# IRVLUTD/Proto-CLIP

Measured on AMD Instinct MI355X. Metric: query images/sec, ImageNet 16-shot ViT-B/16 (few-shot top-1 parity: tests/), higher is better.
Workload: dtype f16; 1 GPU; C3 ImageNet 16-shot ViT-B/16 conv-3x: prototype reduce + encode_image + adapter + dual-bank classify; batch_per_gpu=1024, global_batch=1024, classes=1000, shots=16, embed_dim=512, parallelism=dp1 (support rows and queries sharded; all-gather of class sums)

## Files before the change

### include/pclip.h

```cpp
#ifndef PCLIP_H
#define PCLIP_H
#include <stddef.h>
#include <stdint.h>

#ifdef __cplusplus
extern "C" {
#endif

#define PCLIP_ABI_VERSION 1
#define PCLIP_OK 0
#define PCLIP_E_INVALID (-1)
#define PCLIP_E_LAUNCH (-2)
#define PCLIP_E_WORKSPACE (-3)

typedef void* pclip_stream_t;

int pclip_abi_version(void);
const char* pclip_last_error(void);
int pclip_device_cus(void);
int pclip_gemm_timing(void* buf, int nslots);
int pclip_gemm_timing_count(void);
long pclip_gemm_kernel_launches(void);


int pclip_l2norm_rows_f16(const void* x, void* y, int R, int D, float* sq_out, pclip_stream_t stream);

int pclip_row_sqnorm_f16(const void* x, int R, int D, float* sq_out, pclip_stream_t stream);

int pclip_proto_build_f16(const void* mem, int N, int K, int D, int per_shot_norm, void* proto_f16,
                          float* proto_f32, float* proto_sq, pclip_stream_t stream);

int pclip_bank_reduce_f16(const void* feats, int A, int R, int D, const int32_t* perm, void* keys,
                          pclip_stream_t stream);

int pclip_transpose_f16(const void* x, int R, int C, void* y, pclip_stream_t stream);

int pclip_partial_sums_f16(const void* mem, const int32_t* labels, int R, int N, int D, int per_shot_norm,
                           float* sums, int32_t* counts, pclip_stream_t stream);

int pclip_proto_finalize(const float* sums, const int32_t* counts, int W, int N, int D, void* proto_f16,
                         float* proto_f32, float* proto_sq, pclip_stream_t stream);


int pclip_sqdist_f16(const void* q, const void* zi, const void* zt, int Q, int N, int D,
                     const float* q_sq, const float* zi_sq, const float* zt_sq,
                     float* d2i, float* d2t, int ldd, void* ws, size_t ws_bytes, pclip_stream_t stream);

int pclip_sqdist_f32(const float* q, const float* zi, const float* zt, int Q, int N, int D, float* d2i,
                     float* d2t, int ldd, pclip_stream_t stream);

int pclip_fuse_probs(const float* d2i, const float* d2t, int Q, int N, int ldd, float alpha,
                     float one_minus_alpha, float beta, float* p, int32_t* argmax, float* topk_p,
                     int32_t* topk_i, int k, pclip_stream_t stream);

int pclip_classify_f16(const void* q, const void* zi, const void* zt, int Q, int N, int D,
                       const float* q_sq, const float* zi_sq, const float* zt_sq, float alpha,
                       float one_minus_alpha, float beta, float* p, int32_t* argmax, float* topk_p,
                       int32_t* topk_i, int k, void* ws, size_t ws_bytes, pclip_stream_t stream);
int pclip_classify_ex_f16(const void* q, const void* zi, const void* zt, int Q, int N, int D,
                          const float* q_sq, const float* zi_sq, const float* zt_sq, float alpha,
                          float one_minus_alpha, float beta, float* p, int32_t* argmax, float* topk_p,
                          int32_t* topk_i, int k, int flags, void* ws, size_t ws_bytes, pclip_stream_t stream);

#define PCLIP_CLASSIFY_NO_SMALL 0x1
#define PCLIP_CLASSIFY_NO_MID 0x2
#define PCLIP_CLASSIFY_FORCE_MID 0x4
#define PCLIP_CLASSIFY_NO_PANELS 0x8
#define PCLIP_CLASSIFY_FORCE_PANELS 0x10
#define PCLIP_CLASSIFY_PANEL_TWO_PASS 0x20
#define PCLIP_CLASSIFY_PANEL_FORCE_SECOND 0x40
#define PCLIP_CLASSIFY_PANEL_EXACT 0x80

int pclip_classify_route(int Q, int N, int D, float alpha, float one_minus_alpha, float beta, int has_zt, int want_p, int want_argmax, int topk, size_t ws_bytes);
int pclip_classify_route_ex(int Q, int N, int D, float alpha, float one_minus_alpha, float beta, int has_zt, int want_p, int want_argmax, int topk, int flags,
                            size_t ws_bytes);

int pclip_classify_panel_stats(int* out3, int reset);

int pclip_classify_panel_dump_f16(const void* q, const void* zi, const void* zt, int Q, int N, int D, float* dump, int exact,
                                  void* ws, size_t ws_bytes, pclip_stream_t stream);


int pclip_cosine_logits_f16(const void* a, int lda, int M, const void* b, int ldb, int T, int D, float scale, int flags,
                            void* logits, int ldl, int32_t* argmax, void* topk_v, int32_t* topk_i, int k,
                            void* ws, size_t ws_bytes, pclip_stream_t stream);
#define PCLIP_LOGITS_NORMALIZE_A 0x1
#define PCLIP_LOGITS_NORMALIZE_B 0x2


int pclip_cosine_ce_f16(const void* a, int lda, int M, const void* b, int ldb, int T, int D, float scale, int flags, const void* labels,
                        float* lse_row, float* lse_col, float* row_loss, float* loss, void* ws, size_t ws_bytes, pclip_stream_t stream);
int pclip_cosine_ce_backward_f16(const void* a, int lda, int M, const void* b, int ldb, int T, int D, float scale, int flags, const void* labels,
                                 const float* lse_row, const float* lse_col, float weight, int direction, float* grad, float* dscale,
                                 void* ws, size_t ws_bytes, pclip_stream_t stream);
#define PCLIP_CE_NORMALIZE_A 0x1
#define PCLIP_CE_NORMALIZE_B 0x2
#define PCLIP_CE_SYMMETRIC 0x4
#define PCLIP_CE_LABELS_I64 0x8

int pclip_cosine_ce_grouped_f16(const void* a, int lda, size_t gsa, int M, const void* b, int ldb, size_t gsb, int T, int D, int G, float scale, int flags,
                                const void* labels, float* lse_row, float* row_loss, float* loss, void* ws, size_t ws_bytes, pclip_stream_t stream);
int pclip_cosine_ce_grouped_backward_f16(const void* a, int lda, size_t gsa, int M, const void* b, int ldb, size_t gsb, int T, int D, int G, float scale,
                                         int flags, const void* labels, const float* lse_row, float weight, int direction, float* grad, float* dscale,
                                         void* ws, size_t ws_bytes, pclip_stream_t stream);
size_t pclip_cosine_ce_grouped_workspace(int backward, int G, int M, int T, int D);


int pclip_cosine_sigmoid_f16(const void* a, int lda, int M, const void* b, int ldb, int T, int D, float scale, float bias, int flags,
                             const void* ids_a, const void* ids_b, float* row_loss, float* loss, void* ws, size_t ws_bytes, pclip_stream_t stream);
int pclip_cosine_sigmoid_backward_f16(const void* a, int lda, int M, const void* b, int ldb, int T, int D, float scale, float bias, int flags,
                                      const void* ids_a, const void* ids_b, float weight, int direction, float* grad, float* dscale, float* dbias,
                                      void* ws, size_t ws_bytes, pclip_stream_t stream);
#define PCLIP_SIG_NORMALIZE_A 0x1
#define PCLIP_SIG_NORMALIZE_B 0x2
#define PCLIP_SIG_IDS_I64 0x8


int pclip_tip_logits_f16(const void* f, int ldf, int Q, const void* keys, int ldk, int NK, const int32_t* seg, const void* w, int ldw, int N, int D,
                         float scale, float alpha, float beta, void* logits, int ldl, float* logits32, int32_t* argmax, pclip_stream_t stream);
int pclip_tip_grid_f16(const void* f, int ldf, int Q, const void* keys, int ldk, int NK, const int32_t* seg, const void* w, int ldw, int N, int D,
                       float scale, const float* betas, int nb, const float* alphas, int na, const int32_t* labels, int32_t* correct, pclip_stream_t stream);

int pclip_tip_keys_backward_f16(const void* f, int ldf, int Q, const void* keys, int ldk, int NK, const int32_t* seg, int N, int D, float alpha, float beta,
                                const float* dL, float* dkeys, void* ws, size_t ws_bytes, pclip_stream_t stream);

int pclip_hp_sweep(const float* d2i, const float* d2t, const int32_t* labels, int Q, int N, int ldd,
                   const float* alphas, const float* one_minus_alphas, int na, const float* betas,
                   int nb, int32_t* correct, pclip_stream_t stream);


int pclip_adapter_fc_f16(const void* x, int B, int D, int H, const void* w1, const void* g1, const void* b1,
                         const void* w2, const void* g2, const void* b2, float ratio, float one_minus_ratio,
                         int l2norm_out, void* y, float* y_sq, void* ws, size_t ws_bytes,
                         pclip_stream_t stream);

int pclip_layernorm_blend_f16(const void* h, const void* gamma, const void* beta, float eps, const void* x, float ratio,
                              float one_minus_ratio, int l2norm_out, void* y, float* y_sq, int R, int D,
                              pclip_stream_t stream);

int pclip_adapter_conv_f16(const void* x, int B, int D, int three_x, const void* conv1, const void* ln1w,
                           const void* ln1b, const void* conv2, const void* ln2w, const void* ln2b,
                           const void* conv3, const void* ln3w, const void* ln3b, int l2norm_out, void* y,
                           float* y_sq, pclip_stream_t stream);

int pclip_adapter_conv_w_f16(const void* x, int B, int D, int three_x, int width, const void* conv1, const void* ln1w,
                             const void* ln1b, const void* conv2, const void* ln2w, const void* ln2b,
                             const void* conv3, const void* ln3w, const void* ln3b, int l2norm_out, void* y,
                             float* y_sq, pclip_stream_t stream);


int pclip_gemm_f16(const void* A, int lda, const void* B, int ldb, void* C, int ldc, int M, int N, int K,
                   const void* bias, int act, const void* residual, pclip_stream_t stream);

int pclip_gemm4w_f16(const void* A, int lda, const void* B, int ldb, void* C, int ldc, int M, int N, int K,
                     const void* bias, int act, const void* residual, pclip_stream_t stream);
int pclip_gemm4w_var_f16(const void* A, int lda, const void* B, int ldb, void* C, int ldc, int M, int N, int K,
                         const void* bias, int act, const void* residual, int var, pclip_stream_t stream);
#define PCLIP_ROUTE_AUTO (-1)
#define PCLIP_ROUTE_GENERIC 5
#define PCLIP_ROUTE_RING 6
#define PCLIP_ROUTE_FIELDS 5
#define PCLIP_ROUTE_RAN_FOUR_WAVE 10
#define PCLIP_ROUTE_RAN_RING 11
#define PCLIP_ROUTE_RAN_GENERIC 12
int pclip_gemm_route_f16(const void* A, int lda, const void* B, int ldb, void* C, int ldc, int M, int N, int K,
                         const void* bias, int act, const void* residual, const float* scale, const float* shift,
                         int cfg, int may_split, int band, int band_n, int rev, int use4w, int cus,
                         int* report, int report_len, pclip_stream_t stream);
int pclip_gemm4w_stamp_buffer(void* stamps);
int pclip_gemm4w_config(int mode);

size_t pclip_gemm_splitk_workspace(int M, int N, int K);
int pclip_gemm_splitk_f16(const void* A, int lda, const void* B, int ldb, void* C, int ldc, int M, int N, int K,
                          const void* bias, int act, void* ws, size_t ws_bytes, pclip_stream_t stream);

int pclip_gemm_bn_f16(const void* A, int lda, const void* B, int ldb, void* C, int ldc, int M, int N, int K,
                      const float* scale, const float* shift, int relu, pclip_stream_t stream);

int pclip_gemm_bn_res_f16(const void* A, int lda, const void* B, int ldb, void* C, int ldc, int M, int N, int K,
                          const float* scale, const float* shift, const void* residual, pclip_stream_t stream);

int pclip_conv3x3_bn_f16(const void* x, const void* w, const void* zero_line, int B, int H, int W, int Cin, int Cout,
                         const float* scale, const float* shift, int relu, void* y, pclip_stream_t stream);

int pclip_conv3x3_strip_applies(int B, int H, int W, int Cin, int Cout);
int pclip_conv3x3_strip_config(int mode);

int pclip_conv3x3_pool_applies(int H, int W, int Cin, int Cout);
int pclip_conv3x3_bn_pool_f16(const void* x, const void* w, int B, int H, int W, int Cin, int Cout, const float* scale, const float* shift, void* y,
                              pclip_stream_t stream);

int pclip_stem_conv_applies(int R, int Cout);
int pclip_stem_conv_bn_f16(const void* img, int img_is_f32, int B, int R, const void* w, int Cout, const float* scale, const float* shift, int relu, void* y,
                           pclip_stream_t stream);

int pclip_layernorm_f16(const void* x, int ld_x, const float* gamma, const float* beta, float eps, void* y,
                        int R, int D, pclip_stream_t stream);

int pclip_add_layernorm_f16(const void* x, const void* delta, int ld, void* x_out, const float* gamma,
                            const float* beta, float eps, void* y, int R, int D, pclip_stream_t stream);

int pclip_attention_f16(const void* qkv, void* out, int B, int L, int H, int dh, int causal,
                        pclip_stream_t stream);

int pclip_attention_q_f16(const void* q, int ldq, long q_batch_stride, const void* kv, int ldkv, int k_off, int v_off, void* out,
                          int B, int L, int Lq, int H, int dh, int causal, pclip_stream_t stream);

int pclip_attention_long_q_f16(const void* q, int ldq, long q_batch_stride, const void* kv, int ldkv, int k_off, int v_off, void* out,
                               int B, int L, int Lq, int H, int dh, int causal, pclip_stream_t stream);

int pclip_attention_config(int mode, int max_grid);

int pclip_im2col_patches_f16(const void* img, int B, int R, int P, void* cols, int ld, pclip_stream_t stream);
int pclip_im2col_patches_f32(const float* img, int B, int R, int P, void* cols, int ld, pclip_stream_t stream);
int pclip_vit_assemble_tokens_f16(const void* patch_emb, const void* class_emb, const void* pos_emb, int B,
                                  int G2, int W, void* tokens, pclip_stream_t stream);
int pclip_vit_embed_ln_f16(const void* patch_emb, const void* class_emb, const void* pos_emb, int B, int G2, int W,
                           const float* gamma_pre, const float* beta_pre, const float* gamma_1, const float* beta_1, float eps,
                           void* x0, void* h, pclip_stream_t stream);

int pclip_text_embed_f16(const int64_t* tokens, const void* tok_emb, const void* pos_emb, int B, int L, int W,
                         int vocab, void* x, pclip_stream_t stream);
int pclip_gather_eot_f16(const void* x, const int64_t* tokens, int B, int L, int W, void* out,
                         pclip_stream_t stream);


int pclip_im2col3x3_f16(const void* x, long sb, long sh, long sw, long sc, int B, int H, int W, int C, int stride,
                        void* cols, int ld, pclip_stream_t stream);

int pclip_bn_act_f16(const void* x, const float* scale, const float* shift, const void* residual, int relu, void* y,
                     size_t rows, int C, pclip_stream_t stream);

int pclip_avgpool_nhwc_f16(const void* x, int B, int H, int W, int C, int k, void* y, pclip_stream_t stream);

int pclip_attnpool_tokens_f16(const void* x, const void* pos, int B, int HW, int C, void* tokens, pclip_stream_t stream);

int pclip_cast_f32_f16(const float* x, void* y, size_t n, pclip_stream_t stream);


int pclip_cast_f16_f32(const void* x, float* y, size_t n, pclip_stream_t stream);

int pclip_gemm_f32(const void* A, int a_f16, long rsa, long csa, const void* B, int b_f16, long rsb, long csb, float* C, int ldc,
                   int M, int N, int K, float alpha, float beta, void* ws, size_t ws_bytes, pclip_stream_t stream);

int pclip_colsum_f32(const float* x, int ldx, int R, int C, float scale, float* out, int accumulate, void* ws, size_t ws_bytes,
                     pclip_stream_t stream);

int pclip_addscaled_rows_f32(float* C, int ldc, const float* X, int ldx, const float* rowscale, float s, int R, int D,
                             pclip_stream_t stream);

int pclip_nll_grad(const float* d2i, const float* d2t, const int32_t* labels, int Q, int q_total, int N, int ldd, float alpha,
                   float one_minus_alpha, float beta, float* gi, float* gt, float* rowsum, float* nll, float* pmax,
                   int32_t* argmax, pclip_stream_t stream);

int pclip_fuse_probs_backward(const float* d2i, const float* d2t, const float* dp, int ldp, int Q, int N, int ldd, float alpha,
                              float one_minus_alpha, float beta, float* gi, float* gt, float* rowsum, pclip_stream_t stream);

int pclip_nll_mean_backward(const float* p, int ldp, const int32_t* labels, int Q, int N, const float* g, float* dp, int lddp,
                            pclip_stream_t stream);

int pclip_nll_rows(const float* p, int ldp, const int32_t* labels, int Q, int N, float* nll, float* pmax, int32_t* argmax,
                   pclip_stream_t stream);

int pclip_softmax_ce_rows(const float* S, int lds, int R, int C, float scale, float* dS, int ldds, float* loss,
                          pclip_stream_t stream);

int pclip_l2norm_rows_f32(const float* x, float* y, int R, int D, float eps, pclip_stream_t stream);
int pclip_l2norm_rows_backward_f32(const float* x, const float* gy, float* gx, int R, int D, float eps, int accumulate,
                                   pclip_stream_t stream);

int pclip_proto_backward_f16(const void* mem, const float* g, int N, int K, int D, int per_shot_norm, int final_norm, void* dmem,
                             pclip_stream_t stream);

int pclip_layernorm_backward_f16(const void* x, int ldx, const void* gamma, const void* dy, int lddy, int R, int D, float eps,
                                 float dy_scale, void* dx, int lddx, float* part, int nblk, pclip_stream_t stream);

int pclip_adapter_conv_backward_partials(int B, int D, int three_x);
int pclip_adapter_conv_backward_f16(const void* x, const void* g, int B, int D, int three_x, const void* conv1, const void* ln1w,
                                    const void* ln1b, const void* conv2, const void* ln2w, const void* ln2b, const void* conv3,
                                    const void* ln3w, float* pw1, float* pw2, float* pw3, float* pg1, float* pb1, float* pg2,
                                    float* pb2, float* pg3, float* pb3, pclip_stream_t stream);

int pclip_adapter_conv_w_backward_partials(int B, int D, int three_x, int width);
int pclip_adapter_conv_w_backward_f16(const void* x, const void* g, int B, int D, int three_x, int width, const void* conv1,
                                      const void* ln1w, const void* ln1b, const void* conv2, const void* ln2w, const void* ln2b,
                                      const void* conv3, const void* ln3w, float* pw1, float* pw2, float* pw3, float* pg1, float* pb1,
                                      float* pg2, float* pb2, float* pg3, float* pb3, pclip_stream_t stream);


int pclip_attention_backward_f16(const void* qkv, const void* dout, void* dqkv, int B, int L, int H, int dh, int causal,
                                 pclip_stream_t stream);

int pclip_quick_gelu_backward_f16(const void* u, const void* dy, void* du, size_t n, pclip_stream_t stream);

int pclip_colsum_f16(const void* x, int ldx, int R, int C, float* part, int nslice, pclip_stream_t stream);

int pclip_layernorm_backward_g32_f16(const void* x, int ldx, const float* gamma, const void* dy, int lddy, const void* residual, int ldr,
                                     int R, int D, float eps, void* dx, int lddx, float* part, int nblk, pclip_stream_t stream);



int pclip_prompt_embed_f16(const int64_t* tokens, int L_tok, const void* tok_emb, const void* pos_emb, const float* ctx, int class_specific,
                           int n_ctx, int N, int L_out, int W, int vocab, void* x, pclip_stream_t stream);

#define PCLIP_PROMPT_CTX_SLICE 16
int pclip_prompt_ctx_grad_f32(const void* dx, int N, int L_out, int n_ctx, int W, int class_specific, float* dctx, float* part, int nslice,
                              pclip_stream_t stream);


#define PCLIP_VPT_MAX_L 288
#define PCLIP_VPT_SLICE 16

int pclip_vpt_append_f16(const void* t, const float* ctx, int B, int L0, int P, int W, void* out, pclip_stream_t stream);

int pclip_vpt_replace_f16(void* x, const float* ctx, int B, int L0, int P, int W, pclip_stream_t stream);

int pclip_vpt_grad_f32(void* g, int B, int L0, int P, int W, int clear, float* dctx, float* part, int nslice, pclip_stream_t stream);



int pclip_rows_replace_f16(void* x, const float* ctx, int B, int L, int off, int P, int W, pclip_stream_t stream);

int pclip_rows_grad_f32(void* g, int B, int L, int off, int P, int W, int clear, float* dctx, float* part, int nslice, pclip_stream_t stream);

#define PCLIP_COUPLE_MAX_P 16
#define PCLIP_COUPLE_SLICE 32
int pclip_couple_fwd_f32(const float* X, const float* Wc, const float* bc, int depth, int P, int Wt, int Wv, float* Y, pclip_stream_t stream);

int pclip_couple_bwd_f32(const float* dY, const float* X, const float* Wc, int depth, int P, int Wt, int Wv, float* dWc, float* dbc, float* dX,
                         float* part, int nslice, pclip_stream_t stream);


#define PCLIP_COCOOP_MAX_B 16
int pclip_metanet_fwd_f32(const void* f, const float* W1, const float* b1, const float* W2, const float* b2, int B, int E, int Hd, int Wt, float* h,
                          float* pi, pclip_stream_t stream);

int pclip_metanet_bwd_f32(const float* dpi, const void* f, const float* h, const float* W2, int B, int E, int Hd, int Wt, float* dW1, float* db1,
                          float* dW2, float* db2, float* dpre, pclip_stream_t stream);

int pclip_prompt_embed_cond_f16(const int64_t* tokens, int L_tok, const void* tok_emb, const void* pos_emb, const float* ctx, const float* pi, int n_ctx,
                                int B, int N, int L_out, int W, int vocab, void* x, pclip_stream_t stream);

int pclip_prompt_cond_grad_f32(const void* dx, int B, int N, int L_out, int n_ctx, int W, float* dshift, float* dctx, float* dpi, float* part, int nslice,
                               pclip_stream_t stream);


#define PCLIP_EMBED_BWD_CHUNK 128

int pclip_text_embed_backward(const void* dx, const int64_t* sorted_ids, const int64_t* order, int B, int L, int W, int V, float* dE, float* dpos,
                              float* part, pclip_stream_t stream);

int pclip_vit_embed_backward_f16(const void* dt, int B, int L, int W, float* dpos, void* dpatch, pclip_stream_t stream);

int pclip_adamw_f16(void* p, const void* g, void* m, void* v, size_t n, double lr, double beta1, double beta2, double eps,
                    double weight_decay, int step, pclip_stream_t stream);

#define PCLIP_TOWER_CHUNK 4096
#define PCLIP_TOWER_ROW_BYTES 64
#define PCLIP_TOWER_STATE_BYTES 64
#define PCLIP_TOWER_PARAM_F16 0x1
#define PCLIP_TOWER_GRAD_F16 0x2
#define PCLIP_TOWER_ALIGNED 0x4
#define PCLIP_TOWER_DECAY 0x8

int pclip_tower_grad_sumsq(const void* table, int ntensors, int nchunks, float* partials, pclip_stream_t stream);

int pclip_tower_optim_finish(const float* partials, int nchunks, void* state, float max_norm, double beta1, double beta2, float growth,
                             float backoff, int growth_interval, int dynamic, pclip_stream_t stream);

int pclip_tower_adamw(const void* table, const float* hyper, int ntensors, int nchunks, const void* state, double beta1, double beta2,
                      double eps, pclip_stream_t stream);


int pclip_preprocess_u8(const void* const* srcs, const int32_t* desc, int B, int n_px, int max_box_h, float mean0, float mean1,
                        float mean2, float std0, float std1, float std2, void* out, int out_f16, void* ws, pclip_stream_t stream);

#define PCLIP_OP_SQDIST 1
#define PCLIP_OP_CLASSIFY 2
#define PCLIP_OP_ADAPTER_FC 3
#define PCLIP_OP_LOGITS 4
#define PCLIP_OP_COSINE_CE 5
#define PCLIP_OP_COSINE_CE_BACKWARD 6
#define PCLIP_OP_TIP_BACKWARD 7
#define PCLIP_OP_COSINE_SIGMOID 8
#define PCLIP_OP_COSINE_SIGMOID_BACKWARD 9
size_t pclip_workspace_bytes(int op, int Q, int N, int D);

#ifdef __cplusplus
}
#endif
#endif
```

### proto-clip_amd/_lib.py

```python
import ctypes
import os
from ctypes import c_char_p, c_double, c_float, c_int, c_long, c_size_t, c_void_p

import torch

_HERE = os.path.dirname(os.path.abspath(__file__))
LIB_PATH = os.path.join(_HERE, "libpclip.so")

OP_SQDIST, OP_CLASSIFY, OP_ADAPTER_FC, OP_LOGITS, OP_COSINE_CE, OP_COSINE_CE_BACKWARD, OP_TIP_BACKWARD = 1, 2, 3, 4, 5, 6, 7
OP_COSINE_SIGMOID, OP_COSINE_SIGMOID_BACKWARD = 8, 9
LOGITS_NORMALIZE_A, LOGITS_NORMALIZE_B = 0x1, 0x2
SIG_NORMALIZE_A, SIG_NORMALIZE_B, SIG_IDS_I64 = 0x1, 0x2, 0x8
CE_NORMALIZE_A, CE_NORMALIZE_B, CE_SYMMETRIC, CE_LABELS_I64 = 0x1, 0x2, 0x4, 0x8
CLASSIFY_NO_SMALL, CLASSIFY_NO_MID, CLASSIFY_FORCE_MID, CLASSIFY_NO_PANELS, CLASSIFY_FORCE_PANELS = 0x1, 0x2, 0x4, 0x8, 0x10
CLASSIFY_PANEL_TWO_PASS, CLASSIFY_PANEL_FORCE_SECOND, CLASSIFY_PANEL_EXACT = 0x20, 0x40, 0x80
TIP_MAX_ALPHAS, TIP_MAX_CLASSES, TIP_MAX_D = 32, 4096, 2048
TOWER_CHUNK, TOWER_ROW_BYTES, TOWER_STATE_BYTES = 4096, 64, 64
TOWER_PARAM_F16, TOWER_GRAD_F16, TOWER_ALIGNED, TOWER_DECAY = 0x1, 0x2, 0x4, 0x8
ROUTE_AUTO, ROUTE_GENERIC, ROUTE_RING, ROUTE_FIELDS = -1, 5, 6, 5
ROUTE_RAN = {0: "cfg0", 1: "cfg1", 2: "cfg2", 3: "cfg3", 4: "cfg4", 10: "four_wave", 11: "ring", 12: "generic"}
EMBED_BWD_CHUNK = 128
PROMPT_CTX_SLICE = 16
VPT_SLICE, VPT_MAX_L = 16, 288
COUPLE_MAX_P, COUPLE_SLICE = 16, 32
COCOOP_MAX_B = 16


class PclipError(RuntimeError):
    pass


_lib = None

_P = c_void_p
_SIGS = {
    "pclip_abi_version": [],
    "pclip_last_error": [],
    "pclip_device_cus": [],
    "pclip_gemm_kernel_launches": [],
    "pclip_l2norm_rows_f16": [_P, _P, c_int, c_int, _P, _P],
    "pclip_row_sqnorm_f16": [_P, c_int, c_int, _P, _P],
    "pclip_proto_build_f16": [_P, c_int, c_int, c_int, c_int, _P, _P, _P, _P],
    "pclip_bank_reduce_f16": [_P, c_int, c_int, c_int, _P, _P, _P],
    "pclip_transpose_f16": [_P, c_int, c_int, _P, _P],
    "pclip_partial_sums_f16": [_P, _P, c_int, c_int, c_int, c_int, _P, _P, _P],
    "pclip_proto_finalize": [_P, _P, c_int, c_int, c_int, _P, _P, _P, _P],
    "pclip_sqdist_f16": [_P, _P, _P, c_int, c_int, c_int, _P, _P, _P, _P, _P, c_int, _P, c_size_t, _P],
    "pclip_sqdist_f32": [_P, _P, _P, c_int, c_int, c_int, _P, _P, c_int, _P],
    "pclip_fuse_probs": [_P, _P, c_int, c_int, c_int, c_float, c_float, c_float, _P, _P, _P, _P, c_int, _P],
    "pclip_classify_f16": [_P, _P, _P, c_int, c_int, c_int, _P, _P, _P, c_float, c_float, c_float, _P, _P, _P,
                           _P, c_int, _P, c_size_t, _P],
    "pclip_classify_ex_f16": [_P, _P, _P, c_int, c_int, c_int, _P, _P, _P, c_float, c_float, c_float, _P, _P, _P,
                              _P, c_int, c_int, _P, c_size_t, _P],
    "pclip_classify_panel_stats": [_P, c_int],
    "pclip_classify_panel_dump_f16": [_P, _P, _P, c_int, c_int, c_int, _P, c_int, _P, c_size_t, _P],
    "pclip_gemm_timing": [_P, c_int],
    "pclip_gemm_timing_count": [],
    "pclip_classify_route": [c_int, c_int, c_int, c_float, c_float, c_float, c_int, c_int, c_int, c_int, c_size_t],
    "pclip_classify_route_ex": [c_int, c_int, c_int, c_float, c_float, c_float, c_int, c_int, c_int, c_int, c_int, c_size_t],
    "pclip_cosine_logits_f16": [_P, c_int, c_int, _P, c_int, c_int, c_int, c_float, c_int, _P, c_int, _P, _P, _P, c_int, _P, c_size_t, _P],
    "pclip_cosine_ce_f16": [_P, c_int, c_int, _P, c_int, c_int, c_int, c_float, c_int, _P, _P, _P, _P, _P, _P, c_size_t, _P],
    "pclip_cosine_ce_backward_f16": [_P, c_int, c_int, _P, c_int, c_int, c_int, c_float, c_int, _P, _P, _P, c_float, c_int, _P, _P, _P, c_size_t, _P],
    "pclip_cosine_ce_grouped_f16": [_P, c_int, c_size_t, c_int, _P, c_int, c_size_t, c_int, c_int, c_int, c_float, c_int, _P, _P, _P, _P, _P, c_size_t, _P],
    "pclip_cosine_ce_grouped_backward_f16": [_P, c_int, c_size_t, c_int, _P, c_int, c_size_t, c_int, c_int, c_int, c_float, c_int, _P, _P, c_float, c_int, _P, _P,
                                             _P, c_size_t, _P],
    "pclip_cosine_ce_grouped_workspace": [c_int, c_int, c_int, c_int, c_int],
    "pclip_cosine_sigmoid_f16": [_P, c_int, c_int, _P, c_int, c_int, c_int, c_float, c_float, c_int, _P, _P, _P, _P, _P, c_size_t, _P],
    "pclip_cosine_sigmoid_backward_f16": [_P, c_int, c_int, _P, c_int, c_int, c_int, c_float, c_float, c_int, _P, _P, c_float, c_int, _P, _P, _P, _P, c_size_t, _P],
    "pclip_tip_logits_f16": [_P, c_int, c_int, _P, c_int, c_int, _P, _P, c_int, c_int, c_int, c_float, c_float, c_float, _P, c_int, _P, _P, _P],
    "pclip_tip_grid_f16": [_P, c_int, c_int, _P, c_int, c_int, _P, _P, c_int, c_int, c_int, c_float, _P, c_int, _P, c_int, _P, _P, _P],
    "pclip_tip_keys_backward_f16": [_P, c_int, c_int, _P, c_int, c_int, _P, c_int, c_int, c_float, c_float, _P, _P, _P, c_size_t, _P],
    "pclip_hp_sweep": [_P, _P, _P, c_int, c_int, c_int, _P, _P, c_int, _P, c_int, _P, _P],
    "pclip_adapter_fc_f16": [_P, c_int, c_int, c_int, _P, _P, _P, _P, _P, _P, c_float, c_float, c_int, _P, _P, _P,
                             c_size_t, _P],
    "pclip_layernorm_blend_f16": [_P, _P, _P, c_float, _P, c_float, c_float, c_int, _P, _P, c_int, c_int, _P],
    "pclip_adapter_conv_f16": [_P, c_int, c_int, c_int, _P, _P, _P, _P, _P, _P, _P, _P, _P, c_int, _P, _P, _P],
    "pclip_adapter_conv_w_f16": [_P, c_int, c_int, c_int, c_int, _P, _P, _P, _P, _P, _P, _P, _P, _P, c_int, _P, _P, _P],
    "pclip_gemm_f16": [_P, c_int, _P, c_int, _P, c_int, c_int, c_int, c_int, _P, c_int, _P, _P],
    "pclip_gemm4w_f16": [_P, c_int, _P, c_int, _P, c_int, c_int, c_int, c_int, _P, c_int, _P, _P],
    "pclip_gemm4w_var_f16": [_P, c_int, _P, c_int, _P, c_int, c_int, c_int, c_int, _P, c_int, _P, c_int, _P],
    "pclip_gemm_route_f16": [_P, c_int, _P, c_int, _P, c_int, c_int, c_int, c_int, _P, c_int, _P, _P, _P, c_int, c_int, c_int, c_int, c_int, c_int, c_int,
                             _P, c_int, _P],
    "pclip_gemm4w_stamp_buffer": [_P],
    "pclip_gemm4w_config": [c_int],
    "pclip_gemm_splitk_workspace": [c_int, c_int, c_int],
    "pclip_gemm_splitk_f16": [_P, c_int, _P, c_int, _P, c_int, c_int, c_int, c_int, _P, c_int, _P, c_size_t, _P],
    "pclip_gemm_bn_f16": [_P, c_int, _P, c_int, _P, c_int, c_int, c_int, c_int, _P, _P, c_int, _P],
    "pclip_gemm_bn_res_f16": [_P, c_int, _P, c_int, _P, c_int, c_int, c_int, c_int, _P, _P, _P, _P],
    "pclip_conv3x3_bn_f16": [_P, _P, _P, c_int, c_int, c_int, c_int, c_int, _P, _P, c_int, _P, _P],
    "pclip_conv3x3_strip_applies": [c_int, c_int, c_int, c_int, c_int],
    "pclip_conv3x3_strip_config": [c_int],
    "pclip_conv3x3_pool_applies": [c_int, c_int, c_int, c_int],
    "pclip_conv3x3_bn_pool_f16": [_P, _P, c_int, c_int, c_int, c_int, c_int, _P, _P, _P, _P],
    "pclip_stem_conv_applies": [c_int, c_int],
    "pclip_stem_conv_bn_f16": [_P, c_int, c_int, c_int, _P, c_int, _P, _P, c_int, _P, _P],
    "pclip_layernorm_f16": [_P, c_int, _P, _P, c_float, _P, c_int, c_int, _P],
    "pclip_add_layernorm_f16": [_P, _P, c_int, _P, _P, _P, c_float, _P, c_int, c_int, _P],
    "pclip_attention_f16": [_P, _P, c_int, c_int, c_int, c_int, c_int, _P],
    "pclip_attention_q_f16": [_P, c_int, c_long, _P, c_int, c_int, c_int, _P, c_int, c_int, c_int, c_int, c_int, c_int, _P],
    "pclip_attention_long_q_f16": [_P, c_int, c_long, _P, c_int, c_int, c_int, _P, c_int, c_int, c_int, c_int, c_int, c_int, _P],
    "pclip_attention_config": [c_int, c_int],
    "pclip_im2col_patches_f16": [_P, c_int, c_int, c_int, _P, c_int, _P],
    "pclip_im2col_patches_f32": [_P, c_int, c_int, c_int, _P, c_int, _P],
    "pclip_vit_assemble_tokens_f16": [_P, _P, _P, c_int, c_int, c_int, _P, _P],
    "pclip_vit_embed_ln_f16": [_P, _P, _P, c_int, c_int, c_int, _P, _P, _P, _P, c_float, _P, _P, _P],
    "pclip_text_embed_f16": [_P, _P, _P, c_int, c_int, c_int, c_int, _P, _P],
    "pclip_gather_eot_f16": [_P, _P, c_int, c_int, c_int, _P, _P],
    "pclip_im2col3x3_f16": [_P, c_long, c_long, c_long, c_long, c_int, c_int, c_int, c_int, c_int, _P, c_int, _P],
    "pclip_bn_act_f16": [_P, _P, _P, _P, c_int, _P, c_size_t, c_int, _P],
    "pclip_avgpool_nhwc_f16": [_P, c_int, c_int, c_int, c_int, c_int, _P, _P],
    "pclip_attnpool_tokens_f16": [_P, _P, c_int, c_int, c_int, _P, _P],
    "pclip_cast_f32_f16": [_P, _P, c_size_t, _P],
    "pclip_cast_f16_f32": [_P, _P, c_size_t, _P],
    "pclip_gemm_f32": [_P, c_int, c_long, c_long, _P, c_int, c_long, c_long, _P, c_int, c_int, c_int, c_int, c_float, c_float, _P, c_size_t, _P],
    "pclip_colsum_f32": [_P, c_int, c_int, c_int, c_float, _P, c_int, _P, c_size_t, _P],
    "pclip_adapter_conv_backward_f16": [_P, _P, c_int, c_int, c_int] + [_P] * 8 + [_P] * 9 + [_P],
    "pclip_adapter_conv_backward_partials": [c_int, c_int, c_int],
    "pclip_adapter_conv_w_backward_f16": [_P, _P, c_int, c_int, c_int, c_int] + [_P] * 8 + [_P] * 9 + [_P],
    "pclip_adapter_conv_w_backward_partials": [c_int, c_int, c_int, c_int],
    "pclip_addscaled_rows_f32": [_P, c_int, _P, c_int, _P, c_float, c_int, c_int, _P],
    "pclip_nll_grad": [_P, _P, _P, c_int, c_int, c_int, c_int, c_float, c_float, c_float, _P, _P, _P, _P, _P, _P, _P],
    "pclip_nll_rows": [_P, c_int, _P, c_int, c_int, _P, _P, _P, _P],
    "pclip_fuse_probs_backward": [_P, _P, _P, c_int, c_int, c_int, c_int, c_float, c_float, c_float, _P, _P, _P, _P],
    "pclip_nll_mean_backward": [_P, c_int, _P, c_int, c_int, _P, _P, c_int, _P],
    "pclip_softmax_ce_rows": [_P, c_int, c_int, c_int, c_float, _P, c_int, _P, _P],
    "pclip_l2norm_rows_f32": [_P, _P, c_int, c_int, c_float, _P],
    "pclip_l2norm_rows_backward_f32": [_P, _P, _P, c_int, c_int, c_float, c_int, _P],
    "pclip_proto_backward_f16": [_P, _P, c_int, c_int, c_int, c_int, c_int, _P, _P],
    "pclip_layernorm_backward_f16": [_P, c_int, _P, _P, c_int, c_int, c_int, c_float, c_float, _P, c_int, _P, c_int, _P],
    "pclip_attention_backward_f16": [_P, _P, _P, c_int, c_int, c_int, c_int, c_int, _P],
    "pclip_quick_gelu_backward_f16": [_P, _P, _P, c_size_t, _P],
    "pclip_colsum_f16": [_P, c_int, c_int, c_int, _P, c_int, _P],
    "pclip_layernorm_backward_g32_f16": [_P, c_int, _P, _P, c_int, _P, c_int, c_int, c_int, c_float, _P, c_int, _P, c_int, _P],
    "pclip_prompt_embed_f16": [_P, c_int, _P, _P, _P, c_int, c_int, c_int, c_int, c_int, c_int, _P, _P],
    "pclip_prompt_ctx_grad_f32": [_P, c_int, c_int, c_int, c_int, c_int, _P, _P, c_int, _P],
    "pclip_vpt_append_f16": [_P, _P, c_int, c_int, c_int, c_int, _P, _P],
    "pclip_vpt_replace_f16": [_P, _P, c_int, c_int, c_int, c_int, _P],
    "pclip_vpt_grad_f32": [_P, c_int, c_int, c_int, c_int, c_int, _P, _P, c_int, _P],
    "pclip_rows_replace_f16": [_P, _P, c_int, c_int, c_int, c_int, c_int, _P],
    "pclip_rows_grad_f32": [_P, c_int, c_int, c_int, c_int, c_int, c_int, _P, _P, c_int, _P],
    "pclip_couple_fwd_f32": [_P, _P, _P, c_int, c_int, c_int, c_int, _P, _P],
    "pclip_couple_bwd_f32": [_P, _P, _P, c_int, c_int, c_int, c_int, _P, _P, _P, _P, c_int, _P],
    "pclip_metanet_fwd_f32": [_P, _P, _P, _P, _P, c_int, c_int, c_int, c_int, _P, _P, _P],
    "pclip_metanet_bwd_f32": [_P, _P, _P, _P, c_int, c_int, c_int, c_int, _P, _P, _P, _P, _P, _P],
    "pclip_prompt_embed_cond_f16": [_P, c_int, _P, _P, _P, _P, c_int, c_int, c_int, c_int, c_int, c_int, _P, _P],
    "pclip_prompt_cond_grad_f32": [_P, c_int, c_int, c_int, c_int, c_int, _P, _P, _P, _P, c_int, _P],
    "pclip_text_embed_backward": [_P, _P, _P, c_int, c_int, c_int, c_int, _P, _P, _P, _P],
    "pclip_vit_embed_backward_f16": [_P, c_int, c_int, c_int, _P, _P, _P],
    "pclip_adamw_f16": [_P, _P, _P, _P, c_size_t, c_double, c_double, c_double, c_double, c_double, c_int, _P],
    "pclip_tower_grad_sumsq": [_P, c_int, c_int, _P, _P],
    "pclip_tower_optim_finish": [_P, c_int, _P, c_float, c_double, c_double, c_float, c_float, c_int, c_int, _P],
    "pclip_tower_adamw": [_P, _P, c_int, c_int, _P, c_double, c_double, c_double, _P],
    "pclip_preprocess_u8": [_P, _P, c_int, c_int, c_int, c_float, c_float, c_float, c_float, c_float, c_float, _P, c_int, _P, _P],
    "pclip_workspace_bytes": [c_int, c_int, c_int, c_int],
}
_RESTYPES = {"pclip_last_error": c_char_p, "pclip_workspace_bytes": c_size_t, "pclip_gemm_splitk_workspace": c_size_t, "pclip_cosine_ce_grouped_workspace": c_size_t, "pclip_gemm_kernel_launches": c_long}
EXPORTED_SYMBOLS = tuple(_SIGS)


def load():
    global _lib
    if _lib is not None:
        return _lib
    if not os.path.exists(LIB_PATH):
        raise PclipError(
            f"{LIB_PATH} is missing: the HIP extension is not built. Run `python -c 'import __graft_entry__ as g; "
            "g.build()'` (or `make -C proto-clip_amd/csrc`). There is no CPU/eager fallback for this path.")
    lib = ctypes.CDLL(LIB_PATH)
    for name, argtypes in _SIGS.items():
        fn = getattr(lib, name)
        fn.argtypes = argtypes
        fn.restype = _RESTYPES.get(name, c_int)
    if lib.pclip_abi_version() != 1:
        raise PclipError(f"libpclip ABI version {lib.pclip_abi_version()} != 1")
    _lib = lib
    return lib


def check(rc: int, what: str):
    if rc != 0:
        msg = load().pclip_last_error()
        raise PclipError(f"{what} failed (rc={rc}): {msg.decode() if msg else '?'}")


def ptr(t):
    return None if t is None else c_void_p(t.data_ptr())


def stream():
    return c_void_p(torch.cuda.current_stream().cuda_stream)


def require_cuda(*tensors):
    dev = None
    for t in tensors:
        if t is None:
            continue
        if not t.is_cuda:
            raise PclipError("libpclip operates on device tensors only (got a CPU tensor); there is no CPU fallback")
        if dev is None:
            dev = t.device
        elif t.device != dev:
            raise PclipError(f"operands on different GPUs ({dev} and {t.device}): move them to one device")
    if dev is not None and dev.index != torch.cuda.current_device():
        raise PclipError(f"operands live on {dev} but the current device is cuda:{torch.cuda.current_device()}: call "
                         f"torch.cuda.set_device({dev.index}) or wrap the call in `with torch.cuda.device({dev.index}):`")


def workspace_bytes(op: int, Q: int, N: int, D: int) -> int:
    return int(load().pclip_workspace_bytes(op, Q, N, D))
```

### proto-clip_amd/csrc/pclip_attention.hip

```cpp
#include "pclip_attention_tile.h"
#include <stdlib.h>
#include <type_traits>

namespace {
constexpr int ATT_MAX_L = 288;

template <int NW, int VAR, bool QF = false>
__global__ __launch_bounds__(NW * 64, NW / 2) void attention_kernel(const half_t* __restrict__ qp, int ldq, long q_batch,
                                                           const half_t* __restrict__ kvp, int ldkv, int k_off, int v_off,
                                                           half_t* __restrict__ out, int L, int Lq, int H, int causal, int NT,
                                                           int ) {
    extern __shared__ __attribute__((aligned(16))) char smem[];
    const int LP = NT * 32;
    half_t* Ks = reinterpret_cast<half_t*>(smem);
    half_t* Vs = Ks + LP * ATT_DH;
    const int b = blockIdx.x / H, h = blockIdx.x % H;
    const int W = H * ATT_DH;
    const half_t* kbase = kvp + (size_t)b * L * ldkv + h * ATT_DH + k_off;
    const half_t* vbase = kvp + (size_t)b * L * ldkv + h * ATT_DH + v_off;
    const half_t* qbase = qp + (size_t)b * q_batch + h * ATT_DH;
    const int tid = threadIdx.x, lane = tid & 63, wave = tid >> 6;
    half8_t qf0[4];
    if (QF) {
        const int q0 = wave * 32 + (lane & 31), qc0 = q0 < Lq ? q0 : Lq - 1;
#pragma unroll
        for (int s_ = 0; s_ < 4; ++s_) qf0[s_] = ld_half8(qbase + (size_t)qc0 * ldq + s_ * 16 + (lane >> 5) * 8);
    }

    for (int r0 = wave * 8; r0 < LP; r0 += NW * 8) {
        const int r = r0 + (lane >> 3);
        const int c = (lane & 7) ^ pgemm::swz_key(r);
        const int rc = r < L ? r : L - 1;
        __builtin_amdgcn_global_load_lds((pgemm::gbl_ptr_t)(kbase + (size_t)rc * ldkv + c * 8),
                                         (pgemm::lds_ptr_t)(Ks + r0 * ATT_DH), 16, 0, 0);
    }
    for (int r0 = wave * 8; r0 < LP; r0 += NW * 8) {
        const int r = r0 + (lane >> 3);
        const int c = (lane & 7) ^ (((r >> 1) & 1) << 2);
        const int rc = r < L ? r : L - 1;
        __builtin_amdgcn_global_load_lds((pgemm::gbl_ptr_t)(vbase + (size_t)rc * ldkv + c * 8),
                                         (pgemm::lds_ptr_t)(Vs + r0 * ATT_DH), 16, 0, 0);
    }
#ifndef PCLIP_ATT_VBAR
#define PCLIP_ATT_VBAR 1
#endif
    constexpr bool VB = PCLIP_ATT_VBAR && QF;
    if (VB) {
        const int nv = (LP - wave * 8 + NW * 8 - 1) / (NW * 8);
        if (nv <= 1) pgemm::wait_vm<1>(); else if (nv == 2) pgemm::wait_vm<2>(); else if (nv == 3) pgemm::wait_vm<3>(); else pgemm::wait_vm<4>();
        pgemm::lds_barrier();
    } else
        __syncthreads();

    const int hi = lane >> 5, ql = lane & 31;
    int voff[2];
    attn_voff(lane, voff);
    const int NTq = (Lq + 31) >> 5;
    auto process = [&](int qb, const half8_t (&qf)[4]) {
        const int q = qb * 32 + ql;
        float16_t o[2];
        float lrun;
        attn_query_tile<false, VAR, VB>(Ks, Vs, qf, q, qb, L, causal, NT, hi, ql, voff, o, lrun);
        attn_store_tile(out + ((size_t)b * Lq + q) * W + h * ATT_DH, o, lrun, hi, q < Lq);
    };
    if (QF) {
        if (wave < NTq) process(wave, qf0);
        else if (VB) { pgemm::wait_vm<0>(); pgemm::lds_barrier(); }
        return;
    }
    for (int qb = wave; qb < NTq; qb += NW) {
        const int q = qb * 32 + ql;
        const int qc = q < Lq ? q : Lq - 1;
        half8_t qf[4];
#pragma unroll
        for (int s = 0; s < 4; ++s) qf[s] = ld_half8(qbase + (size_t)qc * ldq + s * 16 + hi * 8);
        process(qb, qf);
    }
}

template <int NW, int WPS, int VAR>
__global__ __launch_bounds__(NW * 64, WPS) void attention_pipe_kernel(const half_t* __restrict__ qp, int ldq, long q_batch,
                                                                      const half_t* __restrict__ kvp, int ldkv, int k_off, int v_off,
                                                                      half_t* __restrict__ out, int L, int H, int causal, int NT, int KR,
                                                                      int nitems) {
    extern __shared__ __attribute__((aligned(16))) char smem[];
    constexpr int NST = 4;
    constexpr int MAXP = 4;
    constexpr int RB = ATT_DH * 2;
    const int LP = NT * 32;
    const int BUF = (KR + LP) * RB;
    const int tid = threadIdx.x, lane = tid & 63, wave = __builtin_amdgcn_readfirstlane(tid >> 6);
    const int hi = lane >> 5, ql = lane & 31;
    const int W = H * ATT_DH, G = gridDim.x;
    const bool has_tile = wave < NT;
    const unsigned lds0 = (unsigned)(size_t)(pgemm::lds_ptr_t)smem;
    char* Qs = smem + 2 * BUF;
    int voff[2];
    attn_voff(lane, voff);
    int kvo[MAXP], vvo[MAXP], qvo[MAXP];
#pragma unroll
    for (int i = 0; i < MAXP; ++i) {
        const int r = wave * 8 + i * NW * 8 + (lane >> 3);
        const int rc = r < L ? r : L - 1;
        const int ck = ((lane & 7) ^ pgemm::swz_key(r)) << 3, cv = ((lane & 7) ^ (((r >> 1) & 1) << 2)) << 3;
        kvo[i] = (rc * ldkv + ck) * 2;
        vvo[i] = (rc * ldkv + cv) * 2;
        qvo[i] = (rc * ldq + ck) * 2;
    }
    const int q = wave * 32 + ql;
    auto stage = [&](int item, int buf) {
        const int b = item / H, h = item - b * H;
        const uint4_t rkv = attn_rsrc(kvp + (size_t)b * L * ldkv + h * ATT_DH);
        const uint4_t rq = attn_rsrc(qp + (size_t)b * q_batch + h * ATT_DH);
        const unsigned kb = lds0 + buf * BUF, vb = kb + KR * RB, qb = lds0 + 2 * BUF;
#pragma unroll
        for (int i = 0; i < MAXP; ++i) {
            const int r0 = wave * 8 + i * NW * 8;
            if (r0 < KR) attn_dma16(rkv, kvo[i], k_off * 2, kb + r0 * RB);
        }
#pragma unroll
        for (int i = 0; i < MAXP; ++i) {
            const int r0 = wave * 8 + i * NW * 8;
            if (r0 < LP) attn_dma16(rkv, vvo[i], v_off * 2, vb + r0 * RB);
        }
#pragma unroll
        for (int i = 0; i < MAXP; ++i) {
            const int r0 = wave * 8 + i * NW * 8;
            if (r0 < KR) attn_dma16(rq, qvo[i], 0, qb + r0 * RB);
        }
    };
    int item = blockIdx.x;
    if (item >= nitems) return;
    stage(item, 0);
    for (int it = 0; item < nitems; item += G, ++it) {
        const int cur = it & 1;
        if (has_tile && it > 0) pgemm::wait_vm<NST>(); else pgemm::wait_vm<0>();
        pgemm::lds_barrier();
        half8_t qf[4];
        if (has_tile) {
            const int qr = q < KR ? q : KR - 1;
#pragma unroll
            for (int s = 0; s < 4; ++s)
                qf[s] = *reinterpret_cast<const half8_t*>(Qs + qr * RB + (((s * 2 + hi) ^ pgemm::swz_key(qr)) << 4));
        }
        pgemm::lds_barrier();
#ifndef PCLIP_ATT_ABL
#define PCLIP_ATT_ABL 0
#endif
        const int next = item + G;
        if (next < nitems && !(PCLIP_ATT_ABL & 1)) stage(next, cur ^ 1);
        if (has_tile) {
            const half_t* Ks = reinterpret_cast<const half_t*>(smem + cur * BUF);
            const half_t* Vs = Ks + KR * ATT_DH;
            float16_t o[2];
            float lrun;
#ifndef PCLIP_ATT_STAGGER
#define PCLIP_ATT_STAGGER 0
#endif
#if PCLIP_ATT_STAGGER && defined(__HIP_DEVICE_COMPILE__)
            if (wave >= NW / 2) __builtin_amdgcn_s_sleep(PCLIP_ATT_STAGGER);
#endif
            if (PCLIP_ATT_ABL & 2) {
#pragma unroll
                for (int j = 0; j < 2; ++j)
#pragma unroll
                    for (int e = 0; e < 16; ++e) o[j][e] = (float)qf[e & 3][e & 7];
                lrun = 1.f;
            } else
                attn_query_tile<true, VAR>(Ks, Vs, qf, q, wave, L, causal, NT, hi, ql, voff, o, lrun);
            const int b = item / H, h = item - b * H;
            attn_store_tile(out + ((size_t)b * L + q) * W + h * ATT_DH, o, lrun, hi, q < L && !(PCLIP_ATT_ABL & 4));
        }
    }
}

}

static int att_mode_from_env() {
    const char* e = getenv("PCLIP_ATT_PIPE");
    return e && (e[0] == '0' || e[0] == '1') ? e[0] - '0' : -1;
}
static int g_att_mode = att_mode_from_env(), g_att_grid = 0;
extern "C" int pclip_attention_config(int mode, int max_grid) {
    PCLIP_REQUIRE(mode >= -1 && mode <= 1 && max_grid >= 0, "pclip_attention_config: bad mode=%d max_grid=%d", mode, max_grid);
    g_att_mode = mode;
    g_att_grid = max_grid;
    return PCLIP_OK;
}

extern "C" int pclip_attention_q_f16(const void* q, int ldq, long q_batch_stride, const void* kv, int ldkv, int k_off, int v_off,
                                     void* out, int B, int L, int Lq, int H, int dh, int causal, pclip_stream_t stream) {
    PCLIP_REQUIRE(q && kv && out, "pclip_attention_q_f16: null pointer");
    PCLIP_REQUIRE(dh == ATT_DH, "pclip_attention_q_f16: head dim %d unsupported (must be 64)", dh);
    PCLIP_REQUIRE(B >= 0 && H > 0 && L > 0 && L <= ATT_MAX_L && Lq > 0 && Lq <= L, "pclip_attention_q_f16: bad B=%d H=%d L=%d Lq=%d (L <= %d)",
                  B, H, L, Lq, ATT_MAX_L);
    PCLIP_REQUIRE(!causal || Lq == L, "pclip_attention_q_f16: the causal mask needs all queries (Lq == L)");
    PCLIP_REQUIRE(ldq % 8 == 0 && ldkv % 8 == 0 && k_off % 8 == 0 && v_off % 8 == 0 && q_batch_stride % 8 == 0,
                  "pclip_attention_q_f16: strides / offsets must be multiples of 8 halves");
    if (B == 0) return PCLIP_OK;
    const int NT = ceil_div(L, 32), LP = NT * 32;
    const long nitems = (long)B * H;
    const int cus = pclip_device_cus();
    const int KR = (L + 7) / 8 * 8;
    const size_t plds = (2 * (size_t)(KR + LP) + KR) * ATT_DH * 2;
    if (Lq == L && g_att_mode != 0 && NT <= 8 && plds <= 160 * 1024 && cus > 0 && g_att_mode == 1) {
        static DevOnce pipe_attr;
        if (int e = pclip_raise_lds(pipe_attr, {(const void*)attention_pipe_kernel<4, 2, PCLIP_ATT_VAR_SHORT>, (const void*)attention_pipe_kernel<8, 2, PCLIP_ATT_VAR_LONG>},
                                    160 * 1024, "pclip_attention_f16"))
            return e;
        int per_cu = NT <= 4 ? (int)((160 * 1024) / plds) : 1;
        per_cu = per_cu < 1 ? 1 : (per_cu > 2 ? 2 : per_cu);
        long grid = (long)cus * per_cu;
        if (g_att_grid > 0 && g_att_grid < grid) grid = g_att_grid;
        if (grid > nitems) grid = nitems;
        if (NT <= 4)
            attention_pipe_kernel<4, 2, PCLIP_ATT_VAR_SHORT><<<(int)grid, 256, plds, (hipStream_t)stream>>>((const half_t*)q, ldq, q_batch_stride, (const half_t*)kv, ldkv,
                                                                                      k_off, v_off, (half_t*)out, L, H, causal, NT, KR, (int)nitems);
        else
            attention_pipe_kernel<8, 2, PCLIP_ATT_VAR_LONG><<<(int)grid, 512, plds, (hipStream_t)stream>>>((const half_t*)q, ldq, q_batch_stride, (const half_t*)kv, ldkv,
                                                                                      k_off, v_off, (half_t*)out, L, H, causal, NT, KR, (int)nitems);
        return pclip_check_launch("attention (pipelined)");
    }
    const size_t lds = 2 * (size_t)LP * ATT_DH * 2;
    static DevOnce attr_set;
    if (int e = pclip_raise_lds(attr_set, {(const void*)attention_kernel<8, PCLIP_ATT_VAR_LONG>, (const void*)attention_kernel<4, PCLIP_ATT_VAR_LONG>,
                                           (const void*)attention_kernel<4, PCLIP_ATT_VAR_SHORT>, (const void*)attention_kernel<8, PCLIP_ATT_VAR_LONG, true>,
                                           (const void*)attention_kernel<4, PCLIP_ATT_VAR_SHORT, true>},
                                80 * 1024, "pclip_attention_f16"))
        return e;
#define PCLIP_ATT_LAUNCH(NW, VAR)                                                                                                         \
    attention_kernel<NW, VAR><<<B * H, NW * 64, lds, (hipStream_t)stream>>>((const half_t*)q, ldq, q_batch_stride, (const half_t*)kv, ldkv, k_off, \
                                                                             v_off, (half_t*)out, L, Lq, H, causal, NT, 0)
    static const bool qfirst = pclip_env_on("PCLIP_ATT_QFIRST");
    if (PCLIP_ATT_QF4 && qfirst && NT <= 4 && Lq == L && !causal)
        attention_kernel<4, PCLIP_ATT_VAR_SHORT, true><<<B * H, 4 * 64, lds, (hipStream_t)stream>>>((const half_t*)q, ldq, q_batch_stride, (const half_t*)kv, ldkv, k_off,
                                                                                                     v_off, (half_t*)out, L, Lq, H, causal, NT, 0);
    else if ((Lq + 31) / 32 > 4 && (Lq + 31) / 32 <= 8 && NT <= 8 && qfirst)
        attention_kernel<8, PCLIP_ATT_VAR_LONG, true><<<B * H, 8 * 64, lds, (hipStream_t)stream>>>((const half_t*)q, ldq, q_batch_stride, (const half_t*)kv, ldkv, k_off,
                                                                                                    v_off, (half_t*)out, L, Lq, H, causal, NT, 0);
    else if ((Lq + 31) / 32 > 4) PCLIP_ATT_LAUNCH(8, PCLIP_ATT_VAR_LONG);
    else if (NT > 4) PCLIP_ATT_LAUNCH(4, PCLIP_ATT_VAR_LONG);
    else PCLIP_ATT_LAUNCH(4, PCLIP_ATT_VAR_SHORT);
#undef PCLIP_ATT_LAUNCH
    return pclip_check_launch("attention");
}

extern "C" int pclip_attention_f16(const void* qkv, void* out, int B, int L, int H, int dh, int causal,
                                   pclip_stream_t stream) {
    PCLIP_REQUIRE(qkv && out, "pclip_attention_f16: null pointer");
    PCLIP_REQUIRE(H > 0 && L > 0, "pclip_attention_f16: bad H=%d L=%d", H, L);
    const int W = H * dh;
    return pclip_attention_q_f16(qkv, 3 * W, (long)L * 3 * W, qkv, 3 * W, W, 2 * W, out, B, L, L, H, dh, causal, stream);
}
```

### proto-clip_amd/csrc/pclip_gemm4w.hip

```cpp
#include "pclip_gemm.h"
#include "pclip_epilogue.h"
#include "pclip_gemm4w_loop.inc"
#include <stdlib.h>

unsigned long long* pclip_gemm_time_slot();
static unsigned* g_gemm4w_stamps = nullptr;

namespace {
using Cfg4 = pgemm::Cfg<256, 256, 2, 2>;
constexpr int RING_BYTES = 5 * 32768;
typedef unsigned uint4_t __attribute__((ext_vector_type(4)));

enum Build : int {
    PRODUCT = 0,
    STRESS = 1,
    NO_EPILOGUE = 6,
    STAMPED = 8,
};
constexpr bool is_build(int var) { return var == PRODUCT || var == STRESS || var == NO_EPILOGUE || var == STAMPED; }

__device__ __forceinline__ int fresh_tid(int wave) {
#if defined(__HIP_DEVICE_COMPILE__)
    int lane;
    asm volatile("v_mbcnt_lo_u32_b32 %0, -1, 0\n\tv_mbcnt_hi_u32_b32 %0, -1, %0" : "=v"(lane));
    return wave * 64 + lane;
#else
    return 0;
#endif
}

template <bool BATCH, class Ahead, class Pre, class Post, class Stamp>
__device__ __forceinline__ void epilogue4w(const pgemm::Acc16& acc, int wave, char* buf0, char* buf1, const Ahead& ahead, const Pre& pre, const Post& post,
                                           const Stamp& stamp) {
    constexpr int NSLAB = 4;
    const int tid = fresh_tid(wave);
    const int lane = tid & 63, wm = wave >> 1, wn = wave & 1;
    constexpr int RB = 512;
    auto stage = [&](int k) {
        char* buf = (k & 1) ? buf1 : buf0;
#pragma unroll
        for (int j = 0; j < 4; ++j)
#pragma unroll
            for (int g = 0; g < 4; ++g) {
                const int rl = (g >> 1) * 16 + (lane & 15), coff = (g & 1) * 16 + 4 * (lane >> 4);
                const int ml = wm * 32 + rl, nl = wn * 128 + j * 32 + coff;
                const half4_t hv = pre(acc.q[2 * k + (g >> 1)][2 * j + (g & 1)]);
                const int unit = (nl >> 2) ^ (ml & 15);
                *reinterpret_cast<half4_t*>(buf + ml * RB + unit * 8) = hv;
            }
    };
#pragma unroll
    for (int ps = 0; ps < 8; ++ps) ahead(0, ps);
    pgemm::lds_barrier();
    stamp(3);
    stage(0);
#pragma unroll
    for (int k = 0; k < NSLAB; ++k) {
        pgemm::lds_barrier();
        stamp(4 + k);
        const bool stage_first = (wave & 1) == 0;
        if (k + 1 < NSLAB && stage_first) stage(k + 1);
        const char* buf = (k & 1) ? buf1 : buf0;
        const int c = tid & 31;
        if (BATCH) {
            half8_t hv[8];
#pragma unroll
            for (int ps = 0; ps < 8; ++ps) {
                const int r = (tid >> 5) + ps * 8;
                hv[ps] = *reinterpret_cast<const half8_t*>(buf + r * RB + ((c ^ ((r & 15) >> 1)) << 4));
            }
#pragma unroll
            for (int ps = 0; ps < 8; ++ps) {
                if ((tid >> 5) & 1) hv[ps] = half8_t{hv[ps][4], hv[ps][5], hv[ps][6], hv[ps][7], hv[ps][0], hv[ps][1], hv[ps][2], hv[ps][3]};
                post(k, ps, hv[ps]);
                if (k + 1 < NSLAB) ahead(k + 1, ps);
            }
        } else {
#pragma unroll
            for (int ps = 0; ps < 8; ++ps) {
                const int r = (tid >> 5) + ps * 8;
                const int pair = c ^ ((r & 15) >> 1);
                half8_t hv = *reinterpret_cast<const half8_t*>(buf + r * RB + pair * 16);
                if (r & 1) hv = half8_t{hv[4], hv[5], hv[6], hv[7], hv[0], hv[1], hv[2], hv[3]};
                post(k, ps, hv);
                if (k + 1 < NSLAB) ahead(k + 1, ps);
            }
        }
        if (k + 1 < NSLAB && !stage_first) stage(k + 1);
    }
}

__device__ __forceinline__ uint4_t make_rsrc(const half_t* base, long bytes) {
    const uint64_t a = (uint64_t)base;
    return uint4_t{(uint32_t)__builtin_amdgcn_readfirstlane((uint32_t)a), (uint32_t)__builtin_amdgcn_readfirstlane((uint32_t)(a >> 32)) & 0xffffu,
                   (uint32_t)__builtin_amdgcn_readfirstlane((uint32_t)(bytes < 0x7fffffffL ? bytes : 0x7fffffffL)), 0x00020000u};
}

struct LaneK {
    int voffa0, voffa1, voffb0, voffb1, lanea, laneb;
    __device__ __forceinline__ LaneK(int lda, int ldb, int ring0, int wave) {
        const int lane = fresh_tid(wave) & 63, wm = wave >> 1, wn = wave & 1;
        const int r0 = wave * 64 + (lane >> 3), r1 = r0 + 8;
        const int c0 = (lane & 7) ^ pgemm::swz_key(r0), c1 = (lane & 7) ^ pgemm::swz_key(r1);
        voffa0 = (r0 * lda + c0 * 8) * 2;
        voffa1 = (r1 * lda + c1 * 8) * 2;
        voffb0 = (r0 * ldb + c0 * 8) * 2;
        voffb1 = (r1 * ldb + c1 * 8) * 2;
        const int lpart = (lane & 15) * pgemm::ROW_BYTES + (((lane >> 4) ^ ((lane & 15) >> 1)) << 4);
        lanea = ring0 + wm * 16384 + lpart;
        laneb = ring0 + wn * 16384 + lpart;
    }
};

template <int ACT, bool HAS_BIAS, int VAR>
__global__ __launch_bounds__(256, 1) void linear4w_kernel(const half_t* __restrict__ A, int lda, const half_t* __restrict__ B, int ldb, int M,
                                                          int N, int K, const half_t* __restrict__ bias, half_t* Cout, int ldc, int tiles_n,
                                                          int ntiles, const half_t* residual, int rev, int band, unsigned* stamps) {
    extern __shared__ __attribute__((aligned(16))) char smem[];
    constexpr bool STAMP = VAR == STAMPED;
    unsigned stampv = 0;
    int stamp_tile = 0;
    auto stamp = [&](int phase) {
        if constexpr (STAMP) {
#if defined(__HIP_DEVICE_COMPILE__)
            if (stamp_tile < 8) { const unsigned t = (unsigned)wall_clock64(); if ((fresh_tid(0) & 63) == stamp_tile * 8 + phase) stampv = t; }
#endif
        }
    };
    const int G = gridDim.x;
    int tile = pgemm::xcd_remap(blockIdx.x, G);
    if (tile >= ntiles) return;
    if constexpr (!STAMP) pgemm::time_begin(reinterpret_cast<unsigned long long*>(stamps));
    const int wave = __builtin_amdgcn_readfirstlane(threadIdx.x >> 6);
    const int nt = K / pgemm::BK;
    const int row16a = 16 * lda * 2, row16b = 16 * ldb * 2;
    const int ring0 = (int)(uintptr_t)smem;
    const int wbase = __builtin_amdgcn_readfirstlane(ring0 + wave * 8192);
    const int tiles_m = ntiles / tiles_n;
    auto origin = [&](int tl, int& m0, int& n0) {
        const int t = rev ? ntiles - 1 - tl : tl;
        int tm, tn;
        if (band <= 0 || band >= tiles_n) { tm = t / tiles_n; tn = t - tm * tiles_n; }
        else {
            const int per_band = tiles_m * band, bnd = t / per_band, r = t - bnd * per_band;
            const int w = band < tiles_n - bnd * band ? band : tiles_n - bnd * band;
            tm = r / w;
            tn = bnd * band + r - tm * w;
        }
        m0 = tm * 256;
        n0 = tn * 256;
    };
    auto rsrc_a = [&](int m0) { return make_rsrc(A + (size_t)m0 * lda, (long)(M - m0) * lda * 2); };
    auto rsrc_b = [&](int n0) { return make_rsrc(B + (size_t)n0 * ldb, (long)(N - n0) * ldb * 2); };
    auto bias_ptr = [&](int n0) { return (HAS_BIAS ? bias : A) + n0 + (wave & 1) * 128 + 4 * ((fresh_tid(wave) & 63) >> 4); };

    int ring_wr = 0, ring_rda = 0, ring_rdb = 0x8000;
    int m0, n0;
    origin(tile, m0, n0);
    uint4_t rsa2 = rsrc_a(m0), rsb2 = rsrc_b(n0);
    half4_t nb[8];
    {
        const half_t* biasp = bias_ptr(n0);
        const LaneK lk(lda, ldb, ring0, wave);
        const int voffa0 = lk.voffa0, voffa1 = lk.voffa1, voffb0 = lk.voffb0, voffb1 = lk.voffb1;
        int so[8], st_cnt, st_tmp, st_scr;
#if defined(__HIP_DEVICE_COMPILE__)
        if (VAR == STRESS) PCLIP_GEMM4W_COLD_STRESS(); else PCLIP_GEMM4W_COLD();
#endif
    }
    for (; tile < ntiles; tile += G) {
        stamp(0);
        const bool full = m0 + 256 <= M;
        const uint4_t rsa = rsa2, rsb = rsb2;
        int m0n = m0, n0n = n0;
        if (tile + G < ntiles) origin(tile + G, m0n, n0n);
        rsa2 = rsrc_a(m0n);
        rsb2 = rsrc_b(n0n);
        const half_t* biasp = bias_ptr(n0n);
        pgemm::Acc16 acc;
#pragma unroll
        for (int j = 0; j < 8; ++j) {
            const float4_t b = HAS_BIAS ? float4_t{(float)nb[j][0], (float)nb[j][1], (float)nb[j][2], (float)nb[j][3]} : float4_t{0.f, 0.f, 0.f, 0.f};
#pragma unroll
            for (int i = 0; i < 8; ++i) acc.q[i][j] = b;
        }
        pgemm::lds_barrier();
        stamp(1);
        {
            const LaneK lk(lda, ldb, ring0, wave);
            const int voffa0 = lk.voffa0, voffa1 = lk.voffa1, voffb0 = lk.voffb0, voffb1 = lk.voffb1, lanea = lk.lanea, laneb = lk.laneb;
            half8_t fr[32];
            int vr[4], so[8], st_cnt, st_tmp, st_scr;
#if defined(__HIP_DEVICE_COMPILE__)
            if constexpr (VAR == STRESS) PCLIP_GEMM4W_LOOP_STRESS(); else PCLIP_GEMM4W_LOOP();
#endif
        }
        stamp(2);
        if constexpr (VAR == NO_EPILOGUE) {
#if defined(__HIP_DEVICE_COMPILE__)
#pragma unroll
            for (int i = 0; i < 8; ++i)
#pragma unroll
                for (int j = 0; j < 8; ++j) asm volatile("" ::"a"(acc.q[i][j]));
#endif
            m0 = m0n;
            n0 = n0n;
            continue;
        }
        char* buf0 = smem + ring_wr;
        char* buf1 = smem + (ring_wr + 0x8000 == RING_BYTES ? 0 : ring_wr + 0x8000);
        const int etid = fresh_tid(wave);
        const int evoff = ((etid >> 5) * ldc + 8 * (etid & 31)) * 2;
        const long cbytes = ((long)(M - m0) * ldc - n0) * 2;
        pgemm::rsrc_t rc;
#if defined(__HIP_DEVICE_COMPILE__)
        {
            auto mk = [&](const half_t* base) {
                const uint64_t a = (uint64_t)(base + (size_t)m0 * ldc + n0);
                const uint32_t lo = __builtin_amdgcn_readfirstlane((uint32_t)a), hi = __builtin_amdgcn_readfirstlane((uint32_t)(a >> 32));
                return __builtin_amdgcn_make_buffer_rsrc((void*)(((uint64_t)hi << 32) | lo), 0, __builtin_amdgcn_readfirstlane((int)(cbytes < 0x7fffffffL ? cbytes : 0x7fffffffL)), 0x00020000);
            };
            rc = mk(Cout);
        }
#endif
        constexpr bool RES = ACT == 6;
        auto soff = [&](int k, int ps) { return ((ps >> 2) * 128 + k * 32 + 8 * (ps & 3)) * ldc * 2; };
        auto pre = [&](float4_t v) { return ACT == 1 ? quick_gelu16x4(v) : cvt16x4(v); };
        constexpr bool FLAT = RES;
        constexpr bool BATCH = !RES;
        const int col = n0 + 8 * (etid & 31);
        half8_t rr[RES ? 8 : 1];
        auto ahead = [&](int k, int ps) {
            if (!RES) return;
            const int r = (ps >> 2) * 128 + k * 32 + 8 * (ps & 3) + (etid >> 5);
            if (full || m0 + r < M) rr[RES ? ps : 0] = ld_half8(residual + (size_t)(m0 + r) * ldc + col);
        };
        auto add_res = [&](int pass, half8_t h) { return add_residual16x8<false>(rr[RES ? pass : 0], h); };
        if (!FLAT)
            epilogue4w<true>(acc, wave, buf0, buf1, ahead, pre, [&](int k, int ps, half8_t h) {
#if defined(__HIP_DEVICE_COMPILE__)
                __builtin_amdgcn_raw_buffer_store_b128(__builtin_bit_cast(uint4_t, h), rc, evoff, soff(k, ps), PCLIP_NT_STORE ? 2 : 0);
#endif
            }, stamp);
        else if (full)
            epilogue4w<BATCH>(acc, wave, buf0, buf1, ahead, pre, [&](int k, int ps, half8_t h) {
                const int r = (ps >> 2) * 128 + k * 32 + 8 * (ps & 3) + (etid >> 5);
                st_out(Cout + (size_t)(m0 + r) * ldc + col, add_res(ps, h));
            }, stamp);
        else
            epilogue4w<BATCH>(acc, wave, buf0, buf1, ahead, pre, [&](int k, int ps, half8_t h) {
                const int r = (ps >> 2) * 128 + k * 32 + 8 * (ps & 3) + (etid >> 5);
                if (m0 + r < M) st_out(Cout + (size_t)(m0 + r) * ldc + col, add_res(ps, h));
            }, stamp);
        m0 = m0n;
        n0 = n0n;
        ++stamp_tile;
    }
    if constexpr (!STAMP) pgemm::time_end(reinterpret_cast<unsigned long long*>(stamps));
    if constexpr (STAMP) {
        const int l = fresh_tid(wave) & 63;
        const int slot = (blockIdx.x == 0 ? 0 : (blockIdx.x == gridDim.x / 2 ? 2 : -1));
        if (stamps && slot >= 0 && (wave == 0 || wave == 3)) {
            const int w = slot + (wave == 3 ? 1 : 0);
            stamps[w * 64 + l] = stampv;
#if defined(__HIP_DEVICE_COMPILE__)
            if (l == 0) stamps[256 + w] = (unsigned)wall_clock64();
#endif
        }
    }
}

template <int ACT, bool HAS_BIAS, int VAR>
int launch4w_v(const half_t* A, int lda, const half_t* B, int ldb, int M, int N, int K, const half_t* bias, half_t* C, int ldc, const half_t* residual,
               int slots, int rev, int band, hipStream_t s) {
    static DevOnce attr;
    auto kern = linear4w_kernel<ACT, HAS_BIAS, VAR>;
    if (int e = pclip_raise_lds(attr, {(const void*)kern}, RING_BYTES, "pclip_gemm4w_f16")) return e;
    const int tiles_m = ceil_div(M, Cfg4::BM), tiles_n = N / Cfg4::BN, ntiles = tiles_m * tiles_n;
    const int grid = ntiles < slots ? ntiles : slots;
    kern<<<grid, 256, RING_BYTES, s>>>(A, lda, B, ldb, M, N, K, bias, C, ldc, tiles_n, ntiles, residual, rev, band, VAR == STAMPED ? g_gemm4w_stamps : reinterpret_cast<unsigned*>(pclip_gemm_time_slot()));
    return pclip_check_launch("gemm4w_f16");
}

template <int ACT, bool HAS_BIAS>
int launch4w(const half_t* A, int lda, const half_t* B, int ldb, int M, int N, int K, const half_t* bias, half_t* C, int ldc, const half_t* residual,
             int slots, int rev, int band, int var, hipStream_t s) {
#define PCLIP_4W_CASE(V) case V: return launch4w_v<ACT, HAS_BIAS, V>(A, lda, B, ldb, M, N, K, bias, C, ldc, residual, slots, rev, band, s)
    if constexpr (HAS_BIAS) {
        switch (var) {
            PCLIP_4W_CASE(STRESS); PCLIP_4W_CASE(NO_EPILOGUE); PCLIP_4W_CASE(STAMPED);
            default: break;
        }
    } else if (var == STRESS) return launch4w_v<ACT, HAS_BIAS, STRESS>(A, lda, B, ldb, M, N, K, bias, C, ldc, residual, slots, rev, band, s);
#undef PCLIP_4W_CASE
    return launch4w_v<ACT, HAS_BIAS, PRODUCT>(A, lda, B, ldb, M, N, K, bias, C, ldc, residual, slots, rev, band, s);
}
}

extern "C" int pclip_gemm4w_stamp_buffer(void* p) { g_gemm4w_stamps = (unsigned*)p; return PCLIP_OK; }

bool pclip_gemm4w_supports(int M, int N, int K, int lda, int ldb, int ldc, const void* C, const void* bias, const void* residual, int act) {
    if (N % 256 || K % 64 || K < 192 || M < 1) return false;
    if (lda % 8 || ldb % 8 || ldc % 8 || ((uintptr_t)C & 15) || ((uintptr_t)bias & 7) || ((uintptr_t)residual & 15)) return false;
    if ((long)256 * lda * 2 >= 0x7fffffffL || (long)256 * ldb * 2 >= 0x7fffffffL) return false;
    if (!(act == 0 || act == 1 || act == 6)) return false;
    if (act == 6 && !(bias && residual)) return false;
    if (act != 6 && residual) return false;
    return true;
}

int pclip_gemm4w_launch_var(const half_t* A, int lda, const half_t* B, int ldb, int M, int N, int K, const half_t* bias, half_t* C, int ldc, int act,
                            const half_t* residual, int slots, int rev, int band, int var, hipStream_t s) {
    if (act == 6) return launch4w<6, true>(A, lda, B, ldb, M, N, K, bias, C, ldc, residual, slots, rev, band, var, s);
    if (act == 1) return bias ? launch4w<1, true>(A, lda, B, ldb, M, N, K, bias, C, ldc, residual, slots, rev, band, var, s)
                              : launch4w<1, false>(A, lda, B, ldb, M, N, K, bias, C, ldc, residual, slots, rev, band, var, s);
    return bias ? launch4w<0, true>(A, lda, B, ldb, M, N, K, bias, C, ldc, residual, slots, rev, band, var, s)
                : launch4w<0, false>(A, lda, B, ldb, M, N, K, bias, C, ldc, residual, slots, rev, band, var, s);
}

int pclip_gemm4w_launch(const half_t* A, int lda, const half_t* B, int ldb, int M, int N, int K, const half_t* bias, half_t* C, int ldc, int act,
                        const half_t* residual, int slots, int rev, int band, hipStream_t s) {
    static const bool stress = getenv("PCLIP_RACE_STRESS") && getenv("PCLIP_RACE_STRESS")[0] == '1';
    return pclip_gemm4w_launch_var(A, lda, B, ldb, M, N, K, bias, C, ldc, act, residual, slots, rev, band, stress ? STRESS : PRODUCT, s);
}

extern "C" int pclip_gemm4w_var_f16(const void* A, int lda, const void* B, int ldb, void* C, int ldc, int M, int N, int K, const void* bias, int act,
                                    const void* residual, int var, pclip_stream_t stream) {
    PCLIP_REQUIRE(A && B && C, "pclip_gemm4w_f16: null pointer");
    PCLIP_REQUIRE(act == 0 || act == 1, "pclip_gemm4w_f16: unknown activation %d", act);
    PCLIP_REQUIRE(lda >= K && ldb >= K && ldc >= N, "pclip_gemm4w_f16: bad leading dims");
    PCLIP_REQUIRE(is_build(var), "pclip_gemm4w_f16: unknown loop variant %d", var);
    if (M == 0) return PCLIP_OK;
    const int a = (residual && bias && act == 0) ? 6 : act;
    PCLIP_REQUIRE(pclip_gemm4w_supports(M, N, K, lda, ldb, ldc, C, bias, residual, a),
                  "pclip_gemm4w_f16: shape M=%d N=%d K=%d / alignment outside the four-wave kernel (N %% 256 == 0, K %% 64 == 0, K >= 192; residual needs bias, no activation)", M, N, K);
    const char* be = getenv("PCLIP_GEMM4W_BAND");
    return pclip_gemm4w_launch_var((const half_t*)A, lda, (const half_t*)B, ldb, M, N, K, (const half_t*)bias, (half_t*)C, ldc, a, (const half_t*)residual, pclip_cus(), 0,
                                   be ? atoi(be) : 0, var, (hipStream_t)stream);
}

extern "C" int pclip_gemm4w_f16(const void* A, int lda, const void* B, int ldb, void* C, int ldc, int M, int N, int K, const void* bias, int act,
                                const void* residual, pclip_stream_t stream) {
    return pclip_gemm4w_var_f16(A, lda, B, ldb, C, ldc, M, N, K, bias, act, residual, PRODUCT, stream);
}
```

### proto-clip_amd/csrc/pclip_linear.hip

```cpp
#include "pclip_encoder_common.h"
#include <stdlib.h>
#include <type_traits>

unsigned long long* pclip_gemm_time_slot();

namespace {
template <class C, bool HAS_BIAS, int ACT>
__global__ __launch_bounds__(C::NTHREADS, 2) void linear_fast_kernel(const half_t* __restrict__ A, int lda,
                                                                     const half_t* __restrict__ B, int ldb, int M, int N,
                                                                     int K, const half_t* __restrict__ bias,
                                                                     const float* __restrict__ scale,
                                                                     const float* __restrict__ shift,
                                                                     half_t* Cout, int ldc, int tiles_n,
                                                                     int ntiles, const half_t* residual = nullptr, int band = 0,
                                                                     unsigned long long* tslot = nullptr) {
    extern __shared__ __attribute__((aligned(16))) char smem[];
    constexpr bool KT = C::TAIL;
    constexpr bool M16 = true;
    half_t* bias_lds = reinterpret_cast<half_t*>(smem + C::LDS_BYTES);
    float* affine_lds = reinterpret_cast<float*>(smem + C::LDS_BYTES);
    constexpr bool AFFINE = ACT == 2 || ACT == 3 || ACT == 5;
    const int G = gridDim.x;
    int tile = pgemm::xcd_remap(blockIdx.x, G);
    if (tile >= ntiles) return;
    pgemm::time_begin(tslot);
    const int tiles_m_all = ntiles / tiles_n;
    auto decomp = [&](int t, int& tm, int& tn) {
        if (band < 0) t = ntiles - 1 - t;
        if (band <= 0 || band >= tiles_n) { tm = t / tiles_n; tn = t - tm * tiles_n; return; }
        const int per_band = tiles_m_all * band, bnd = t / per_band, r = t - bnd * per_band;
        const int w = band < tiles_n - bnd * band ? band : tiles_n - bnd * band;
        tm = r / w;
        tn = bnd * band + r - tm * w;
    };
    int p = 0;
    const int tid = threadIdx.x, lane = tid & 63, wave = __builtin_amdgcn_readfirstlane(tid >> 6), wn = wave % C::WN;
    using TP = std::conditional_t<(PCLIP_DMA_ROLES && C::NWAVES == 8), pgemm::TilePairR<C, KT>, pgemm::TilePair<C, KT>>;
    TP tp;
    const pgemm::rsrc_t rs_bias = pgemm::make_rsrc(bias, KT ? (unsigned)N * 2u : 0x7fffffffu), rs_scale = pgemm::make_rsrc(scale, KT ? (unsigned)N * 4u : 0x7fffffffu),
                        rs_shift = pgemm::make_rsrc(shift, KT ? (unsigned)N * 4u : 0x7fffffffu);
    (void)rs_bias; (void)rs_scale; (void)rs_shift;
    auto copy_bias = [&](int t, int par) {
        int tm_, tn;
        decomp(t, tm_, tn);
        (void)tn;
#if defined(__HIP_DEVICE_COMPILE__)
        if (lane < C::BN / 8)
            __builtin_amdgcn_raw_ptr_buffer_load_lds(rs_bias, (pgemm::lds_ptr_t)(bias_lds + par * C::BN), 16, (tn * C::BN + lane * 8) * 2, 0, 0, 0);
#endif
    };
    auto copy_affine = [&](int t, int par) {
        int tm_, tn;
        decomp(t, tm_, tn);
        (void)tn;
#if defined(__HIP_DEVICE_COMPILE__)
        if (lane < C::BN / 4) {
            __builtin_amdgcn_raw_ptr_buffer_load_lds(rs_scale, (pgemm::lds_ptr_t)(affine_lds + par * 2 * C::BN), 16, (tn * C::BN + lane * 4) * 4, 0, 0, 0);
            __builtin_amdgcn_raw_ptr_buffer_load_lds(rs_shift, (pgemm::lds_ptr_t)(affine_lds + par * 2 * C::BN + C::BN), 16, (tn * C::BN + lane * 4) * 4, 0, 0, 0);
        }
#endif
    };
    if (HAS_BIAS || AFFINE) {
        if (AFFINE) copy_affine(tile, 0); else copy_bias(tile, 0);
        pgemm::wait_vm<0>();
        pgemm::lds_barrier();
    }
    {
        int tm, tn;
        decomp(tile, tm, tn);
        tp.prepare(A, lda, B, ldb, M, N, tm * C::BM, tn * C::BN, wave, lane, K);
        tp.stage(0, smem + p * C::STAGE_BYTES, wave);
    }
    constexpr int YOUNGER = C::NH * C::NPASS + (AFFINE ? 2 : (HAS_BIAS ? 1 : 0));
    bool prev_full = false;
    int parity = 0;
    for (; tile < ntiles; tile += G, parity ^= 1) {
        int tile_m, tile_n;
        decomp(tile, tile_m, tile_n);
        const int m0 = tile_m * C::BM, n0 = tile_n * C::BN;
        const bool full = m0 + C::BM <= M;
        pgemm::Acc<C> acc;
        if (HAS_BIAS) {
            if (KT ? K <= pgemm::BK : K == pgemm::BK) { pgemm::wait_vm<0>(); pgemm::lds_barrier(); }
            const half_t* bl = bias_lds + parity * C::BN + wn * (C::BN / C::WN);
#pragma unroll
            for (int j = 0; j < C::TN; ++j)
#pragma unroll
                for (int g = 0; g < 4; ++g) {
                    const int coff = (g & 1) * 16 + 4 * (lane >> 4);
                    const half4_t b = *reinterpret_cast<const half4_t*>(bl + j * 32 + coff);
#pragma unroll
                    for (int e = 0; e < 4; ++e)
#pragma unroll
                        for (int i = 0; i < C::TM; ++i) acc.v[i][j][4 * g + e] = (float)b[e];
                }
            copy_bias(tile + G < ntiles ? tile + G : tile, parity ^ 1);
        }
        if (AFFINE) copy_affine(tile + G < ntiles ? tile + G : tile, parity ^ 1);
        const int next = tile + G;
        pgemm::mainloop_sr<C, YOUNGER, !HAS_BIAS, TP>(tp, KT ? (K + pgemm::BK - 1) / pgemm::BK : K / pgemm::BK, smem, acc, p, prev_full, wave, lane);
        if (next < ntiles) {
            int tm, tn;
            decomp(next, tm, tn);
            tp.prepare(A, lda, B, ldb, M, N, tm * C::BM, tn * C::BN, wave, lane, K);
            tp.stage(0, smem + p * C::STAGE_BYTES, wave);
        }
        char* stg = smem + (p ^ 1) * C::STAGE_BYTES;
        int etid = tid;
#if defined(__HIP_DEVICE_COMPILE__)
        asm volatile("" : "+v"(etid));
#endif
        const int col = n0 + 8 * (etid % C::CPR);
        const bool colok = !KT || col < N;
        auto pre = [&](int i, int j, int coff, float4_t v, int rl, int g) {
            if (ACT == 1) return quick_gelu16x4(v);
            if (AFFINE) {
                const float* st = affine_lds + parity * 2 * C::BN + wn * (C::BN / C::WN) + j * 32 + coff;
                return bn16x4<ACT == 3>(v, *reinterpret_cast<const float4_t*>(st), *reinterpret_cast<const float4_t*>(st + C::BN));
            }
            return cvt16x4(v);
        };
        constexpr bool RES = ACT == 5 || ACT == 6;
        constexpr bool PIPE = PCLIP_EPI_PIPE && (ACT == 1 || PCLIP_EPI_PIPE == 2) && C::BM == 256 && C::BN == 256 && C::WM == 2 && C::WN == 4;
        half8_t rr[RES ? C::NPASS : 1];
        auto ahead = [&](int k) {
            if (!RES) return;
#pragma unroll
            for (int ps = 0; ps < 4; ++ps) {
                const int rs = etid / C::CPR + ps * 16, r = (rs >> 5) * 128 + k * 32 + (rs & 31);
                if ((full || m0 + r < M) && colok) rr[RES ? (k & 1) * 4 + ps : 0] = ld_half8(residual + (size_t)(m0 + r) * ldc + col);
            }
        };
        auto slab = [&](int h) {
            if (!RES) return;
#pragma unroll
            for (int ps = 0; ps < C::NPASS; ++ps) {
                const int r = h * C::HR + etid / C::CPR + ps * C::ROWS_PER_PASS;
                if ((full || m0 + r < M) && colok) rr[ps] = ld_half8(residual + (size_t)(m0 + r) * ldc + col);
            }
        };
        auto add_res = [&](int pass, half8_t h) { return add_residual16x8<ACT == 5>(rr[RES ? pass % C::NPASS : 0], h); };
        if constexpr (PIPE) {
            static_assert(C::NPASS == 8, "rr[pass % NPASS] pairs slab parity and pass");
            if (full)
                pgemm::epilogue_pipe<C>(acc, stg, ahead, pre, [&](int r, int c, int pass, half8_t h) {
                    const size_t o = (size_t)(m0 + r) * ldc + col;
                    if (RES) h = add_res(pass, h);
                    if (colok) st_out(Cout + o, h);
                });
            else
                pgemm::epilogue_pipe<C>(acc, stg, ahead, pre, [&](int r, int c, int pass, half8_t h) {
                    const size_t o = (size_t)(m0 + r) * ldc + col;
                    if (RES) h = add_res(pass, h);
                    if (m0 + r < M && colok) st_out(Cout + o, h);
                });
            prev_full = full;
            continue;
        }
        if (full)
            pgemm::epilogue_f16<C, M16>(acc, stg, slab, pre, [&](int r, int c, int pass, half8_t h) {
                const size_t o = (size_t)(m0 + r) * ldc + col;
                if (RES) h = add_res(pass, h);
                if (colok) st_out(Cout + o, h);
            });
        else
            pgemm::epilogue_f16<C, M16>(acc, stg, slab, pre, [&](int r, int c, int pass, half8_t h) {
                const size_t o = (size_t)(m0 + r) * ldc + col;
                if (RES) h = add_res(pass, h);
                if (m0 + r < M && colok) st_out(Cout + o, h);
            });
        prev_full = full;
    }
    pgemm::time_end(tslot);
}


template <class C, int ACT>
__global__ __launch_bounds__(C::NTHREADS, 2) void conv3x3_fast_kernel(const half_t* __restrict__ x,
                                                                      const half_t* __restrict__ w, int H, int W, int Cin, int M,
                                                                      int N, const float* __restrict__ scale,
                                                                      const float* __restrict__ shift, half_t* __restrict__ Cout,
                                                                      int tiles_n, int ntiles) {
    extern __shared__ __attribute__((aligned(16))) char smem[];
    float* affine_lds = reinterpret_cast<float*>(smem + C::LDS_BYTES);
    constexpr bool TAIL = C::TAIL;
    const int G = gridDim.x;
    int tile = pgemm::xcd_remap(blockIdx.x, G);
    if (tile >= ntiles) return;
    const int nt = (9 * Cin + pgemm::BK - 1) / pgemm::BK, ldb = nt * pgemm::BK;
    const int tid = threadIdx.x, lane = tid & 63, wave = __builtin_amdgcn_readfirstlane(tid >> 6), wn = wave % C::WN;
    pgemm::ConvPair<C, TAIL> cp(x, H, W, Cin, M);
    pgemm::ConvGather<C, TAIL>& ga = cp.a.g;
    const pgemm::rsrc_t rs_scale = pgemm::make_rsrc(scale, TAIL ? (unsigned)N * 4u : 0x7fffffffu), rs_shift = pgemm::make_rsrc(shift, TAIL ? (unsigned)N * 4u : 0x7fffffffu);
    (void)rs_scale; (void)rs_shift;
    auto copy_affine = [&](int t, int par) {
        const int tn = t - (t / tiles_n) * tiles_n;
        (void)tn;
#if defined(__HIP_DEVICE_COMPILE__)
        if (lane < C::BN / 4) {
            __builtin_amdgcn_raw_ptr_buffer_load_lds(rs_scale, (pgemm::lds_ptr_t)(affine_lds + par * 2 * C::BN), 16, (tn * C::BN + lane * 4) * 4, 0, 0, 0);
            __builtin_amdgcn_raw_ptr_buffer_load_lds(rs_shift, (pgemm::lds_ptr_t)(affine_lds + par * 2 * C::BN + C::BN), 16, (tn * C::BN + lane * 4) * 4, 0, 0, 0);
        }
#endif
    };
    auto stage0 = [&](int t, int pbuf) {
        const int tm = t / tiles_n, tn = t - tm * tiles_n;
        char* a = smem + pbuf * C::STAGE_BYTES;
        cp.b.prepare(w, ldb, tn * C::BN, N, wave, lane);
        cp.stage(0, a, wave);
    };
    copy_affine(tile, 0);
    pgemm::wait_vm<0>();
    pgemm::lds_barrier();
    int p = 0;
    ga.prepare((tile / tiles_n) * C::BM);
    stage0(tile, p);
    constexpr int YOUNGER = C::NH * C::NPASS + 2;
    bool prev_full = false;
    int parity = 0;
    for (; tile < ntiles; tile += G, parity ^= 1) {
        const int tile_m = tile / tiles_n, tile_n = tile - tile_m * tiles_n;
        const int m0 = tile_m * C::BM, n0 = tile_n * C::BN;
        const bool full = m0 + C::BM <= M;
        pgemm::Acc<C> acc;
        copy_affine(tile + G < ntiles ? tile + G : tile, parity ^ 1);
        pgemm::mainloop_sr<C, YOUNGER, true, pgemm::ConvPair<C, TAIL>>(cp, nt, smem, acc, p, prev_full, wave, lane);
        const int next = tile + G;
        if (next < ntiles) {
            ga.prepare((next / tiles_n) * C::BM);
            stage0(next, p);
        }
        char* stg = smem + (p ^ 1) * C::STAGE_BYTES;
        const int col = n0 + 8 * (tid % C::CPR);
        auto pre = [&](int, int j, int coff, float4_t v, int rl, int g) {
            const float* st = affine_lds + parity * 2 * C::BN + wn * (C::BN / C::WN) + j * 32 + coff;
            return bn16x4<ACT == 3>(v, *reinterpret_cast<const float4_t*>(st), *reinterpret_cast<const float4_t*>(st + C::BN));
        };
        const bool colok = !TAIL || col < N;
        if (full)
            pgemm::epilogue_f16<C, true>(acc, stg, [](int) {}, pre,
                                   [&](int r, int, int, half8_t h) { if (colok) st_half8(Cout + (size_t)(m0 + r) * N + col, h); });
        else
            pgemm::epilogue_f16<C, true>(acc, stg, [](int) {}, pre, [&](int r, int, int, half8_t h) {
                if (m0 + r < M && colok) st_half8(Cout + (size_t)(m0 + r) * N + col, h);
            });
        prev_full = full;
    }
}


template <bool KT = false>
__global__ __launch_bounds__(256, 2) void linear_generic_kernel(const half_t* __restrict__ A, int lda,
                                                                const half_t* __restrict__ B, int ldb, int M, int N,
                                                                int K, LinearEpi epi, int tiles_n) {
    using C = pgemm::CfgSmall;
    extern __shared__ __attribute__((aligned(16))) char smem[];
    const int swz = pgemm::xcd_remap(blockIdx.x, gridDim.x);
    const int tile_m = swz / tiles_n, tile_n = swz - tile_m * tiles_n;
    const int m0 = tile_m * C::BM, n0 = tile_n * C::BN;
    const int tid = threadIdx.x, wave = tid >> 6, wn = wave % C::WN;
    int p = 0;
    pgemm::stage_first<C, KT>(A, lda, B, ldb, M, N, m0, n0, smem, p, K);
    pgemm::Acc<C> acc;
    pgemm::mainloop<C, 0, true, KT, KT>(A, lda, B, ldb, M, N, K, m0, n0, smem, acc, p, false);
    const half_t* __restrict__ bias = epi.bias;
    const half_t* __restrict__ residual = epi.residual;
    const int act = epi.act, ldc = epi.ldc;
    const int col = n0 + 8 * (tid % C::CPR);
    pgemm::epilogue_f16<C, KT>(
        acc, smem + (p ^ 1) * C::STAGE_BYTES, [](int) {},
        [&](int, int j, int coff, float4_t v, int rl, int g) {
            const int n = n0 + wn * (C::BN / C::WN) + j * 32 + coff;
            half4_t h;
#pragma unroll
            for (int e = 0; e < 4; ++e) {
                float x = v[e];
                if (bias) x += (float)bias[n + e < N ? n + e : N - 1];
                x = r16(x);
                if (act == 1) x = quick_gelu16(x);
                if (act >= 2) {
                    const int nn = n + e < N ? n + e : N - 1;
                    x = r16(x * epi.scale[nn] + epi.shift[nn]);
                    if (act == 3) x = fmaxf(x, 0.f);
                }
                h[e] = (half_t)x;
            }
            return h;
        },
        [&](int r, int, int, half8_t h) {
            const int row = m0 + r;
            if (row >= M || col >= N) return;
            const size_t o = (size_t)row * ldc + col;
            for (int e = 0; e < 8 && col + e < N; ++e) {
                float x = (float)h[e];
                if (residual) x = (float)residual[o + e] + x;
                epi.C[o + e] = (half_t)x;
            }
        });
}

using CfgBig = pgemm::Cfg<256, 256, 2, 4>;
using CfgWide = pgemm::Cfg<256, 128, 4, 2>;
using CfgNarrow = pgemm::Cfg<256, 64, 4, 2>;
using CfgThin = pgemm::Cfg<256, 32, 4, 1>;
using CfgSmall = pgemm::CfgSmall;

struct TileOrder {
    int band, rev, band_n;
    bool descending(int K) const { return rev == 1 || (rev == 2 && K <= 1024); }
};
static TileOrder read_tile_order() {
    const char* b = getenv("PCLIP_GEMM_BAND");
    const char* r = getenv("PCLIP_GEMM_REV");
    const char* bn = getenv("PCLIP_GEMM_BAND_N");
    return TileOrder{b ? atoi(b) : 0, r ? atoi(r) : 2, bn ? atoi(bn) : 0};
}
static const TileOrder& tile_order() {
    static const bool live = getenv("PCLIP_GEMM_CFG_LIVE") != nullptr;
    static TileOrder order = read_tile_order();
    if (live) order = read_tile_order();
    return order;
}

struct Route {
    TileOrder order;
    int use4w;
    int* report;
    int cap;
    void note(int family, bool kt, int rows, int rev, int band) {
        const int i = report[0]++;
        if (i >= cap) return;
        int* r = report + 1 + PCLIP_ROUTE_FIELDS * i;
        r[0] = family; r[1] = kt; r[2] = rows; r[3] = rev; r[4] = band;
    }
};

template <class C, bool HAS_BIAS, int ACT, bool KT>
static int launch_fast2(const void* A, int lda, const void* B, int ldb, int M, int N, int K, const LinearEpi& epi,
                        int slots, hipStream_t s, Route* rt, int family) {
    static DevOnce attr;
    constexpr int LDS = C::LDS_BYTES + ((ACT == 2 || ACT == 3 || ACT == 5) ? 2 * 2 * C::BN * 4 : 2 * C::BN * 2) + 256;
    using CK = std::conditional_t<KT, pgemm::Tail<C>, C>;
    if (int e = pclip_raise_lds(attr, {(const void*)linear_fast_kernel<CK, HAS_BIAS, ACT>}, LDS, "pclip_gemm_f16")) return e;
    const int tiles_m = ceil_div(M, C::BM), tiles_n = KT ? ceil_div(N, C::BN) : N / C::BN, ntiles = tiles_m * tiles_n;
    const int grid = ntiles < slots ? ntiles : slots;
    const TileOrder& order = rt ? rt->order : tile_order();
    const int band = order.descending(K) ? -1 : (tiles_n >= 8 ? order.band : 0);
    if (rt) rt->note(family, KT, M, band < 0, band < 0 ? 0 : band);
    linear_fast_kernel<CK, HAS_BIAS, ACT><<<grid, C::NTHREADS, LDS, s>>>(
        (const half_t*)A, lda, (const half_t*)B, ldb, M, N, K, epi.bias, epi.scale, epi.shift, epi.C, epi.ldc, tiles_n, ntiles, epi.residual,
        band, pclip_gemm_time_slot());
    return pclip_check_launch("gemm_f16");
}

template <class C, bool KT = false>
static int launch_fast(const void* A, int lda, const void* B, int ldb, int M, int N, int K, const LinearEpi& epi,
                       int slots, hipStream_t s, Route* rt, int family) {
    if (epi.act == 2) return launch_fast2<C, false, 2, KT>(A, lda, B, ldb, M, N, K, epi, slots, s, rt, family);
    if (epi.act == 3) return launch_fast2<C, false, 3, KT>(A, lda, B, ldb, M, N, K, epi, slots, s, rt, family);
    if (epi.act == 5) return launch_fast2<C, false, 5, KT>(A, lda, B, ldb, M, N, K, epi, slots, s, rt, family);
    if (epi.act == 6) return launch_fast2<C, true, 6, KT>(A, lda, B, ldb, M, N, K, epi, slots, s, rt, family);
    if (epi.bias) {
        if (epi.act == 1) return launch_fast2<C, true, 1, KT>(A, lda, B, ldb, M, N, K, epi, slots, s, rt, family);
        return launch_fast2<C, true, 0, KT>(A, lda, B, ldb, M, N, K, epi, slots, s, rt, family);
    }
    if (epi.act == 1) return launch_fast2<C, false, 1, KT>(A, lda, B, ldb, M, N, K, epi, slots, s, rt, family);
    return launch_fast2<C, false, 0, KT>(A, lda, B, ldb, M, N, K, epi, slots, s, rt, family);
}
template <class C>
static int launch_fast_k(bool kt, const void* A, int lda, const void* B, int ldb, int M, int N, int K, const LinearEpi& epi, int slots, hipStream_t s, Route* rt, int family) {
    return kt ? launch_fast<C, true>(A, lda, B, ldb, M, N, K, epi, slots, s, rt, family) : launch_fast<C, false>(A, lda, B, ldb, M, N, K, epi, slots, s, rt, family);
}

}

#ifndef PCLIP_GEMM_4W_DEFAULT
#define PCLIP_GEMM_4W_DEFAULT 1
#endif
static long g_gemm_launches = 0;
static unsigned long long* g_time_buf = nullptr;
static int g_time_cap = 0, g_time_next = 0;
unsigned long long* pclip_gemm_time_slot() {
    if (!g_time_buf || g_time_next >= g_time_cap) return nullptr;
    return g_time_buf + 2 * (size_t)g_time_next++;
}
extern "C" int pclip_gemm_timing(void* buf, int nslots) {
    g_time_buf = (unsigned long long*)buf;
    g_time_cap = buf ? nslots : 0;
    g_time_next = 0;
    return PCLIP_OK;
}
extern "C" int pclip_gemm_timing_count(void) { return g_time_next; }
static int g_use4w = -1;
extern "C" int pclip_gemm4w_config(int mode) {
    const int before = g_use4w;
    if (mode >= 0) g_use4w = mode != 0;
    return before;
}
extern "C" long pclip_gemm_kernel_launches(void) { return g_gemm_launches; }

namespace {
struct TileCfg { int bm, bn, wg_per_cu; double eff; };
constexpr int kNumCfgs = 5;
constexpr TileCfg kTileCfgs[kNumCfgs] = {{128, 128, 2, 0.85}, {256, 128, 1, 0.85}, {256, 256, 1, 1.0}, {256, 64, 1, 0.6}, {256, 32, 2, 0.4}};
constexpr double kLaunchCost = 0.5;

inline long col_tiles(int N, int bn, bool ragged) { return ragged ? (N + bn - 1) / bn : N / bn; }
inline double tile_cost(const TileCfg& c, long M, int N, int cus, bool ragged = false) {
    if (!ragged && N % c.bn) return 1e30;
    const long slots = (long)c.wg_per_cu * cus, nt = ((M + c.bm - 1) / c.bm) * col_tiles(N, c.bn, ragged);
    const double share = nt <= cus ? 1.0 : (double)c.wg_per_cu;
    return (double)((nt + slots - 1) / slots) * (c.bm / 128.0) * (c.bn / 128.0) * share / c.eff;
}
inline int best_cfg(long M, int N, int cus, double* cost_out, bool ragged = false, unsigned allowed = ~0u) {
    int pick = -1;
    double best = 1e29;
    for (int i = 0; i < kNumCfgs; ++i) {
        if (!((allowed >> i) & 1)) continue;
        const double c = tile_cost(kTileCfgs[i], M, N, cus, ragged);
        if (c < best) { best = c; pick = i; }
    }
    if (cost_out) *cost_out = best;
    return pick;
}

bool small_applies(int M, int N, int cus, bool ragged = false);
bool small_enabled() {
    static const bool on = pclip_env_on("PCLIP_GEMM_SMALL");
    return on;
}
int launch_small_one(const half_t* A, int lda, const half_t* B, int ldb, int M, int N, int K, const LinearEpi& epi, hipStream_t s, bool kt = false, Route* rt = nullptr);

}
bool pclip_gemm4w_supports(int M, int N, int K, int lda, int ldb, int ldc, const void* C, const void* bias, const void* residual, int act);
int pclip_gemm4w_launch(const half_t* A, int lda, const half_t* B, int ldb, int M, int N, int K, const half_t* bias, half_t* C, int ldc, int act,
                        const half_t* residual, int slots, int rev, int band, hipStream_t s);
int pclip_gemm4w_launch_var(const half_t* A, int lda, const half_t* B, int ldb, int M, int N, int K, const half_t* bias, half_t* C, int ldc, int act,
                            const half_t* residual, int slots, int rev, int band, int var, hipStream_t s);
namespace {
int gemm_dispatch(const half_t* A, int lda, const half_t* B, int ldb, int M, int N, int K, LinearEpi epi, int cus, int forced,
                  bool may_split, hipStream_t s, Route* rt = nullptr) {
    const bool kt = K % pgemm::BK != 0;
    const bool aligned = (!epi.residual || ((epi.act == 5 || epi.act == 6) && ((uintptr_t)epi.residual & 15) == 0)) && epi.ldc % 8 == 0 && ((uintptr_t)epi.C & 15) == 0 &&
                         (!epi.bias || ((uintptr_t)epi.bias & 15) == 0) && (!kt || N % 8 == 0);
    const bool ring_ok = aligned && (epi.act <= 1 || epi.act == 6 || (((uintptr_t)epi.scale | (uintptr_t)epi.shift) & 15) == 0);
    if (ring_ok && forced == -1 && (rt || small_enabled()) && small_applies(M, N, cus, kt))
        return launch_small_one(A, lda, B, ldb, M, N, K, epi, s, kt, rt);
    if (forced == -3) {
        if (!ring_ok || !(kt || N % 64 == 0)) { pclip_set_error("pclip_gemm_route_f16: N=%d / alignment outside the ring kernel", N); return PCLIP_E_INVALID; }
        return launch_small_one(A, lda, B, ldb, M, N, K, epi, s, kt, rt);
    }
    double cost = 1e30;
    int pick = aligned ? best_cfg(M, N, cus, &cost, kt) : -1;
    if (forced == -2) { may_split = false; pick = -1; }
    if (epi.act == 5 && pick < 0) { pclip_set_error("pclip_gemm_bn_res_f16: N=%d / alignment not supported by the fused epilogue", N); return PCLIP_E_INVALID; }
    if (forced >= 0) {
        may_split = false;
        if (aligned && forced < kNumCfgs && (kt || N % kTileCfgs[forced].bn == 0)) pick = forced;
    }
    if (pick >= 0 && may_split) {
        long split_rows = 0;
        int split_cfg = -1;
        for (int i = 0; i < kNumCfgs; ++i) {
            const TileCfg& c = kTileCfgs[i];
            if (!kt && N % c.bn) continue;
            const long slots = (long)c.wg_per_cu * cus, tiles_n = col_tiles(N, c.bn, kt), nt = ((M + c.bm - 1) / c.bm) * tiles_n;
            const long full_rows = (nt / slots) * slots / tiles_n * c.bm;
            if (nt <= slots || nt % slots == 0 || full_rows >= M) continue;
            double rest = 1e30;
            best_cfg(M - full_rows, N, cus, &rest, kt);
            const double split = tile_cost(c, full_rows, N, cus, kt) + rest + kLaunchCost;
            if (split < cost) { cost = split; split_cfg = i; split_rows = full_rows; }
        }
        if (split_cfg >= 0) {
            int rc = gemm_dispatch(A, lda, B, ldb, (int)split_rows, N, K, epi, cus, split_cfg, false, s, rt);
            if (rc != PCLIP_OK) return rc;
            LinearEpi tail = epi;
            tail.C = epi.C + (size_t)split_rows * epi.ldc;
            if (epi.residual) tail.residual = epi.residual + (size_t)split_rows * epi.ldc;
            return gemm_dispatch(A + (size_t)split_rows * lda, lda, B, ldb, M - (int)split_rows, N, K, tail, cus, -1, true, s, rt);
        }
    }
    ++g_gemm_launches;
    if (pick < 0 && epi.act == 6) epi.act = 0;
    if (pick == 2) {
        if (!rt && g_use4w < 0) { const char* e = getenv("PCLIP_GEMM_4W"); g_use4w = e ? (atoi(e) != 0) : PCLIP_GEMM_4W_DEFAULT; }
        if ((rt ? rt->use4w : g_use4w) && pclip_gemm4w_supports(M, N, K, lda, ldb, epi.ldc, epi.C, epi.bias, epi.residual, epi.act)) {
            const TileOrder& order = rt ? rt->order : tile_order();
            const int rev = order.descending(K) ? 1 : 0, band = N / 256 >= 8 ? order.band : order.band_n;
            if (!rt) return pclip_gemm4w_launch(A, lda, B, ldb, M, N, K, epi.bias, epi.C, epi.ldc, epi.act, epi.residual, cus, rev, band, s);
            rt->note(PCLIP_ROUTE_RAN_FOUR_WAVE, false, M, rev, band);
            return pclip_gemm4w_launch_var(A, lda, B, ldb, M, N, K, epi.bias, epi.C, epi.ldc, epi.act, epi.residual, cus, rev, band, rt->use4w == 2 ? 1 : 0, s);
        }
        return launch_fast_k<CfgBig>(kt, A, lda, B, ldb, M, N, K, epi, cus, s, rt, 2);
    }
    if (pick == 1) return launch_fast_k<CfgWide>(kt, A, lda, B, ldb, M, N, K, epi, cus, s, rt, 1);
    if (pick == 0) return launch_fast_k<CfgSmall>(kt, A, lda, B, ldb, M, N, K, epi, 2 * cus, s, rt, 0);
    if (pick == 3) return launch_fast_k<CfgNarrow>(kt, A, lda, B, ldb, M, N, K, epi, cus, s, rt, 3);
    if (pick == 4) return launch_fast_k<CfgThin>(kt, A, lda, B, ldb, M, N, K, epi, 2 * cus, s, rt, 4);
    if (rt) rt->note(PCLIP_ROUTE_RAN_GENERIC, kt, M, 0, 0);
    const int tiles_m = ceil_div(M, 128), tiles_n = ceil_div(N, 128);
    if (kt)
        linear_generic_kernel<true><<<tiles_m * tiles_n, 256, CfgSmall::LDS_BYTES, s>>>(A, lda, B, ldb, M, N, K, epi, tiles_n);
    else
        linear_generic_kernel<false><<<tiles_m * tiles_n, 256, CfgSmall::LDS_BYTES, s>>>(A, lda, B, ldb, M, N, K, epi, tiles_n);
    return pclip_check_launch("gemm_f16 (generic)");
}
}

extern "C" int pclip_gemm_f16(const void* A, int lda, const void* B, int ldb, void* C, int ldc, int M, int N, int K,
                              const void* bias, int act, const void* residual, pclip_stream_t stream) {
    PCLIP_REQUIRE(A && B && C, "pclip_gemm_f16: null pointer");
    PCLIP_REQUIRE(M >= 0 && N > 0 && K > 0, "pclip_gemm_f16: bad shape M=%d N=%d K=%d", M, N, K);
    PCLIP_REQUIRE(K % 8 == 0, "pclip_gemm_f16: K=%d must be a multiple of 8", K);
    PCLIP_REQUIRE(lda >= K && ldb >= K && ldc >= N && lda % 8 == 0 && ldb % 8 == 0, "pclip_gemm_f16: bad leading dims");
    PCLIP_REQUIRE(act == 0 || act == 1, "pclip_gemm_f16: unknown activation %d", act);
    if (M == 0) return PCLIP_OK;
    LinearEpi epi{(const half_t*)bias, (const half_t*)residual, (half_t*)C, ldc, act, nullptr, nullptr};
    if (residual && bias && act == 0) epi.act = 6;
    const int cus = pclip_cus();
    static int forced = -1;
    static bool live = false, nosplit = false, init = false;
    if (!init || live) {
        init = true;
        const char* f = getenv("PCLIP_GEMM_CFG");
        forced = f ? atoi(f) : -1;
        if (forced == 3) forced = -2;
        else if (forced == 4) forced = 3;
        else if (forced >= 5) forced = -1;
        live = getenv("PCLIP_GEMM_CFG_LIVE") != nullptr;
        nosplit = getenv("PCLIP_GEMM_NOSPLIT") != nullptr;
    }
    return gemm_dispatch((const half_t*)A, lda, (const half_t*)B, ldb, M, N, K, epi, cus, forced, !nosplit, (hipStream_t)stream);
}

extern "C" int pclip_gemm_route_f16(const void* A, int lda, const void* B, int ldb, void* C, int ldc, int M, int N, int K, const void* bias, int act,
                                    const void* residual, const float* scale, const float* shift, int cfg, int may_split, int band, int band_n, int rev,
                                    int use4w, int cus, int* report, int report_len, pclip_stream_t stream) {
    PCLIP_REQUIRE(A && B && C && report, "pclip_gemm_route_f16: null pointer");
    PCLIP_REQUIRE(M >= 0 && N > 0 && K > 0, "pclip_gemm_route_f16: bad shape M=%d N=%d K=%d", M, N, K);
    PCLIP_REQUIRE(K % 8 == 0, "pclip_gemm_route_f16: K=%d must be a multiple of 8", K);
    PCLIP_REQUIRE(lda >= K && ldb >= K && ldc >= N && lda % 8 == 0 && ldb % 8 == 0, "pclip_gemm_route_f16: bad leading dims");
    PCLIP_REQUIRE(act == 0 || act == 1 || act == 2 || act == 3 || act == 5, "pclip_gemm_route_f16: unknown activation %d", act);
    PCLIP_REQUIRE(cfg >= PCLIP_ROUTE_AUTO && cfg <= PCLIP_ROUTE_RING, "pclip_gemm_route_f16: unknown configuration %d", cfg);
    PCLIP_REQUIRE(use4w >= 0 && use4w <= 2 && cus >= 1 && rev >= 0 && rev <= 2 && band >= 0 && band_n >= 0, "pclip_gemm_route_f16: bad route arguments");
    PCLIP_REQUIRE(report_len >= 1, "pclip_gemm_route_f16: the report needs room for the launch count");
    const bool affine = act >= 2;
    PCLIP_REQUIRE(!affine || (scale && shift && !bias), "pclip_gemm_route_f16: act %d takes scale and shift, no bias", act);
    PCLIP_REQUIRE(affine || (!scale && !shift), "pclip_gemm_route_f16: scale / shift without a BatchNorm epilogue");
    PCLIP_REQUIRE(act != 5 || (residual && N % 64 == 0 && (((uintptr_t)scale | (uintptr_t)shift) & 15) == 0), "pclip_gemm_route_f16: act 5 as pclip_gemm_bn_res_f16");
    PCLIP_REQUIRE(act == 5 || !affine || !residual, "pclip_gemm_route_f16: a residual with BatchNorm is act 5");
    PCLIP_REQUIRE(act != 1 || !residual, "pclip_gemm_route_f16: no residual behind QuickGELU");
    report[0] = 0;
    if (M == 0) return PCLIP_OK;
    LinearEpi epi{(const half_t*)bias, (const half_t*)residual, (half_t*)C, ldc, act, scale, shift};
    if (residual && bias && act == 0) epi.act = 6;
    int forced = cfg == PCLIP_ROUTE_GENERIC ? -2 : cfg == PCLIP_ROUTE_RING ? -3 : cfg;
    if ((act == 2 || act == 3) && !(N % 4 == 0 && (((uintptr_t)scale | (uintptr_t)shift) & 15) == 0)) forced = -2;
    Route rt{TileOrder{band, rev, band_n}, use4w, report, (report_len - 1) / PCLIP_ROUTE_FIELDS};
    return gemm_dispatch((const half_t*)A, lda, (const half_t*)B, ldb, M, N, K, epi, cus, forced, may_split != 0, (hipStream_t)stream, &rt);
}

namespace {
using CfgSplit = pgemm::Cfg<128, 64, 4, 2>;

constexpr int kSmallStages = 4;
constexpr int kSmallLds = kSmallStages * CfgSplit::STAGE_BYTES;

constexpr int ACT_KT = 0x100;
template <int ACT_FLAGS>
__global__ __launch_bounds__(CfgSplit::NTHREADS, 1) void linear_small_kernel(const half_t* __restrict__ A, int lda,
                                                                           const half_t* __restrict__ B, int ldb, int M, int N,
                                                                           int K, int tiles_n, int S, int steps_per,
                                                                           float* __restrict__ ws, const half_t* __restrict__ bias,
                                                                           half_t* Cout, int ldc,
                                                                           const float* __restrict__ scale,
                                                                           const float* __restrict__ shift,
                                                                           const half_t* residual = nullptr, unsigned long long* tslot = nullptr) {
    using C = CfgSplit;
    constexpr int ACT = ACT_FLAGS & 0xff;
    constexpr bool KT = (ACT_FLAGS & ACT_KT) != 0;
    extern __shared__ __attribute__((aligned(16))) char smem[];
    pgemm::time_begin(tslot);
    const int tile = blockIdx.x / S, ks = blockIdx.x - tile * S;
    const int tile_m = tile / tiles_n, tile_n = tile - tile_m * tiles_n;
    const int m0 = tile_m * C::BM, n0 = tile_n * C::BN;
    const int k0 = ks * steps_per * pgemm::BK;
    const int klen = (K - k0 < steps_per * pgemm::BK) ? K - k0 : steps_per * pgemm::BK;
    const int tid = threadIdx.x, lane = tid & 63, wave = tid >> 6, wm = wave / C::WN, wn = wave % C::WN;
    pgemm::Acc<C> acc;
    pgemm::mainloop_ring<C, kSmallStages, KT>(A + k0, lda, B + k0, ldb, M, N, KT ? (klen + pgemm::BK - 1) / pgemm::BK : klen / pgemm::BK, m0, n0, smem, acc, [&]() {
#pragma unroll
        for (int j = 0; j < C::TN; ++j)
#pragma unroll
            for (int g = 0; g < 4; ++g) {
                half4_t b = {(half_t)0.f, (half_t)0.f, (half_t)0.f, (half_t)0.f};
                if constexpr (KT) {
                    const int nb = n0 + wn * (C::BN / C::WN) + j * 32 + (g & 1) * 16 + 4 * (lane >> 4);
                    if (bias && nb < N) b = *reinterpret_cast<const half4_t*>(bias + nb);
                } else if (S == 1 && bias) b = *reinterpret_cast<const half4_t*>(bias + n0 + wn * (C::BN / C::WN) + j * 32 + (g & 1) * 16 + 4 * (lane >> 4));
#pragma unroll
                for (int e = 0; e < 4; ++e)
#pragma unroll
                    for (int i = 0; i < C::TM; ++i) acc.v[i][j][4 * g + e] = (float)b[e];
            }
    }, klen);
    if (S == 1) {
        const int col = n0 + 8 * (tid % C::CPR);
        auto pre = [&](int i, int j, int coff, float4_t v, int rl, int g) {
            if (ACT == 1) return quick_gelu16x4(v);
            if (ACT == 2 || ACT == 3 || ACT == 5) {
                const int n = n0 + wn * (C::BN / C::WN) + j * 32 + coff;
                const float4_t z4 = {0.f, 0.f, 0.f, 0.f};
                const float4_t sc = KT && n >= N ? z4 : *reinterpret_cast<const float4_t*>(scale + n), sh = KT && n >= N ? z4 : *reinterpret_cast<const float4_t*>(shift + n);
                return bn16x4<ACT == 3>(v, sc, sh);
            }
            return cvt16x4(v);
        };
        pgemm::epilogue_f16<C, true>(acc, smem, [](int) {}, pre, [&](int r, int c, int, half8_t h) {
            const bool valid = KT ? m0 + r < M && col < N : m0 + r < M;
            const size_t o = (size_t)(m0 + r) * ldc + col;
            if ((ACT == 5 || ACT == 6) && valid) h = add_residual16x8<ACT == 5>(ld_half8(residual + o), h);
            if (valid) st_half8(Cout + o, h);
        });
        pgemm::time_end(tslot);
        return;
    }
    float* slab = ws + (size_t)ks * M * N;
#pragma unroll
    for (int i = 0; i < C::TM; ++i)
#pragma unroll
        for (int j = 0; j < C::TN; ++j)
#pragma unroll
            for (int g = 0; g < 4; ++g) {
                const int m = m0 + wm * (C::BM / C::WM) + i * 32 + (g >> 1) * 16 + (lane & 15);
                const int n = n0 + wn * (C::BN / C::WN) + j * 32 + (g & 1) * 16 + 4 * (lane >> 4);
                if (m < M)
                    *reinterpret_cast<float4_t*>(slab + (size_t)m * N + n) =
                        float4_t{acc.v[i][j][4 * g], acc.v[i][j][4 * g + 1], acc.v[i][j][4 * g + 2], acc.v[i][j][4 * g + 3]};
            }
}

template <int ACT_FLAGS>
__global__ __launch_bounds__(CfgSplit::NTHREADS, 1) void conv3x3_small_kernel(const half_t* __restrict__ x,
                                                                            const half_t* __restrict__ w, int H, int W, int Cin, int M,
                                                                            int N, const float* __restrict__ scale,
                                                                            const float* __restrict__ shift, half_t* __restrict__ Cout,
                                                                            int tiles_n) {
    using C = CfgSplit;
    constexpr int ACT = ACT_FLAGS & 0xff;
    constexpr bool TAIL = (ACT_FLAGS & ACT_KT) != 0;
    extern __shared__ __attribute__((aligned(16))) char smem[];
    const int tile_m = blockIdx.x / tiles_n, tile_n = blockIdx.x - tile_m * tiles_n;
    const int m0 = tile_m * C::BM, n0 = tile_n * C::BN;
    const int nt = (9 * Cin + pgemm::BK - 1) / pgemm::BK, K = nt * pgemm::BK;
    const int tid = threadIdx.x, wave = tid >> 6, wn = wave % C::WN;
    pgemm::ConvGather<C, TAIL> ga(x, H, W, Cin, M);
    ga.prepare(m0);
    pgemm::Acc<C> acc;
    pgemm::mainloop_ring_g<C, kSmallStages>([&](int t, char* dst) { ga.stage(t, dst); }, w, K, N, nt, n0, smem, acc, [&]() {
#pragma unroll
        for (int i = 0; i < C::TM; ++i)
#pragma unroll
            for (int j = 0; j < C::TN; ++j)
#pragma unroll
                for (int e = 0; e < 16; ++e) acc.v[i][j][e] = 0.f;
    });
    const int col = n0 + 8 * (tid % C::CPR);
    auto pre = [&](int, int j, int coff, float4_t v, int rl, int g) {
        const int n = n0 + wn * (C::BN / C::WN) + j * 32 + coff;
        const float4_t z4 = {0.f, 0.f, 0.f, 0.f};
        const float4_t sc = TAIL && n >= N ? z4 : *reinterpret_cast<const float4_t*>(scale + n), sh = TAIL && n >= N ? z4 : *reinterpret_cast<const float4_t*>(shift + n);
        return bn16x4<ACT == 3>(v, sc, sh);
    };
    pgemm::epilogue_f16<C, true>(acc, smem, [](int) {}, pre, [&](int r, int, int, half8_t h) {
        if (TAIL ? m0 + r < M && col < N : m0 + r < M) st_half8(Cout + (size_t)(m0 + r) * N + col, h);
    });
}


template <int ACT>
__global__ __launch_bounds__(256) void splitk_reduce_kernel(const float* __restrict__ ws, int S, int M, int N,
                                                            const half_t* __restrict__ bias, half_t* __restrict__ Cout, int ldc) {
    const int cpr = N >> 3;
    const size_t idx = (size_t)blockIdx.x * 256 + threadIdx.x;
    if (idx >= (size_t)M * cpr) return;
    const int m = (int)(idx / cpr), n = (int)(idx - (size_t)m * cpr) * 8;
    const float* src = ws + (size_t)m * N + n;
    const size_t slab = (size_t)M * N;
    float4_t lo = {0.f, 0.f, 0.f, 0.f}, hi = lo;
#pragma unroll 8
    for (int s = 0; s < S; ++s) {
        lo += *reinterpret_cast<const float4_t*>(src + s * slab);
        hi += *reinterpret_cast<const float4_t*>(src + s * slab + 4);
    }
    if (bias) {
        const half8_t b = ld_half8(bias + n);
#pragma unroll
        for (int e = 0; e < 4; ++e) { lo[e] += (float)b[e]; hi[e] += (float)b[e + 4]; }
    }
    half4_t h0, h1;
    if (ACT == 1) { h0 = quick_gelu16x4(lo); h1 = quick_gelu16x4(hi); }
    else {
#pragma unroll
        for (int e = 0; e < 4; ++e) { h0[e] = (half_t)lo[e]; h1[e] = (half_t)hi[e]; }
    }
    st_half8(Cout + (size_t)m * ldc + n, half8_t{h0[0], h0[1], h0[2], h0[3], h1[0], h1[1], h1[2], h1[3]});
}

inline int small_attr() {
    static DevOnce done;
    return pclip_raise_lds(done,
                           {(const void*)linear_small_kernel<0>, (const void*)linear_small_kernel<1>, (const void*)linear_small_kernel<2>,
                            (const void*)linear_small_kernel<3>, (const void*)linear_small_kernel<5>, (const void*)linear_small_kernel<6>,
                            (const void*)linear_small_kernel<7>, (const void*)linear_small_kernel<8>, (const void*)linear_small_kernel<9>, (const void*)conv3x3_small_kernel<2>, (const void*)conv3x3_small_kernel<3>,
                            (const void*)linear_small_kernel<0 | ACT_KT>, (const void*)linear_small_kernel<1 | ACT_KT>, (const void*)linear_small_kernel<2 | ACT_KT>,
                            (const void*)linear_small_kernel<3 | ACT_KT>, (const void*)linear_small_kernel<5 | ACT_KT>, (const void*)linear_small_kernel<6 | ACT_KT>,
                            (const void*)conv3x3_small_kernel<2 | ACT_KT>, (const void*)conv3x3_small_kernel<3 | ACT_KT>},
                           kSmallLds, "gemm_f16 (small M)");
}

bool small_applies(int M, int N, int cus, bool ragged) {
    return M > 0 && (ragged || N % CfgSplit::BN == 0) && (long)ceil_div(M, CfgSplit::BM) * col_tiles(N, CfgSplit::BN, ragged) <= cus;
}

template <bool KT>
int launch_small_kt(const half_t* A, int lda, const half_t* B, int ldb, int M, int N, int K, const LinearEpi& epi, hipStream_t s, Route* rt) {
    if (int e = small_attr()) return e;
    if (rt) rt->note(PCLIP_ROUTE_RAN_RING, KT, M, 0, 0);
    constexpr int FLAGS = KT ? ACT_KT : 0;
    const int tiles_n = KT ? ceil_div(N, CfgSplit::BN) : N / CfgSplit::BN, grid = ceil_div(M, CfgSplit::BM) * tiles_n;
    const int steps = KT ? ceil_div(K, pgemm::BK) : K / pgemm::BK;
    ++g_gemm_launches;
    unsigned long long* tslot = pclip_gemm_time_slot();
#define PCLIP_SMALL_LAUNCH(ACT)                                                                                                                  \
    linear_small_kernel<ACT | FLAGS><<<grid, CfgSplit::NTHREADS, kSmallLds, s>>>(A, lda, B, ldb, M, N, K, tiles_n, 1, steps, nullptr, epi.bias, epi.C, \
                                                                                epi.ldc, epi.scale, epi.shift, epi.residual, tslot)
    if (epi.act == 5) PCLIP_SMALL_LAUNCH(5);
    else if (epi.act == 6) PCLIP_SMALL_LAUNCH(6);
    else if (epi.act == 1) PCLIP_SMALL_LAUNCH(1);
    else if (epi.act == 2) PCLIP_SMALL_LAUNCH(2);
    else if (epi.act == 3) PCLIP_SMALL_LAUNCH(3);
    else PCLIP_SMALL_LAUNCH(0);
#undef PCLIP_SMALL_LAUNCH
    return pclip_check_launch("gemm_f16 (small M)");
}
int launch_small_one(const half_t* A, int lda, const half_t* B, int ldb, int M, int N, int K, const LinearEpi& epi, hipStream_t s, bool kt, Route* rt) {
    return kt ? launch_small_kt<true>(A, lda, B, ldb, M, N, K, epi, s, rt) : launch_small_kt<false>(A, lda, B, ldb, M, N, K, epi, s, rt);
}

template <bool TAIL>
int launch_conv_small(const void* x, const void* w, int M, int H, int W, int Cin, int Cout, const float* scale, const float* shift, int relu, void* y, hipStream_t s) {
    if (int e = small_attr()) return e;
    constexpr int FLAGS = TAIL ? ACT_KT : 0;
    const int tiles_n = TAIL ? ceil_div(Cout, CfgSplit::BN) : Cout / CfgSplit::BN, grid = ceil_div(M, CfgSplit::BM) * tiles_n;
    if (relu)
        conv3x3_small_kernel<3 | FLAGS><<<grid, CfgSplit::NTHREADS, kSmallLds, s>>>((const half_t*)x, (const half_t*)w, H, W, Cin, M, Cout, scale, shift, (half_t*)y, tiles_n);
    else
        conv3x3_small_kernel<2 | FLAGS><<<grid, CfgSplit::NTHREADS, kSmallLds, s>>>((const half_t*)x, (const half_t*)w, H, W, Cin, M, Cout, scale, shift, (half_t*)y, tiles_n);
    return pclip_check_launch("conv3x3_bn (small M)");
}

struct SplitPlan { int tiles_m, tiles_n, S, steps_per; size_t bytes; };
inline SplitPlan splitk_plan(int M, int N, int K, int cus) {
    SplitPlan pl{0, 0, 0, 0, 0};
    if (M <= 0 || N <= 0 || K <= 0 || N % CfgSplit::BN || K % pgemm::BK) return pl;
    pl.tiles_m = ceil_div(M, CfgSplit::BM);
    pl.tiles_n = N / CfgSplit::BN;
    const int tiles = pl.tiles_m * pl.tiles_n, steps = K / pgemm::BK;
    if (steps < 8) return pl;
    pl.steps_per = steps / 8 > 2 ? steps / 8 : 2;
    pl.S = ceil_div(steps, pl.steps_per);
    pl.bytes = (size_t)pl.S * M * N * sizeof(float);
    static const int always = getenv("PCLIP_SPLITK_ALWAYS") ? atoi(getenv("PCLIP_SPLITK_ALWAYS")) : 0;
    const double t_one = 3.0 + 0.34 * steps, t_split = 4.5 + 0.34 * pl.steps_per + 2.0 * (double)pl.bytes / 3.0e6;
    if (tiles > cus || tiles * pl.S > 4 * cus || (!always && t_split + 0.5 > t_one)) { pl.S = 0; pl.bytes = 0; return pl; }
    return pl;
}

}

extern "C" size_t pclip_gemm_splitk_workspace(int M, int N, int K) {
    return splitk_plan(M, N, K, pclip_cus()).bytes;
}

extern "C" int pclip_gemm_splitk_f16(const void* A, int lda, const void* B, int ldb, void* C, int ldc, int M, int N, int K,
                                     const void* bias, int act, void* ws, size_t ws_bytes, pclip_stream_t stream) {
    PCLIP_REQUIRE(A && B && C && ws, "pclip_gemm_splitk_f16: null pointer");
    PCLIP_REQUIRE(act == 0 || act == 1, "pclip_gemm_splitk_f16: unknown activation %d", act);
    PCLIP_REQUIRE(lda >= K && ldb >= K && ldc >= N && lda % 8 == 0 && ldb % 8 == 0 && ldc % 8 == 0, "pclip_gemm_splitk_f16: bad leading dims");
    PCLIP_REQUIRE(((uintptr_t)A & 15) == 0 && ((uintptr_t)B & 15) == 0 && ((uintptr_t)C & 15) == 0 && (!bias || ((uintptr_t)bias & 15) == 0) &&
                      ((uintptr_t)ws & 15) == 0, "pclip_gemm_splitk_f16: operands must be 16-byte aligned");
    const SplitPlan pl = splitk_plan(M, N, K, pclip_cus());
    PCLIP_REQUIRE(pl.S >= 2, "pclip_gemm_splitk_f16: shape M=%d N=%d K=%d is not a split-K shape (pclip_gemm_splitk_workspace == 0)", M, N, K);
    if (ws_bytes < pl.bytes) { pclip_set_error("pclip_gemm_splitk_f16: workspace %zu < %zu", ws_bytes, pl.bytes); return PCLIP_E_WORKSPACE; }
    hipStream_t s = (hipStream_t)stream;
    if (int e = small_attr()) return e;
    linear_small_kernel<0><<<pl.tiles_m * pl.tiles_n * pl.S, CfgSplit::NTHREADS, kSmallLds, s>>>(
        (const half_t*)A, lda, (const half_t*)B, ldb, M, N, K, pl.tiles_n, pl.S, pl.steps_per, (float*)ws, nullptr, nullptr, 0, nullptr, nullptr);
    const int rgrid = (int)(((size_t)M * (N / 8) + 255) / 256);
    if (act == 1)
        splitk_reduce_kernel<1><<<rgrid, 256, 0, s>>>((const float*)ws, pl.S, M, N, (const half_t*)bias, (half_t*)C, ldc);
    else
        splitk_reduce_kernel<0><<<rgrid, 256, 0, s>>>((const float*)ws, pl.S, M, N, (const half_t*)bias, (half_t*)C, ldc);
    return pclip_check_launch("gemm_f16 (split-K)");
}

static int bn_forced_cfg() {
    static const int f = getenv("PCLIP_GEMM_BN_CFG") ? atoi(getenv("PCLIP_GEMM_BN_CFG")) : -1;
    return f;
}

extern "C" int pclip_gemm_bn_res_f16(const void* A, int lda, const void* B, int ldb, void* C, int ldc, int M, int N, int K,
                                     const float* scale, const float* shift, const void* residual, pclip_stream_t stream) {
    PCLIP_REQUIRE(A && B && C && scale && shift && residual, "pclip_gemm_bn_res_f16: null pointer");
    PCLIP_REQUIRE(M >= 0 && N > 0 && K > 0, "pclip_gemm_bn_res_f16: bad shape M=%d N=%d K=%d", M, N, K);
    PCLIP_REQUIRE(K % 8 == 0 && N % 64 == 0, "pclip_gemm_bn_res_f16: K=%d must be a multiple of 8 and N=%d a multiple of 64", K, N);
    PCLIP_REQUIRE(lda >= K && ldb >= K && ldc >= N && lda % 8 == 0 && ldb % 8 == 0, "pclip_gemm_bn_res_f16: bad leading dims");
    PCLIP_REQUIRE(((uintptr_t)scale & 15) == 0 && ((uintptr_t)shift & 15) == 0, "pclip_gemm_bn_res_f16: scale / shift must be 16-byte aligned");
    if (M == 0) return PCLIP_OK;
    LinearEpi epi{nullptr, (const half_t*)residual, (half_t*)C, ldc, 5, scale, shift};
    return gemm_dispatch((const half_t*)A, lda, (const half_t*)B, ldb, M, N, K, epi, pclip_cus(), bn_forced_cfg(), true, (hipStream_t)stream);
}

extern "C" int pclip_gemm_bn_f16(const void* A, int lda, const void* B, int ldb, void* C, int ldc, int M, int N, int K,
                                 const float* scale, const float* shift, int relu, pclip_stream_t stream) {
    PCLIP_REQUIRE(A && B && C && scale && shift, "pclip_gemm_bn_f16: null pointer");
    PCLIP_REQUIRE(M >= 0 && N > 0 && K > 0, "pclip_gemm_bn_f16: bad shape M=%d N=%d K=%d", M, N, K);
    PCLIP_REQUIRE(K % 8 == 0, "pclip_gemm_bn_f16: K=%d must be a multiple of 8", K);
    PCLIP_REQUIRE(lda >= K && ldb >= K && ldc >= N && lda % 8 == 0 && ldb % 8 == 0, "pclip_gemm_bn_f16: bad leading dims");
    if (M == 0) return PCLIP_OK;
    LinearEpi epi{nullptr, nullptr, (half_t*)C, ldc, relu ? 3 : 2, scale, shift};
    const bool strips_ok = N % 4 == 0 && ((uintptr_t)scale & 15) == 0 && ((uintptr_t)shift & 15) == 0;
    return gemm_dispatch((const half_t*)A, lda, (const half_t*)B, ldb, M, N, K, epi, pclip_cus(), strips_ok ? bn_forced_cfg() : -2, true, (hipStream_t)stream);
}

// ... 78 lines not shown
```

### proto-clip_amd/ops.py

```python
import contextvars
import ctypes
import math
import os

import numpy as np
import torch

from . import _lib
from ._lib import check, ptr, require_cuda, stream

_ws_cache = {}


def _workspace(nbytes: int, device) -> torch.Tensor:
    if torch.cuda.is_current_stream_capturing():
        return torch.empty(max(nbytes, 1 << 20), dtype=torch.uint8, device=device)
    key = (device, torch.cuda.current_stream(device).cuda_stream)
    buf = _ws_cache.get(key)
    if buf is None or buf.numel() < nbytes:
        buf = torch.empty(max(nbytes, 1 << 20), dtype=torch.uint8, device=device)
        _ws_cache[key] = buf
    return buf


# ... 441 lines not shown
        onehot, labels = torch.ones((), dtype=torch.bool, device=t.device), t.long()
    else:
        raise _lib.PclipError(f"tip_segments: expected one-hot cache_values [NK, N] or labels [NK], got shape {tuple(t.shape)}")
    NK = labels.shape[0]
    if NK:
        ordered = (labels[1:] >= labels[:-1]).all()
        facts = torch.stack([onehot.long(), ordered.long(), labels.min(), labels.max()]).cpu().tolist()
    else:
        facts = [1, 1, 0, 0]
    if not facts[0]:
        raise _lib.PclipError("tip_segments: cache_values is not one-hot (every row needs exactly one 1 among zeros; soft cache values are not supported)")
    if N is None:
        N = facts[3] + 1
    N = int(N)
    if N < 1 or facts[2] < 0 or facts[3] >= N:
        raise _lib.PclipError(f"tip_segments: labels span [{facts[2]}, {facts[3]}], outside [0, N={N})")
    if not facts[1]:
        raise _lib.PclipError("tip_segments: the cache rows are not sorted by class (build_cache_model sorts them; sort keys and values with the same permutation)")
    seg = torch.searchsorted(labels, torch.arange(N + 1, dtype=labels.dtype, device=t.device)).int()
    return seg, N


def tip_segments(cache_values_or_labels: torch.Tensor, N: int = None) -> torch.Tensor:
    require_cuda(cache_values_or_labels)
    return _tip_segment_table(cache_values_or_labels, N)[0]


def _tip_coef(what: str, name: str, v) -> float:
    if isinstance(v, torch.Tensor):
        if v.requires_grad:
            raise NotImplementedError(f"{what}: {name} requires grad — no gradient is produced for it (upstream trains only the cache keys)")
        v = v.item()
    v = float(np.float32(v))
    if not math.isfinite(v) or v < 0:
        raise _lib.PclipError(f"{what}: {name}={v} must be finite and >= 0")
    return v


def _tip_args(what, features, cache_keys, seg, clip_rows, layout, N=None):
    if layout not in (None, "dn", "nd"):
        raise _lib.PclipError(f"{what}: layout={layout!r}: expected 'dn' (cache_keys [D, NK], as build_cache_model returns), 'nd' ([NK, D] rows) or None")
    for name, t in (("features", features), ("cache_keys", cache_keys), ("clip weight rows", clip_rows)):
        if t is not None and (t.dtype != torch.float16 or t.dim() != 2):
            raise _lib.PclipError(f"{what}: {name} must be a 2-D float16 tensor, got {t.dtype} {tuple(t.shape)}")
    Q, D = features.shape
    if D % 64 or D < 64 or D > _lib.TIP_MAX_D:
        raise _lib.PclipError(f"{what}: D={D} must be a multiple of 64, <= {_lib.TIP_MAX_D}")
    if Q < 1:
        raise _lib.PclipError(f"{what}: no query rows")
    N = clip_rows.shape[0] if clip_rows is not None else int(N)
    if clip_rows is not None and clip_rows.shape[1] != D:
        raise _lib.PclipError(f"{what}: clip weight rows {tuple(clip_rows.shape)} are not [N, D={D}]")
    if N < 1 or N > _lib.TIP_MAX_CLASSES:
        raise _lib.PclipError(f"{what}: N={N} must be in [1, {_lib.TIP_MAX_CLASSES}] (the fused argmax's cap)")
    if layout is None:
        if D not in cache_keys.shape:
            raise _lib.PclipError(f"{what}: cache_keys {tuple(cache_keys.shape)} matches neither [D={D}, NK] nor [NK, D]")
        layout = "dn" if cache_keys.shape[0] == D else "nd"
    if cache_keys.shape[0 if layout == "dn" else 1] != D:
        raise _lib.PclipError(f"{what}: cache_keys {tuple(cache_keys.shape)} is not {'[D, NK]' if layout == 'dn' else '[NK, D]'} with D={D}")
    NK = cache_keys.shape[1 if layout == "dn" else 0]
    if seg.dtype != torch.int32 or seg.dim() != 1 or seg.shape[0] != N + 1 or not seg.is_contiguous():
        raise _lib.PclipError(f"{what}: seg must be a contiguous int32 tensor of N + 1 = {N + 1} entries (ops.tip_segments), got {seg.dtype} {tuple(seg.shape)}")
    require_cuda(features, cache_keys, seg, clip_rows)
    f = _f16_rows(features, f"{what}: features")
    w = _f16_rows(clip_rows, f"{what}: clip weight rows") if clip_rows is not None else None
    if NK == 0:
        keys = None
    else:
        keys = transpose(cache_keys) if layout == "dn" else _f16_rows(cache_keys, f"{what}: cache_keys")
    ldk = keys.stride(0) if NK > 1 else D
    return f, keys, seg, w, (f.stride(0) if Q > 1 else D), ldk, (w.stride(0) if w is not None and N > 1 else D), Q, NK, N, D


def tip_logits(features, cache_keys, seg, clip_rows, alpha, beta, scale: float = 100., want_logits: bool = True, want_f32: bool = False,
               want_argmax: bool = False, layout=None):
    what = "tip_logits"
    alpha, beta = _tip_coef(what, "alpha", alpha), _tip_coef(what, "beta", beta)
    if not (want_logits or want_f32 or want_argmax):
        raise _lib.PclipError(f"{what}: no output requested")
    f, keys, seg, w, ldf, ldk, ldw, Q, NK, N, D = _tip_args(what, features, cache_keys, seg, clip_rows, layout)
    dev = f.device
    ldl = (N + 7) // 8 * 8
    buf = torch.empty(Q, ldl, dtype=torch.float16, device=dev) if want_logits else None
    l32 = torch.empty(Q, N, dtype=torch.float32, device=dev) if want_f32 else None
    am = torch.empty(Q, dtype=torch.int32, device=dev) if want_argmax else None
    check(_lib.load().pclip_tip_logits_f16(ptr(f), ldf, Q, ptr(keys), ldk, NK, ptr(seg), ptr(w), ldw, N, D, float(np.float32(scale)), alpha, beta,
                                           ptr(buf), ldl, ptr(l32), ptr(am), stream()), "pclip_tip_logits_f16")
    return (buf[:, :N] if want_logits else None), l32, am


def tip_grid(features, cache_keys, seg, clip_rows, betas, alphas, labels, scale: float = 100., layout=None) -> torch.Tensor:
    what = "tip_grid"
    betas = [_tip_coef(what, f"betas[{i}]", b) for i, b in enumerate(betas)]
    alphas = [_tip_coef(what, f"alphas[{i}]", a) for i, a in enumerate(alphas)]
    if not betas or not alphas or len(alphas) > _lib.TIP_MAX_ALPHAS:
        raise _lib.PclipError(f"{what}: {len(betas)} betas x {len(alphas)} alphas: at least one of each, at most {_lib.TIP_MAX_ALPHAS} alphas")
    if labels.dtype not in (torch.int32, torch.int64) or labels.dim() != 1 or labels.shape[0] != features.shape[0]:
        raise _lib.PclipError(f"{what}: labels must be an int32 / int64 tensor of {features.shape[0]} entries")
    f, keys, seg, w, ldf, ldk, ldw, Q, NK, N, D = _tip_args(what, features, cache_keys, seg, clip_rows, layout)
    require_cuda(f, labels)
    dev = f.device
    lab = torch.where((labels >= 0) & (labels < N), labels, torch.full_like(labels, -1)).int().contiguous()
    bt = torch.tensor(betas, dtype=torch.float32).to(dev)
    at = torch.tensor(alphas, dtype=torch.float32).to(dev)
    correct = torch.empty(len(betas), len(alphas), dtype=torch.int32, device=dev)
    check(_lib.load().pclip_tip_grid_f16(ptr(f), ldf, Q, ptr(keys), ldk, NK, ptr(seg), ptr(w), ldw, N, D, float(np.float32(scale)), ptr(bt), len(betas),
                                         ptr(at), len(alphas), ptr(lab), ptr(correct), stream()), "pclip_tip_grid_f16")
    return correct


def tip_keys_backward(features, cache_keys, seg, dlogits, alpha, beta, layout=None, out: torch.Tensor = None) -> torch.Tensor:
    what = "tip_keys_backward"
    alpha, beta = _tip_coef(what, "alpha", alpha), _tip_coef(what, "beta", beta)
    if dlogits.dtype != torch.float32 or dlogits.dim() != 2 or dlogits.shape[0] != features.shape[0] or dlogits.shape[1] != seg.shape[0] - 1:
        raise _lib.PclipError(f"{what}: dlogits must be a float32 [Q={features.shape[0]}, N={seg.shape[0] - 1}] tensor, got {dlogits.dtype} {tuple(dlogits.shape)}")
    N = dlogits.shape[1]
    f, keys, seg, _, ldf, ldk, _, Q, NK, N, D = _tip_args(what, features, cache_keys, seg, None, layout, N=N)
    require_cuda(f, dlogits)
    dl = dlogits.contiguous()
    if out is None:
        dkeys = torch.empty(NK, D, dtype=torch.float32, device=f.device)
    else:
        if out.dtype != torch.float32 or tuple(out.shape) != (NK, D) or not out.is_contiguous() or not out.is_cuda or out.data_ptr() % 16:
            raise _lib.PclipError(f"{what}: out must be a contiguous, 16-byte aligned float32 [NK={NK}, D={D}] device tensor")
        dkeys = out
    nws = _lib.workspace_bytes(_lib.OP_TIP_BACKWARD, Q, NK, D)
    ws = _workspace(nws, f.device)
    check(_lib.load().pclip_tip_keys_backward_f16(ptr(f), ldf, Q, ptr(keys), ldk, NK, ptr(seg), N, D, alpha, beta, ptr(dl), ptr(dkeys), ptr(ws), nws, stream()),
          "pclip_tip_keys_backward_f16")
    return dkeys


CLASSIFY_ROUTES = ("two stages", "one launch, small N", "one launch, mid N", "fused row panels")


def classify_route(Q: int, N: int, D: int, alpha: float, beta: float, want_p=False, want_argmax=True, topk: int = 0, has_zt: bool = True) -> str:
    a32, oma32 = float(np.float32(alpha)), float(np.float32(1 - float(alpha)))
    r = _lib.load().pclip_classify_route_ex(Q, N, D, a32, oma32, float(np.float32(beta)), int(has_zt), int(bool(want_p)), int(bool(want_argmax)), topk,
                                            _classify_flags.get(), _lib.workspace_bytes(_lib.OP_CLASSIFY, Q, N, D))
    return CLASSIFY_ROUTES[r]


_classify_flags = contextvars.ContextVar("pclip_classify_flags", default=0)
_MID = _lib.CLASSIFY_NO_MID | _lib.CLASSIFY_FORCE_MID
_PANELS = _lib.CLASSIFY_NO_PANELS | _lib.CLASSIFY_FORCE_PANELS
_PASSES = _lib.CLASSIFY_PANEL_TWO_PASS | _lib.CLASSIFY_PANEL_FORCE_SECOND


class _classify_routing:
    mask = bits = 0

    def __enter__(self):
        self._token = _classify_flags.set(_classify_flags.get() & ~self.mask | self.bits)
        return self

    def __exit__(self, *exc):
        _classify_flags.reset(self._token)
        return False


class classify_mid(_classify_routing):
    def __init__(self, mode: int):
        self.mode = mode
        self.mask = _MID if mode >= 0 else 0
        self.bits = {0: _lib.CLASSIFY_NO_MID, 2: _lib.CLASSIFY_FORCE_MID}.get(mode, 0)


class classify_two_stage(_classify_routing):
    mask, bits = _MID | _PANELS, _lib.CLASSIFY_NO_MID | _lib.CLASSIFY_NO_PANELS


class classify_fused(_classify_routing):
    mask, bits = _MID | _PANELS, _lib.CLASSIFY_NO_MID | _lib.CLASSIFY_FORCE_PANELS


class classify_panel_passes(_classify_routing):
    def __init__(self, mode: int):
        self.mode = mode
        self.mask = _PASSES if mode >= 0 else 0
        self.bits = {1: _lib.CLASSIFY_PANEL_TWO_PASS, 2: _lib.CLASSIFY_PANEL_FORCE_SECOND}.get(mode, 0)


class classify_panel_exact(_classify_routing):
    def __init__(self, exact: bool = True):
        self.mask, self.bits = _lib.CLASSIFY_PANEL_EXACT, _lib.CLASSIFY_PANEL_EXACT if exact else 0


def classify_panel_stats(reset: bool = False, tiles: bool = False):
    import ctypes
    out = (ctypes.c_int * 3)()
    check(_lib.load().pclip_classify_panel_stats(ctypes.cast(out, ctypes.c_void_p), int(reset)), "pclip_classify_panel_stats")
    return (int(out[0]), int(out[1]), int(out[2])) if tiles else (int(out[0]), int(out[1]))


def classify_panel_distances(q, zi, zt, exact: bool = False):
    require_cuda(q, zi, zt)
    Q, D = q.shape
    N = zi.shape[0]
    dump = torch.empty(2, 256, 128, dtype=torch.float32, device=q.device)
    ws = _workspace(_lib.workspace_bytes(_lib.OP_CLASSIFY, max(Q, 4096), N, D), q.device)
    check(_lib.load().pclip_classify_panel_dump_f16(ptr(q), ptr(zi), ptr(zt), Q, N, D, ptr(dump), int(exact), ptr(ws), ws.numel(), stream()), "pclip_classify_panel_dump_f16")
    return dump[0], dump[1]


def hp_sweep(d2i, d2t, N: int, labels, alphas, betas) -> torch.Tensor:
    require_cuda(d2i, d2t, labels)
    Q, ldd = d2i.shape
    dev = d2i.device
    a = np.asarray(alphas, dtype=np.float64)
    a32 = torch.tensor(a.astype(np.float32), device=dev)
    oma32 = torch.tensor((1 - a).astype(np.float32), device=dev)
    b32 = torch.tensor(np.asarray(betas, dtype=np.float64).astype(np.float32), device=dev)
    labels = labels.to(torch.int32).contiguous()
    correct = torch.zeros(len(a), len(b32), dtype=torch.int32, device=dev)
    check(_lib.load().pclip_hp_sweep(ptr(d2i), ptr(d2t), ptr(labels), Q, N, ldd, ptr(a32), ptr(oma32), len(a),
                                     ptr(b32), len(b32), ptr(correct), stream()), "pclip_hp_sweep")
    return correct


def adapter_fc(x, w1, g1, b1, w2, g2, b2, ratio: float = 0.2, l2norm_out: bool = False, want_sq: bool = False):
    require_cuda(x, w1, w2)
    x = _f16c(x)
    B, D = x.shape
    H = w1.shape[0]
    y = torch.empty_like(x)
    sq = torch.empty(B, dtype=torch.float32, device=x.device) if want_sq else None
    ws = _workspace(_lib.workspace_bytes(_lib.OP_ADAPTER_FC, B, H, D), x.device)
    r32, omr32 = float(np.float32(ratio)), float(np.float32(1 - ratio))
    check(_lib.load().pclip_adapter_fc_f16(ptr(x), B, D, H, ptr(_f16c(w1)), ptr(_f16c(g1)), ptr(_f16c(b1)),
                                           ptr(_f16c(w2)), ptr(_f16c(g2)), ptr(_f16c(b2)), r32, omr32,
                                           int(l2norm_out), ptr(y), ptr(sq), ptr(ws), ws.numel(), stream()),
          "pclip_adapter_fc_f16")
    return (y, sq) if want_sq else y


def layernorm_blend(h, gamma, beta, x, ratio: float = 0.2, l2norm_out: bool = False, eps: float = 1e-5, want_sq: bool = False, out=None):
    require_cuda(h, gamma, beta, x)
    h, x = _f16c(h), _f16c(x)
    R, D = h.shape
    y = torch.empty_like(h) if out is None else out
    sq = torch.empty(R, dtype=torch.float32, device=h.device) if want_sq else None
    r32, omr32 = float(np.float32(ratio)), float(np.float32(1 - ratio))
    check(_lib.load().pclip_layernorm_blend_f16(ptr(h), ptr(_f16c(gamma)), ptr(_f16c(beta)), eps, ptr(x), r32, omr32, int(l2norm_out),
                                                ptr(y), ptr(sq), R, D, stream()), "pclip_layernorm_blend_f16")
    return (y, sq) if want_sq else y


ADAPTER_WIDTHS = (8, 16, 24, 32)


def _adapter_width(conv1):
    width = int(conv1.shape[0])
    if width not in ADAPTER_WIDTHS:
        raise _lib.PclipError(f"conv adapter width {width}: the gfx950 adapter kernels are built for widths {ADAPTER_WIDTHS}")
    return width


def adapter_conv(x, three_x: bool, conv1, ln1w, ln1b, conv2, ln2w, ln2b, conv3, ln3w, ln3b,
                 l2norm_out: bool = False, want_sq: bool = False):
    require_cuda(x, conv1)
    x = _f16c(x)
    B, D = x.shape
    width = _adapter_width(conv1)
    y = torch.empty_like(x)
    sq = torch.empty(B, dtype=torch.float32, device=x.device) if want_sq else None
    f = lambda t: None if t is None else ptr(_f16c(t))
    check(_lib.load().pclip_adapter_conv_w_f16(ptr(x), B, D, int(three_x), width, f(conv1), f(ln1w), f(ln1b), f(conv2),
                                               f(ln2w), f(ln2b), f(conv3), f(ln3w), f(ln3b), int(l2norm_out), ptr(y),
                                               ptr(sq), stream()), "pclip_adapter_conv_w_f16")
    return (y, sq) if want_sq else y



def gemm(a, w, bias=None, act: int = 0, residual=None, out=None):
    require_cuda(a, w)
    M, K = a.shape
    N = w.shape[0]
    if out is None:
        out = torch.empty(M, N, dtype=torch.float16, device=a.device)
    lib = _lib.load()
    if residual is None and M <= _SPLITK_MAX_M and _SPLITK:
        need = lib.pclip_gemm_splitk_workspace(M, N, K)
        if need and a.stride(0) % 8 == 0 and w.stride(0) % 8 == 0 and out.stride(0) % 8 == 0 and \
                not ((a.data_ptr() | w.data_ptr() | out.data_ptr()) & 15) and (bias is None or not (bias.data_ptr() & 15)):
            ws = _workspace(need, a.device)
            check(lib.pclip_gemm_splitk_f16(ptr(a), a.stride(0), ptr(w), w.stride(0), ptr(out), out.stride(0), M, N, K, ptr(bias), act,
                                            ptr(ws), ws.numel(), stream()), "pclip_gemm_splitk_f16")
            return out
    check(lib.pclip_gemm_f16(ptr(a), a.stride(0), ptr(w), w.stride(0), ptr(out), out.stride(0), M, N, K,
                             ptr(bias), act, ptr(residual), stream()), "pclip_gemm_f16")
    return out


def gemm4w(a, w, bias=None, act: int = 0, residual=None, out=None, var: int = 0):
    require_cuda(a, w)
    M, K = a.shape
    N = w.shape[0]
    if out is None:
        out = torch.empty(M, N, dtype=torch.float16, device=a.device)
    check(_lib.load().pclip_gemm4w_var_f16(ptr(a), a.stride(0), ptr(w), w.stride(0), ptr(out), out.stride(0), M, N, K, ptr(bias), act, ptr(residual), var,
                                           stream()), "pclip_gemm4w_f16")
    return out


ROUTE_AUTO, ROUTE_GENERIC, ROUTE_RING = _lib.ROUTE_AUTO, _lib.ROUTE_GENERIC, _lib.ROUTE_RING


def gemm_route(a, w, bias=None, act: int = 0, residual=None, scale=None, shift=None, out=None, cfg: int = ROUTE_AUTO, may_split: bool = True,
               band: int = 0, band_n: int = 0, rev: int = 2, use4w: int = 1, cus: int = 0):
    require_cuda(a, w, bias, residual, scale, shift, out)
    M, K = a.shape
    N = w.shape[0]
    if out is None:
        out = torch.empty(M, N, dtype=torch.float16, device=a.device)
    lib = _lib.load()
    fields, cap = _lib.ROUTE_FIELDS, 8
    report = (ctypes.c_int * (1 + fields * cap))()
    check(lib.pclip_gemm_route_f16(ptr(a), a.stride(0), ptr(w), w.stride(0), ptr(out), out.stride(0), M, N, K, ptr(bias), act, ptr(residual), ptr(scale), ptr(shift),
                                   cfg, int(may_split), band, band_n, rev, use4w, cus or lib.pclip_device_cus(), report, len(report), stream()), "pclip_gemm_route_f16")
    if report[0] > cap:
        raise _lib.PclipError(f"pclip_gemm_route_f16: {report[0]} launches, the report holds {cap}")
    launches = []
    for i in range(report[0]):
        family, kt, rows, rv, bd = report[1 + fields * i:1 + fields * (i + 1)]
        launches.append(dict(family=_lib.ROUTE_RAN[family], kt=bool(kt), rows=rows, rev=bool(rv), band=bd))
    return out, launches


class gemm_eight_wave:
    def __enter__(self):
        self.before = _lib.load().pclip_gemm4w_config(0)
        return self

    def __exit__(self, *exc):
        _lib.load().pclip_gemm4w_config(1 if self.before != 0 else 0)
        return False


_SPLITK = os.environ.get("PCLIP_GEMM_SPLITK", "0") == "1"
_SPLITK_MAX_M = 4096


def splitk_active(M: int) -> bool:
    return _SPLITK and M <= _SPLITK_MAX_M


class low_latency:

    def __init__(self, enabled: bool = True):
        self.enabled = enabled

    def __enter__(self):
        global _SPLITK
        self.prev, _SPLITK = _SPLITK, self.enabled
        return self

    def __exit__(self, *exc):
        global _SPLITK
        _SPLITK = self.prev
        return False


def gemm_bn(a, w, scale, shift, relu: bool = True, out=None):
    require_cuda(a, w, scale, shift)
    a, w = _f16c(a), _f16c(w)
    M, K = a.shape
    N = w.shape[0]
    if out is None:
        out = torch.empty(M, N, dtype=torch.float16, device=a.device)
    check(_lib.load().pclip_gemm_bn_f16(ptr(a), K, ptr(w), w.shape[1], ptr(out), N, M, N, K, ptr(scale), ptr(shift), int(relu),
                                        stream()), "pclip_gemm_bn_f16")
    return out


def gemm_bn_res_relu(a, w, scale, shift, residual, out=None):
    require_cuda(a, w, scale, shift, residual)
    a, w, residual = _f16c(a), _f16c(w), _f16c(residual)
    M, K = a.shape
    N = w.shape[0]
    if out is None:
        out = torch.empty(M, N, dtype=torch.float16, device=a.device)
    if N % 64 == 0 and K % 8 == 0 and not ((a.data_ptr() | w.data_ptr() | out.data_ptr() | residual.data_ptr() | scale.data_ptr() | shift.data_ptr()) & 15):
        check(_lib.load().pclip_gemm_bn_res_f16(ptr(a), K, ptr(w), w.shape[1], ptr(out), N, M, N, K, ptr(scale), ptr(shift), ptr(residual),
                                                stream()), "pclip_gemm_bn_res_f16")
        return out
    gemm(a, w, out=out)
    return bn_act(out, scale, shift, residual=residual, relu=True, out=out)


_zero_line = {}


def conv3x3_bn(x, w, scale, shift, B: int, H: int, W: int, Cin: int, relu: bool = True):
    require_cuda(x, w, scale, shift)
    x, w = _f16c(x), _f16c(w)
    Cout = w.shape[0]
    if w.shape[1] != (9 * Cin + 63) // 64 * 64 or x.numel() != B * H * W * Cin:
        raise _lib.PclipError("conv3x3_bn: shape mismatch")
    z = _zero_line.get(x.device)
    if z is None:
        z = _zero_line[x.device] = torch.zeros(64, dtype=torch.float16, device=x.device)
    y = torch.empty(B * H * W, Cout, dtype=torch.float16, device=x.device)
    check(_lib.load().pclip_conv3x3_bn_f16(ptr(x), ptr(w), ptr(z), B, H, W, Cin, Cout, ptr(scale), ptr(shift), int(relu), ptr(y),
                                           stream()), "pclip_conv3x3_bn_f16")
    return y


class conv_strip:
    def __init__(self, on: bool):
        self.mode = int(bool(on))

    def __enter__(self):
        self.before = _lib.load().pclip_conv3x3_strip_config(self.mode)
        return self

    def __exit__(self, *exc):
        _lib.load().pclip_conv3x3_strip_config(self.before)
        return False


def conv_strip_applies(B: int, H: int, W: int, Cin: int, Cout: int) -> bool:
    return bool(_lib.load().pclip_conv3x3_strip_applies(B, H, W, Cin, Cout))


def conv3x3_pool_applies(H: int, W: int, Cin: int, Cout: int) -> bool:
    return bool(_lib.load().pclip_conv3x3_pool_applies(H, W, Cin, Cout))


def conv3x3_bn_pool(x, w, scale, shift, B: int, H: int, W: int, Cin: int):
    require_cuda(x, w, scale, shift)
    x, w = _f16c(x), _f16c(w)
    Cout = w.shape[0]
    if w.shape[1] != (9 * Cin + 63) // 64 * 64 or x.numel() != B * H * W * Cin:
        raise _lib.PclipError("conv3x3_bn_pool: shape mismatch")
    y = torch.empty(B * (H // 2) * (W // 2), Cout, dtype=torch.float16, device=x.device)
    check(_lib.load().pclip_conv3x3_bn_pool_f16(ptr(x), ptr(w), B, H, W, Cin, Cout, ptr(scale), ptr(shift), ptr(y), stream()), "pclip_conv3x3_bn_pool_f16")
    return y


def stem_conv_applies(R: int, Cout: int) -> bool:
    return bool(_lib.load().pclip_stem_conv_applies(R, Cout))


def stem_conv_bn(img, w, scale, shift, relu: bool = True):
    require_cuda(img, w, scale, shift)
    if img.dim() != 4 or img.shape[1] != 3 or img.shape[2] != img.shape[3] or img.dtype not in (torch.float32, torch.float16) or w.shape[1] != 64:
        raise _lib.PclipError("stem_conv_bn: images [B, 3, R, R] fp32 / fp16 and w [Cout, 64] expected")
    img, w = img.contiguous(), _f16c(w)
    B, R, Cout = img.shape[0], img.shape[2], w.shape[0]
    Ho = (R - 1) // 2 + 1
    y = torch.empty(B * Ho * Ho, Cout, dtype=torch.float16, device=img.device)
    check(_lib.load().pclip_stem_conv_bn_f16(ptr(img), int(img.dtype == torch.float32), B, R, ptr(w), Cout, ptr(scale), ptr(shift), int(relu), ptr(y), stream()),
          "pclip_stem_conv_bn_f16")
    return y


def layernorm(x, gamma, beta, eps: float = 1e-5, out=None, rows: int = None, ld: int = None):
    require_cuda(x, gamma, beta)
    D = x.shape[-1]
    R = x.numel() // D if rows is None else rows
    ld = D if ld is None else ld
    if out is None:
        out = torch.empty(R, D, dtype=torch.float16, device=x.device)
    check(_lib.load().pclip_layernorm_f16(ptr(x), ld, ptr(gamma), ptr(beta), eps, ptr(out), R, D, stream()),
          "pclip_layernorm_f16")
    return out


def add_layernorm(x, delta, gamma, beta, eps: float = 1e-5, out=None, update_x: bool = True, rows: int = None,
                  ld: int = None):
    require_cuda(x, delta, gamma, beta)
    D = x.shape[-1]
    R = x.numel() // D if rows is None else rows
    ld = D if ld is None else ld
    if out is None:
        out = torch.empty(R, D, dtype=torch.float16, device=x.device)
    check(_lib.load().pclip_add_layernorm_f16(ptr(x), ptr(delta), ld, ptr(x) if update_x else None, ptr(gamma), ptr(beta),
                                              eps, ptr(out), R, D, stream()), "pclip_add_layernorm_f16")
    return out


ATT_SHORT_MAX_L = 288


def attention(qkv, B: int, L: int, H: int, causal: bool = False, out=None):
    require_cuda(qkv)
    W = H * 64
    if out is None:
        out = torch.empty(B * L, W, dtype=torch.float16, device=qkv.device)
    if L > ATT_SHORT_MAX_L:
        check(_lib.load().pclip_attention_long_q_f16(ptr(qkv), 3 * W, L * 3 * W, ptr(qkv), 3 * W, W, 2 * W, ptr(out), B, L, L, H, 64,
                                                     int(causal), stream()), "pclip_attention_long_q_f16")
        return out
    check(_lib.load().pclip_attention_f16(ptr(qkv), ptr(out), B, L, H, 64, int(causal), stream()),
          "pclip_attention_f16")
    return out


def attention_first_queries(q, kv, B: int, L: int, Lq: int, H: int):
    require_cuda(q, kv)
    W = H * 64
    out = torch.empty(B * Lq, W, dtype=torch.float16, device=q.device)
    fn = "pclip_attention_long_q_f16" if L > ATT_SHORT_MAX_L else "pclip_attention_q_f16"
    check(getattr(_lib.load(), fn)(ptr(q), W, Lq * W, ptr(kv), 2 * W, 0, W, ptr(out), B, L, Lq, H, 64, 0, stream()), fn)
    return out


def cast_f16(x: torch.Tensor) -> torch.Tensor:
    require_cuda(x)
    x = x.contiguous()
    y = torch.empty(x.shape, dtype=torch.float16, device=x.device)
    check(_lib.load().pclip_cast_f32_f16(ptr(x), ptr(y), x.numel(), stream()), "pclip_cast_f32_f16")
    return y


def im2col_patches(img: torch.Tensor, P: int) -> torch.Tensor:
    require_cuda(img)
    B, C, R, _ = img.shape
    G = R // P
    ld = (3 * P * P + 63) // 64 * 64
    cols = torch.empty(B * G * G, ld, dtype=torch.float16, device=img.device)
    if img.dtype == torch.float32:
        check(_lib.load().pclip_im2col_patches_f32(ptr(img), B, R, P, ptr(cols), ld, stream()), "pclip_im2col_patches_f32")
        return cols
    check(_lib.load().pclip_im2col_patches_f16(ptr(img), B, R, P, ptr(cols), ld, stream()),
          "pclip_im2col_patches_f16")
    return cols


def vit_assemble_tokens(patch_emb, class_emb, pos_emb, B: int, G2: int, W: int) -> torch.Tensor:
    tokens = torch.empty(B * (G2 + 1), W, dtype=torch.float16, device=patch_emb.device)
    check(_lib.load().pclip_vit_assemble_tokens_f16(ptr(patch_emb), ptr(class_emb), ptr(pos_emb), B, G2, W,
                                                    ptr(tokens), stream()), "pclip_vit_assemble_tokens_f16")
    return tokens


def vit_embed_ln(patch_emb, class_emb, pos_emb, B: int, G2: int, W: int, g_pre, b_pre, g_1, b_1, eps: float = 1e-5):
    R = B * (G2 + 1)
    x0 = torch.empty(R, W, dtype=torch.float16, device=patch_emb.device)
    f = lambda t: t if t is None or t.dtype == torch.float32 else t.float()
    g_pre, b_pre, g_1, b_1 = f(g_pre), f(b_pre), f(g_1), f(b_1)
    h = torch.empty_like(x0)
    check(_lib.load().pclip_vit_embed_ln_f16(ptr(patch_emb), ptr(class_emb), ptr(pos_emb), B, G2, W, ptr(g_pre), ptr(b_pre), ptr(g_1),
                                             ptr(b_1), eps, ptr(x0), ptr(h), stream()), "pclip_vit_embed_ln_f16")
    return x0, h


def text_embed(tokens, tok_emb, pos_emb) -> torch.Tensor:
    require_cuda(tokens, tok_emb)
    B, L = tokens.shape
    vocab, W = tok_emb.shape
    tokens = tokens.to(torch.int64).contiguous()
    x = torch.empty(B * L, W, dtype=torch.float16, device=tok_emb.device)
    check(_lib.load().pclip_text_embed_f16(ptr(tokens), ptr(tok_emb), ptr(pos_emb), B, L, W, vocab, ptr(x),
                                           stream()), "pclip_text_embed_f16")
    return x


EMBED_BWD_CHUNK = _lib.EMBED_BWD_CHUNK
EMBED_BWD_MAX_L, EMBED_BWD_MAX_W = 4096, 2048


def _embed_bwd_envelope(what: str, B: int, L: int, W: int):
    if not (B >= 1 and 1 <= L <= EMBED_BWD_MAX_L and W >= 64 and W % 64 == 0 and W <= EMBED_BWD_MAX_W):
        raise _lib.PclipError(f"{what}: B={B} L={L} W={W} outside the envelope (B >= 1, 1 <= L <= {EMBED_BWD_MAX_L}, W % 64 == 0, W <= {EMBED_BWD_MAX_W})")


def text_embed_backward(dx, tokens, vocab: int, want_emb: bool = True, want_pos: bool = True):
    require_cuda(dx, tokens)
    dx = _f16c(dx)
    if tokens.dim() != 2 or tokens.dtype != torch.int64:
        raise _lib.PclipError(f"text_embed_backward: tokens must be int64 [B, L], got {tokens.dtype} {tuple(tokens.shape)}")
    B, L = tokens.shape
    W = dx.shape[-1]
    _embed_bwd_envelope("text_embed_backward", B, L, W)
    if dx.dim() != 2 or dx.shape[0] != B * L:
        raise _lib.PclipError(f"text_embed_backward: dx {tuple(dx.shape)} does not hold B * L = {B * L} rows")
    if vocab < 1:
        raise _lib.PclipError(f"text_embed_backward: vocab={vocab}")
    if not (want_emb or want_pos):
        return None, None
    dE = ids = order = part = None
    if want_emb:
        ids, order = torch.sort(tokens.reshape(-1).clamp(0, vocab - 1), stable=True)
        dE = torch.empty(vocab, W, dtype=torch.float32, device=dx.device)
        part = torch.empty((B * L + EMBED_BWD_CHUNK - 1) // EMBED_BWD_CHUNK, 2, W, dtype=torch.float32, device=dx.device)
    dpos = torch.empty(L, W, dtype=torch.float32, device=dx.device) if want_pos else None
    check(_lib.load().pclip_text_embed_backward(ptr(dx), ptr(ids), ptr(order), B, L, W, vocab, ptr(dE), ptr(dpos), ptr(part), stream()),
          "pclip_text_embed_backward")
    return dE, dpos


def vit_embed_backward(dt, B: int, L: int, want_pos: bool = True, want_patch: bool = True):
    require_cuda(dt)
    dt = _f16c(dt)
    W = dt.shape[-1]
    _embed_bwd_envelope("vit_embed_backward", B, L, W)
    if dt.numel() != B * L * W:
        raise _lib.PclipError(f"vit_embed_backward: dt {tuple(dt.shape)} does not hold B * L = {B * L} rows")
    if not (want_pos or want_patch):
        return None, None
    dpos = torch.empty(L, W, dtype=torch.float32, device=dt.device) if want_pos else None
    dpatch = torch.empty(B * (L - 1), W, dtype=torch.float16, device=dt.device) if want_patch else None
    if dpos is None and L == 1:
        return None, dpatch
# ... 600 lines not shown
```

### proto-clip_amd/tower.py

```python
import torch

from . import ops
from ._lib import PclipError


def _block_params(blk):
    attn, mlp, ln_1, ln_2 = blk.attn, blk.mlp, blk.ln_1, blk.ln_2
    out, fc, pr = attn.out_proj, mlp.c_fc, mlp.c_proj
    return [ln_1.weight, ln_1.bias, attn.in_proj_weight, attn.in_proj_bias, out.weight, out.bias, ln_2.weight, ln_2.bias, fc.weight, fc.bias,
            pr.weight, pr.bias]


def residual_block(x, h, params, B, L, heads, causal, pick=None, first_token=False, splitk=False, rec=None):
    ln1w, ln1b, win, bin_, wout, bout, ln2w, ln2b, wfc, bfc, wpr, bpr = params
    if rec is not None:
        rec.update(x_in=x.clone(), h1=h, picked=pick is not None)
    if pick is not None and first_token and not causal:
        W = x.shape[1]
        kv = ops.gemm(h, win[W:3 * W], bin_[W:3 * W])
        q = ops.gemm(pick(h), win[0:W], bin_[0:W])
        a, x = ops.attention_first_queries(q, kv, B, L, 1, heads), pick(x)
        if rec is not None:
            rec.update(q=q, kv=kv)
    else:
        qkv = ops.gemm(h, win, bin_)
        a = ops.attention(qkv, B, L, heads, causal=causal)
        if rec is not None:
            rec.update(qkv=qkv)
        if pick is not None:
            a, x = pick(a), pick(x)
    if splitk and ops.splitk_active(a.shape[0]):
        h = ops.add_layernorm(x, ops.gemm(a, wout, bout), ln2w, ln2b)
    else:
        ops.gemm(a, wout, bout, residual=x, out=x)
        h = ops.layernorm(x, ln2w, ln2b)
    if rec is not None:
        rec.update(a=a, x_mid=x.clone(), h2=h)
    f = ops.gemm(h, wfc, bfc, act=1)
    if rec is not None:
        rec.update(f=f)
    if splitk and ops.splitk_active(f.shape[0]):
        return x, ops.gemm(f, wpr, bpr)
    ops.gemm(f, wpr, bpr, residual=x, out=x)
    return x, None


def _run_blocks(x, blocks, B, L, heads, causal, select=None, first_token=False, h0=None):
    params = [_block_params(blk) for blk in blocks]
    n, d = len(params), None
    if n > 0:
        h = h0 if h0 is not None else ops.layernorm(x, params[0][0], params[0][1])
    for i in range(n):
        last = i == n - 1
        x, d = residual_block(x, h, params[i], B, L, heads, causal, select if last else None, first_token, splitk=True)
        if not last:
            lnw, lnb = params[i + 1][0], params[i + 1][1]
            h = ops.layernorm(x, lnw, lnb) if d is None else ops.add_layernorm(x, d, lnw, lnb)
    if select is not None and n == 0:
        x = select(x)
    return x, d


def eot_positions(tokens: torch.Tensor) -> torch.Tensor:
    L = tokens.shape[1]
    pos = torch.arange(L, device=tokens.device).expand(tokens.shape[0], L)
    return torch.where(tokens == tokens.max(dim=-1, keepdim=True).values, pos, pos.new_full((), L)).min(dim=-1).values


def class_row_pick(B, L, device, tokens=None):
    return (lambda t: t.view(B, L, -1)[:, 0, :].contiguous()), (lambda: torch.arange(B, device=device) * L)


def eot_row_pick(B, L, device, tokens):
    return (lambda t: ops.gather_eot(t, tokens, B, L, t.shape[1])), (lambda: torch.arange(B, device=device) * L + eot_positions(tokens))


class Tower:

    def __init__(self, entry, name, stem_word, *, blocks, heads, causal, ln, proj, cache, projT_key, prefix, head, pick):
        self.entry, self.name, self.stem_word = entry, name, stem_word
        self.blocks, self.heads, self.causal, self.ln, self.proj, self.cache, self.projT_key = blocks, heads, causal, ln, proj, cache, projT_key
        self.prefix, self.head, self.pick, self.first_token = prefix, head, pick, not causal
        self.stem_opt_in = False

    def tape_from(self, prefix=None):
        for name, p in self.prefix if prefix is None else prefix:
            if p.requires_grad:
                raise PclipError(f"{self.name}: parameter {name} requires grad but lies in the frozen prefix of the tower (only a tail of residual "
                                 "blocks, the final LayerNorm and the projection are differentiable)")
        for i, blk in enumerate(self.blocks):
            if any(p.requires_grad for p in blk.parameters()):
                return i
        return len(self.blocks) if any(p.requires_grad for _, p in self.head) else None

    def tape_plan(self):
        if not self.stem_opt_in:
            return self.tape_from(), False
        if any(p.requires_grad for _, p in self.prefix):
            for name, p in self.prefix:
                if p.requires_grad and p.dtype not in (torch.float16, torch.float32):
                    raise PclipError(f"{self.name}: unsupported dtype {p.dtype} of parameter {name}")
            return 0, True
        return self.tape_from(prefix=[]), False

    def what(self, first, stem):
        n = len(self.blocks)
        if stem:
            return f"{self.entry} ({self.name}, {self.stem_word} + blocks 0..{n - 1} + heads on the tape)"
        return f"{self.entry} ({self.name}, blocks {first}..{n - 1} + heads trainable)"


def run_tower(tw, x, B, L, plan, pick, what=None, h0=None, deep=None, deep_off=None):
    first, stem = plan
    select, _ = pick
    if first is None:
        x, d = _run_blocks(x, tw.blocks, B, L, tw.heads, tw.causal, select=select, first_token=tw.first_token, h0=h0)
        if d is None:
            y = ops.layernorm(x, tw.ln.weight, tw.ln.bias)
        else:
            y = ops.add_layernorm(x, d, tw.ln.weight, tw.ln.bias, update_x=False)
        return ops.gemm(y, tw.cache.get(tw.projT_key, tw.proj, lambda t: t.t().contiguous()))
    from .autograd import run_tower_tail
    what = tw.what(first, stem) if what is None else what
    if first == len(tw.blocks) and not x.requires_grad:
        with torch.no_grad():
            x, _ = _run_blocks(x, tw.blocks, B, L, tw.heads, tw.causal, select=select, first_token=tw.first_token, h0=h0)
        return run_tower_tail(tw, x, None, first, B, L, (None, None), what)
    if first > 0:
        with torch.no_grad():
            x, _ = _run_blocks(x, tw.blocks[:first], B, L, tw.heads, tw.causal, h0=h0)
        h0 = None
    return run_tower_tail(tw, x, h0, first, B, L, pick, what, deep=deep, deep_off=deep_off)


def _pad_patch_weight(w):
    kp = w.shape[1] * w.shape[2] * w.shape[3]
    kpad = (kp + 63) // 64 * 64
    w2 = w.reshape(w.shape[0], kp)
    if kpad != kp:
        w2 = torch.cat([w2, w2.new_zeros(w.shape[0], kpad - kp)], dim=1)
    return w2.contiguous()


def vit_stem(cache, img, wconv, cls, pos, P, fused=None):
    B, W = img.shape[0], wconv.shape[0]
    G2 = (img.shape[2] // P) ** 2
    w16 = cache.get("conv1", wconv, _pad_patch_weight)
    cls16 = cache.get("cls", cls, lambda t: t.half())
    pos16 = cache.get("pos", pos, lambda t: t.half().contiguous())
    patch = ops.gemm(ops.im2col_patches(img, P), w16 if w16.dtype == torch.float16 else w16.half())
    if fused is not None:
        return ops.vit_embed_ln(patch, cls16, pos16, B, G2, W, *fused)
    return ops.vit_assemble_tokens(patch, cls16, pos16, B, G2, W)
```

Before: 29090 query images/sec.

## Write QKV projection in 16x32 blocked layout and read it blocked in attention

```diff
diff --git a/include/pclip.h b/include/pclip.h
--- a/include/pclip.h
+++ b/include/pclip.h
@@ -167,6 +167,9 @@
                          const void* bias, int act, const void* residual, const float* scale, const float* shift,
                          int cfg, int may_split, int band, int band_n, int rev, int use4w, int cus,
                          int* report, int report_len, pclip_stream_t stream);
+int pclip_gemm_blocked_f16(const void* A, int lda, const void* B, const void* Bperm, int ldb, void* C, int M, int N, int K,
+                           const void* bias, const void* bias_perm, int var, pclip_stream_t stream);
+
 int pclip_gemm4w_stamp_buffer(void* stamps);
 int pclip_gemm4w_config(int mode);
 
@@ -205,6 +208,9 @@
 
 int pclip_attention_q_f16(const void* q, int ldq, long q_batch_stride, const void* kv, int ldkv, int k_off, int v_off, void* out,
                           int B, int L, int Lq, int H, int dh, int causal, pclip_stream_t stream);
+
+int pclip_attention_blocked_f16(const void* q, int ldq, long q_batch_stride, int q_blocked, const void* kv, int nkv, int k_off, int v_off, void* out,
+                                int B, int L, int Lq, int H, int dh, pclip_stream_t stream);
 
 int pclip_attention_long_q_f16(const void* q, int ldq, long q_batch_stride, const void* kv, int ldkv, int k_off, int v_off, void* out,
                                int B, int L, int Lq, int H, int dh, int causal, pclip_stream_t stream);
diff --git a/proto-clip_amd/_lib.py b/proto-clip_amd/_lib.py
--- a/proto-clip_amd/_lib.py
+++ b/proto-clip_amd/_lib.py
@@ -81,6 +81,7 @@
     "pclip_gemm4w_var_f16": [_P, c_int, _P, c_int, _P, c_int, c_int, c_int, c_int, _P, c_int, _P, c_int, _P],
     "pclip_gemm_route_f16": [_P, c_int, _P, c_int, _P, c_int, c_int, c_int, c_int, _P, c_int, _P, _P, _P, c_int, c_int, c_int, c_int, c_int, c_int, c_int,
                              _P, c_int, _P],
+    "pclip_gemm_blocked_f16": [_P, c_int, _P, _P, c_int, _P, c_int, c_int, c_int, _P, _P, c_int, _P],
     "pclip_gemm4w_stamp_buffer": [_P],
     "pclip_gemm4w_config": [c_int],
     "pclip_gemm_splitk_workspace": [c_int, c_int, c_int],
@@ -98,6 +99,7 @@
     "pclip_add_layernorm_f16": [_P, _P, c_int, _P, _P, _P, c_float, _P, c_int, c_int, _P],
     "pclip_attention_f16": [_P, _P, c_int, c_int, c_int, c_int, c_int, _P],
     "pclip_attention_q_f16": [_P, c_int, c_long, _P, c_int, c_int, c_int, _P, c_int, c_int, c_int, c_int, c_int, c_int, _P],
+    "pclip_attention_blocked_f16": [_P, c_int, c_long, c_int, _P, c_int, c_int, c_int, _P, c_int, c_int, c_int, c_int, c_int, _P],
     "pclip_attention_long_q_f16": [_P, c_int, c_long, _P, c_int, c_int, c_int, _P, c_int, c_int, c_int, c_int, c_int, c_int, _P],
     "pclip_attention_config": [c_int, c_int],
     "pclip_im2col_patches_f16": [_P, c_int, c_int, c_int, _P, c_int, _P],
diff --git a/proto-clip_amd/csrc/pclip_attention.hip b/proto-clip_amd/csrc/pclip_attention.hip
--- a/proto-clip_amd/csrc/pclip_attention.hip
+++ b/proto-clip_amd/csrc/pclip_attention.hip
@@ -1,15 +1,16 @@
 #include "pclip_attention_tile.h"
+#include "pclip_blocked.h"
 #include <stdlib.h>
 #include <type_traits>
 
 namespace {
 constexpr int ATT_MAX_L = 288;
 
-template <int NW, int VAR, bool QF = false>
+template <int NW, int VAR, bool QF = false, bool BLK = false>
 __global__ __launch_bounds__(NW * 64, NW / 2) void attention_kernel(const half_t* __restrict__ qp, int ldq, long q_batch,
                                                            const half_t* __restrict__ kvp, int ldkv, int k_off, int v_off,
                                                            half_t* __restrict__ out, int L, int Lq, int H, int causal, int NT,
-                                                           int ) {
+                                                           int q_blocked ) {
     extern __shared__ __attribute__((aligned(16))) char smem[];
     const int LP = NT * 32;
     half_t* Ks = reinterpret_cast<half_t*>(smem);
@@ -20,25 +21,35 @@
     const half_t* vbase = kvp + (size_t)b * L * ldkv + h * ATT_DH + v_off;
     const half_t* qbase = qp + (size_t)b * q_batch + h * ATT_DH;
     const int tid = threadIdx.x, lane = tid & 63, wave = tid >> 6;
+    auto kv_blocked = [&](int col_off, int r, int c8) { return kvp + pblk::off((long)b * L + r, col_off + h * ATT_DH + c8, ldkv); };
+    auto q_blocked_at = [&](int r, int c8) { return qp + pblk::off((long)b * L + r, h * ATT_DH + c8, ldq); };
     half8_t qf0[4];
     if (QF) {
         const int q0 = wave * 32 + (lane & 31), qc0 = q0 < Lq ? q0 : Lq - 1;
 #pragma unroll
-        for (int s_ = 0; s_ < 4; ++s_) qf0[s_] = ld_half8(qbase + (size_t)qc0 * ldq + s_ * 16 + (lane >> 5) * 8);
+        for (int s_ = 0; s_ < 4; ++s_) {
+            const half_t* src = qbase + (size_t)qc0 * ldq + s_ * 16 + (lane >> 5) * 8;
+            if constexpr (BLK) { if (q_blocked) src = q_blocked_at(qc0, s_ * 16 + (lane >> 5) * 8); }
+            qf0[s_] = ld_half8(src);
+        }
     }
 
     for (int r0 = wave * 8; r0 < LP; r0 += NW * 8) {
         const int r = r0 + (lane >> 3);
         const int c = (lane & 7) ^ pgemm::swz_key(r);
         const int rc = r < L ? r : L - 1;
-        __builtin_amdgcn_global_load_lds((pgemm::gbl_ptr_t)(kbase + (size_t)rc * ldkv + c * 8),
+        const half_t* src = kbase + (size_t)rc * ldkv + c * 8;
+        if constexpr (BLK) src = kv_blocked(k_off, rc, c * 8);
+        __builtin_amdgcn_global_load_lds((pgemm::gbl_ptr_t)src,
                                          (pgemm::lds_ptr_t)(Ks + r0 * ATT_DH), 16, 0, 0);
     }
     for (int r0 = wave * 8; r0 < LP; r0 += NW * 8) {
         const int r = r0 + (lane >> 3);
         const int c = (lane & 7) ^ (((r >> 1) & 1) << 2);
         const int rc = r < L ? r : L - 1;
-        __builtin_amdgcn_global_load_lds((pgemm::gbl_ptr_t)(vbase + (size_t)rc * ldkv + c * 8),
+        const half_t* src = vbase + (size_t)rc * ldkv + c * 8;
+        if constexpr (BLK) src = kv_blocked(v_off, rc, c * 8);
+        __builtin_amdgcn_global_load_lds((pgemm::gbl_ptr_t)src,
                                          (pgemm::lds_ptr_t)(Vs + r0 * ATT_DH), 16, 0, 0);
     }
 #ifndef PCLIP_ATT_VBAR
@@ -73,7 +84,11 @@
         const int qc = q < Lq ? q : Lq - 1;
         half8_t qf[4];
 #pragma unroll
-        for (int s = 0; s < 4; ++s) qf[s] = ld_half8(qbase + (size_t)qc * ldq + s * 16 + hi * 8);
+        for (int s = 0; s < 4; ++s) {
+            const half_t* src = qbase + (size_t)qc * ldq + s * 16 + hi * 8;
+            if constexpr (BLK) { if (q_blocked) src = q_blocked_at(qc, s * 16 + hi * 8); }
+            qf[s] = ld_half8(src);
+        }
         process(qb, qf);
     }
 }
@@ -188,22 +203,15 @@
     return PCLIP_OK;
 }
 
-extern "C" int pclip_attention_q_f16(const void* q, int ldq, long q_batch_stride, const void* kv, int ldkv, int k_off, int v_off,
-                                     void* out, int B, int L, int Lq, int H, int dh, int causal, pclip_stream_t stream) {
-    PCLIP_REQUIRE(q && kv && out, "pclip_attention_q_f16: null pointer");
-    PCLIP_REQUIRE(dh == ATT_DH, "pclip_attention_q_f16: head dim %d unsupported (must be 64)", dh);
-    PCLIP_REQUIRE(B >= 0 && H > 0 && L > 0 && L <= ATT_MAX_L && Lq > 0 && Lq <= L, "pclip_attention_q_f16: bad B=%d H=%d L=%d Lq=%d (L <= %d)",
-                  B, H, L, Lq, ATT_MAX_L);
-    PCLIP_REQUIRE(!causal || Lq == L, "pclip_attention_q_f16: the causal mask needs all queries (Lq == L)");
-    PCLIP_REQUIRE(ldq % 8 == 0 && ldkv % 8 == 0 && k_off % 8 == 0 && v_off % 8 == 0 && q_batch_stride % 8 == 0,
-                  "pclip_attention_q_f16: strides / offsets must be multiples of 8 halves");
-    if (B == 0) return PCLIP_OK;
+template <bool BLK>
+static int attention_run(const void* q, int ldq, long q_batch_stride, const void* kv, int ldkv, int k_off, int v_off, void* out, int B, int L, int Lq, int H,
+                         int causal, int q_blocked, pclip_stream_t stream) {
     const int NT = ceil_div(L, 32), LP = NT * 32;
     const long nitems = (long)B * H;
     const int cus = pclip_device_cus();
     const int KR = (L + 7) / 8 * 8;
     const size_t plds = (2 * (size_t)(KR + LP) + KR) * ATT_DH * 2;
-    if (Lq == L && g_att_mode != 0 && NT <= 8 && plds <= 160 * 1024 && cus > 0 && g_att_mode == 1) {
+    if (!BLK && Lq == L && g_att_mode != 0 && NT <= 8 && plds <= 160 * 1024 && cus > 0 && g_att_mode == 1) {
         static DevOnce pipe_attr;
         if (int e = pclip_raise_lds(pipe_attr, {(const void*)attention_pipe_kernel<4, 2, PCLIP_ATT_VAR_SHORT>, (const void*)attention_pipe_kernel<8, 2, PCLIP_ATT_VAR_LONG>},
                                     160 * 1024, "pclip_attention_f16"))
@@ -223,26 +231,54 @@
     }
     const size_t lds = 2 * (size_t)LP * ATT_DH * 2;
     static DevOnce attr_set;
-    if (int e = pclip_raise_lds(attr_set, {(const void*)attention_kernel<8, PCLIP_ATT_VAR_LONG>, (const void*)attention_kernel<4, PCLIP_ATT_VAR_LONG>,
-                                           (const void*)attention_kernel<4, PCLIP_ATT_VAR_SHORT>, (const void*)attention_kernel<8, PCLIP_ATT_VAR_LONG, true>,
-                                           (const void*)attention_kernel<4, PCLIP_ATT_VAR_SHORT, true>},
+    if (int e = pclip_raise_lds(attr_set, {(const void*)attention_kernel<8, PCLIP_ATT_VAR_LONG, false, BLK>, (const void*)attention_kernel<4, PCLIP_ATT_VAR_LONG, false, BLK>,
+                                           (const void*)attention_kernel<4, PCLIP_ATT_VAR_SHORT, false, BLK>, (const void*)attention_kernel<8, PCLIP_ATT_VAR_LONG, true, BLK>,
+                                           (const void*)attention_kernel<4, PCLIP_ATT_VAR_SHORT, true, BLK>},
                                 80 * 1024, "pclip_attention_f16"))
         return e;
 #define PCLIP_ATT_LAUNCH(NW, VAR)                                                                                                         \
-    attention_kernel<NW, VAR><<<B * H, NW * 64, lds, (hipStream_t)stream>>>((const half_t*)q, ldq, q_batch_stride, (const half_t*)kv, ldkv, k_off, \
-                                                                             v_off, (half_t*)out, L, Lq, H, causal, NT, 0)
+    attention_kernel<NW, VAR, false, BLK><<<B * H, NW * 64, lds, (hipStream_t)stream>>>((const half_t*)q, ldq, q_batch_stride, (const half_t*)kv, ldkv, k_off, \
+                                                                             v_off, (half_t*)out, L, Lq, H, causal, NT, q_blocked)
     static const bool qfirst = pclip_env_on("PCLIP_ATT_QFIRST");
     if (PCLIP_ATT_QF4 && qfirst && NT <= 4 && Lq == L && !causal)
-        attention_kernel<4, PCLIP_ATT_VAR_SHORT, true><<<B * H, 4 * 64, lds, (hipStream_t)stream>>>((const half_t*)q, ldq, q_batch_stride, (const half_t*)kv, ldkv, k_off,
-                                                                                                     v_off, (half_t*)out, L, Lq, H, causal, NT, 0);
+        attention_kernel<4, PCLIP_ATT_VAR_SHORT, true, BLK><<<B * H, 4 * 64, lds, (hipStream_t)stream>>>((const half_t*)q, ldq, q_batch_stride, (const half_t*)kv, ldkv, k_off,
+                                                                                                     v_off, (half_t*)out, L, Lq, H, causal, NT, q_blocked);
     else if ((Lq + 31) / 32 > 4 && (Lq + 31) / 32 <= 8 && NT <= 8 && qfirst)
-        attention_kernel<8, PCLIP_ATT_VAR_LONG, true><<<B * H, 8 * 64, lds, (hipStream_t)stream>>>((const half_t*)q, ldq, q_batch_stride, (const half_t*)kv, ldkv, k_off,
-                                                                                                    v_off, (half_t*)out, L, Lq, H, causal, NT, 0);
+        attention_kernel<8, PCLIP_ATT_VAR_LONG, true, BLK><<<B * H, 8 * 64, lds, (hipStream_t)stream>>>((const half_t*)q, ldq, q_batch_stride, (const half_t*)kv, ldkv, k_off,
+                                                                                                    v_off, (half_t*)out, L, Lq, H, causal, NT, q_blocked);
     else if ((Lq + 31) / 32 > 4) PCLIP_ATT_LAUNCH(8, PCLIP_ATT_VAR_LONG);
     else if (NT > 4) PCLIP_ATT_LAUNCH(4, PCLIP_ATT_VAR_LONG);
     else PCLIP_ATT_LAUNCH(4, PCLIP_ATT_VAR_SHORT);
 #undef PCLIP_ATT_LAUNCH
     return pclip_check_launch("attention");
+}
+
+extern "C" int pclip_attention_q_f16(const void* q, int ldq, long q_batch_stride, const void* kv, int ldkv, int k_off, int v_off,
+                                     void* out, int B, int L, int Lq, int H, int dh, int causal, pclip_stream_t stream) {
+    PCLIP_REQUIRE(q && kv && out, "pclip_attention_q_f16: null pointer");
+    PCLIP_REQUIRE(dh == ATT_DH, "pclip_attention_q_f16: head dim %d unsupported (must be 64)", dh);
+    PCLIP_REQUIRE(B >= 0 && H > 0 && L > 0 && L <= ATT_MAX_L && Lq > 0 && Lq <= L, "pclip_attention_q_f16: bad B=%d H=%d L=%d Lq=%d (L <= %d)",
+                  B, H, L, Lq, ATT_MAX_L);
+    PCLIP_REQUIRE(!causal || Lq == L, "pclip_attention_q_f16: the causal mask needs all queries (Lq == L)");
+    PCLIP_REQUIRE(ldq % 8 == 0 && ldkv % 8 == 0 && k_off % 8 == 0 && v_off % 8 == 0 && q_batch_stride % 8 == 0,
+                  "pclip_attention_q_f16: strides / offsets must be multiples of 8 halves");
+    if (B == 0) return PCLIP_OK;
+    return attention_run<false>(q, ldq, q_batch_stride, kv, ldkv, k_off, v_off, out, B, L, Lq, H, causal, 0, stream);
+}
+
+extern "C" int pclip_attention_blocked_f16(const void* q, int ldq, long q_batch_stride, int q_blocked, const void* kv, int nkv, int k_off, int v_off,
+                                           void* out, int B, int L, int Lq, int H, int dh, pclip_stream_t stream) {
+    PCLIP_REQUIRE(q && kv && out, "pclip_attention_blocked_f16: null pointer");
+    PCLIP_REQUIRE(dh == ATT_DH, "pclip_attention_blocked_f16: head dim %d unsupported (must be 64)", dh);
+    PCLIP_REQUIRE(B >= 0 && H > 0 && L > 0 && L <= ATT_MAX_L && Lq > 0 && Lq <= L, "pclip_attention_blocked_f16: bad B=%d H=%d L=%d Lq=%d (L <= %d)",
+                  B, H, L, Lq, ATT_MAX_L);
+    PCLIP_REQUIRE(nkv % pblk::COLS == 0 && k_off % 8 == 0 && v_off % 8 == 0 && k_off >= 0 && v_off >= 0 && k_off + H * ATT_DH <= nkv && v_off + H * ATT_DH <= nkv,
+                  "pclip_attention_blocked_f16: kv needs N %% 32 == 0 and H heads at k_off / v_off inside it (N=%d)", nkv);
+    PCLIP_REQUIRE(q_blocked == 0 || q_blocked == 1, "pclip_attention_blocked_f16: q_blocked is 0 or 1");
+    PCLIP_REQUIRE(q_blocked ? (Lq == L && ldq % pblk::COLS == 0 && H * ATT_DH <= ldq) : (ldq % 8 == 0 && q_batch_stride % 8 == 0),
+                  "pclip_attention_blocked_f16: blocked queries are rows of a [B*L, ldq] blocked tensor (Lq == L, ldq %% 32 == 0); row-major ones need strides in multiples of 8 halves");
+    if (B == 0) return PCLIP_OK;
+    return attention_run<true>(q, ldq, q_batch_stride, kv, nkv, k_off, v_off, out, B, L, Lq, H, 0, q_blocked, stream);
 }
 
 extern "C" int pclip_attention_f16(const void* qkv, void* out, int B, int L, int H, int dh, int causal,
diff --git a/proto-clip_amd/csrc/pclip_blocked.h b/proto-clip_amd/csrc/pclip_blocked.h
--- /dev/null
+++ b/proto-clip_amd/csrc/pclip_blocked.h
@@ -0,0 +1,10 @@
+#pragma once
+#include <stddef.h>
+
+namespace pblk {
+constexpr int ROWS = 16, COLS = 32, BLOCK = ROWS * COLS;
+__host__ __device__ __forceinline__ size_t off(long r, int c, int N) {
+    return ((size_t)(r >> 4) * (size_t)(N >> 5) + (size_t)(c >> 5)) * BLOCK + (size_t)((r & 15) * COLS + (c & 31));
+}
+__host__ __device__ __forceinline__ long padded_rows(long M) { return (M + ROWS - 1) / ROWS * ROWS; }
+}
diff --git a/proto-clip_amd/csrc/pclip_gemm4w.hip b/proto-clip_amd/csrc/pclip_gemm4w.hip
--- a/proto-clip_amd/csrc/pclip_gemm4w.hip
+++ b/proto-clip_amd/csrc/pclip_gemm4w.hip
@@ -1,5 +1,6 @@
 #include "pclip_gemm.h"
 #include "pclip_epilogue.h"
+#include "pclip_blocked.h"
 #include "pclip_gemm4w_loop.inc"
 #include <stdlib.h>
 
@@ -207,6 +208,35 @@
             n0 = n0n;
             continue;
         }
+        if constexpr (ACT == 7) {
+            const int lane = fresh_tid(wave) & 63;
+            const int bvoff = (lane & 15) * (pblk::COLS * 2) + (lane >> 4) * 16;
+            const int nb = N >> 5, g0 = m0 >> 4;
+            const long bbytes = ((long)((M + 15) / 16 - g0) * nb - (n0 >> 5)) * (pblk::BLOCK * 2);
+            pgemm::rsrc_t rb;
+#if defined(__HIP_DEVICE_COMPILE__)
+            {
+                const uint64_t a = (uint64_t)(Cout + ((size_t)g0 * nb + (n0 >> 5)) * pblk::BLOCK);
+                const uint32_t lo = __builtin_amdgcn_readfirstlane((uint32_t)a), hi = __builtin_amdgcn_readfirstlane((uint32_t)(a >> 32));
+                rb = __builtin_amdgcn_make_buffer_rsrc((void*)(((uint64_t)hi << 32) | lo), 0, __builtin_amdgcn_readfirstlane((int)(bbytes < 0x7fffffffL ? bbytes : 0x7fffffffL)), 0x00020000);
+            }
+#endif
+            const int sbase = (((wave >> 1) * 8) * nb + (wave & 1) * 4) * (pblk::BLOCK * 2);
+#pragma unroll
+            for (int i = 0; i < 8; ++i)
+#pragma unroll
+                for (int jj = 0; jj < 4; ++jj) {
+                    const half4_t lo = cvt16x4(acc.q[i][2 * jj]), hi = cvt16x4(acc.q[i][2 * jj + 1]);
+                    const half8_t h{lo[0], lo[1], lo[2], lo[3], hi[0], hi[1], hi[2], hi[3]};
+#if defined(__HIP_DEVICE_COMPILE__)
+                    __builtin_amdgcn_raw_buffer_store_b128(__builtin_bit_cast(uint4_t, h), rb, bvoff, sbase + (i * nb + jj) * (pblk::BLOCK * 2), PCLIP_NT_STORE ? 2 : 0);
+#endif
+                }
+            m0 = m0n;
+            n0 = n0n;
+            ++stamp_tile;
+            continue;
+        }
         char* buf0 = smem + ring_wr;
         char* buf1 = smem + (ring_wr + 0x8000 == RING_BYTES ? 0 : ring_wr + 0x8000);
         const int etid = fresh_tid(wave);
@@ -303,7 +333,8 @@
     if (N % 256 || K % 64 || K < 192 || M < 1) return false;
     if (lda % 8 || ldb % 8 || ldc % 8 || ((uintptr_t)C & 15) || ((uintptr_t)bias & 7) || ((uintptr_t)residual & 15)) return false;
     if ((long)256 * lda * 2 >= 0x7fffffffL || (long)256 * ldb * 2 >= 0x7fffffffL) return false;
-    if (!(act == 0 || act == 1 || act == 6)) return false;
+    if (!(act == 0 || act == 1 || act == 6 || act == 7)) return false;
+    if (act == 7 && (!bias || residual || ldc != N || pblk::padded_rows(M) * N * 2 >= 0x7fffffffL)) return false;
     if (act == 6 && !(bias && residual)) return false;
     if (act != 6 && residual) return false;
     return true;
@@ -312,6 +343,9 @@
 int pclip_gemm4w_launch_var(const half_t* A, int lda, const half_t* B, int ldb, int M, int N, int K, const half_t* bias, half_t* C, int ldc, int act,
                             const half_t* residual, int slots, int rev, int band, int var, hipStream_t s) {
     if (act == 6) return launch4w<6, true>(A, lda, B, ldb, M, N, K, bias, C, ldc, residual, slots, rev, band, var, s);
+    if (act == 7)
+        return var == STRESS ? launch4w_v<7, true, STRESS>(A, lda, B, ldb, M, N, K, bias, C, ldc, residual, slots, rev, band, s)
+                             : launch4w_v<7, true, PRODUCT>(A, lda, B, ldb, M, N, K, bias, C, ldc, residual, slots, rev, band, s);
     if (act == 1) return bias ? launch4w<1, true>(A, lda, B, ldb, M, N, K, bias, C, ldc, residual, slots, rev, band, var, s)
                               : launch4w<1, false>(A, lda, B, ldb, M, N, K, bias, C, ldc, residual, slots, rev, band, var, s);
     return bias ? launch4w<0, true>(A, lda, B, ldb, M, N, K, bias, C, ldc, residual, slots, rev, band, var, s)
diff --git a/proto-clip_amd/csrc/pclip_linear.hip b/proto-clip_amd/csrc/pclip_linear.hip
--- a/proto-clip_amd/csrc/pclip_linear.hip
+++ b/proto-clip_amd/csrc/pclip_linear.hip
@@ -1,4 +1,5 @@
 #include "pclip_encoder_common.h"
+#include "pclip_blocked.h"
 #include <stdlib.h>
 #include <type_traits>
 
@@ -144,13 +145,15 @@
             static_assert(C::NPASS == 8, "rr[pass % NPASS] pairs slab parity and pass");
             if (full)
                 pgemm::epilogue_pipe<C>(acc, stg, ahead, pre, [&](int r, int c, int pass, half8_t h) {
-                    const size_t o = (size_t)(m0 + r) * ldc + col;
+                    size_t o = (size_t)(m0 + r) * ldc + col;
+                if constexpr (ACT == 7) o = pblk::off(m0 + r, col, N);
                     if (RES) h = add_res(pass, h);
                     if (colok) st_out(Cout + o, h);
                 });
             else
                 pgemm::epilogue_pipe<C>(acc, stg, ahead, pre, [&](int r, int c, int pass, half8_t h) {
-                    const size_t o = (size_t)(m0 + r) * ldc + col;
+                    size_t o = (size_t)(m0 + r) * ldc + col;
+                if constexpr (ACT == 7) o = pblk::off(m0 + r, col, N);
                     if (RES) h = add_res(pass, h);
                     if (m0 + r < M && colok) st_out(Cout + o, h);
                 });
@@ -159,13 +162,15 @@
         }
         if (full)
             pgemm::epilogue_f16<C, M16>(acc, stg, slab, pre, [&](int r, int c, int pass, half8_t h) {
-                const size_t o = (size_t)(m0 + r) * ldc + col;
+                size_t o = (size_t)(m0 + r) * ldc + col;
+                if constexpr (ACT == 7) o = pblk::off(m0 + r, col, N);
                 if (RES) h = add_res(pass, h);
                 if (colok) st_out(Cout + o, h);
             });
         else
             pgemm::epilogue_f16<C, M16>(acc, stg, slab, pre, [&](int r, int c, int pass, half8_t h) {
-                const size_t o = (size_t)(m0 + r) * ldc + col;
+                size_t o = (size_t)(m0 + r) * ldc + col;
+                if constexpr (ACT == 7) o = pblk::off(m0 + r, col, N);
                 if (RES) h = add_res(pass, h);
                 if (m0 + r < M && colok) st_out(Cout + o, h);
             });
@@ -360,6 +365,10 @@
     if (epi.act == 3) return launch_fast2<C, false, 3, KT>(A, lda, B, ldb, M, N, K, epi, slots, s, rt, family);
     if (epi.act == 5) return launch_fast2<C, false, 5, KT>(A, lda, B, ldb, M, N, K, epi, slots, s, rt, family);
     if (epi.act == 6) return launch_fast2<C, true, 6, KT>(A, lda, B, ldb, M, N, K, epi, slots, s, rt, family);
+    if (epi.act == 7) {
+        if constexpr (KT) { pclip_set_error("pclip_gemm_blocked_f16: K=%d must be a multiple of 64", K); return PCLIP_E_INVALID; }
+        else return launch_fast2<C, true, 7, false>(A, lda, B, ldb, M, N, K, epi, slots, s, rt, family);
+    }
     if (epi.bias) {
         if (epi.act == 1) return launch_fast2<C, true, 1, KT>(A, lda, B, ldb, M, N, K, epi, slots, s, rt, family);
         return launch_fast2<C, true, 0, KT>(A, lda, B, ldb, M, N, K, epi, slots, s, rt, family);
@@ -438,13 +447,14 @@
 int pclip_gemm4w_launch_var(const half_t* A, int lda, const half_t* B, int ldb, int M, int N, int K, const half_t* bias, half_t* C, int ldc, int act,
                             const half_t* residual, int slots, int rev, int band, int var, hipStream_t s);
 namespace {
+struct BlockedOperands { const half_t* Bperm; const half_t* bias_perm; int var; };
 int gemm_dispatch(const half_t* A, int lda, const half_t* B, int ldb, int M, int N, int K, LinearEpi epi, int cus, int forced,
-                  bool may_split, hipStream_t s, Route* rt = nullptr) {
+                  bool may_split, hipStream_t s, Route* rt = nullptr, const BlockedOperands* blk = nullptr) {
     const bool kt = K % pgemm::BK != 0;
     const bool aligned = (!epi.residual || ((epi.act == 5 || epi.act == 6) && ((uintptr_t)epi.residual & 15) == 0)) && epi.ldc % 8 == 0 && ((uintptr_t)epi.C & 15) == 0 &&
                          (!epi.bias || ((uintptr_t)epi.bias & 15) == 0) && (!kt || N % 8 == 0);
     const bool ring_ok = aligned && (epi.act <= 1 || epi.act == 6 || (((uintptr_t)epi.scale | (uintptr_t)epi.shift) & 15) == 0);
-    if (ring_ok && forced == -1 && (rt || small_enabled()) && small_applies(M, N, cus, kt))
+    if (!blk && ring_ok && forced == -1 && (rt || small_enabled()) && small_applies(M, N, cus, kt))
         return launch_small_one(A, lda, B, ldb, M, N, K, epi, s, kt, rt);
     if (forced == -3) {
         if (!ring_ok || !(kt || N % 64 == 0)) { pclip_set_error("pclip_gemm_route_f16: N=%d / alignment outside the ring kernel", N); return PCLIP_E_INVALID; }
@@ -453,6 +463,7 @@
     double cost = 1e30;
     int pick = aligned ? best_cfg(M, N, cus, &cost, kt) : -1;
     if (forced == -2) { may_split = false; pick = -1; }
+    if (blk && (pick < 0 || kt)) { pclip_set_error("pclip_gemm_blocked_f16: N=%d K=%d / alignment outside the persistent kernels", N, K); return PCLIP_E_INVALID; }
     if (epi.act == 5 && pick < 0) { pclip_set_error("pclip_gemm_bn_res_f16: N=%d / alignment not supported by the fused epilogue", N); return PCLIP_E_INVALID; }
     if (forced >= 0) {
         may_split = false;
@@ -473,12 +484,12 @@
             if (split < cost) { cost = split; split_cfg = i; split_rows = full_rows; }
         }
         if (split_cfg >= 0) {
-            int rc = gemm_dispatch(A, lda, B, ldb, (int)split_rows, N, K, epi, cus, split_cfg, false, s, rt);
+            int rc = gemm_dispatch(A, lda, B, ldb, (int)split_rows, N, K, epi, cus, split_cfg, false, s, rt, blk);
             if (rc != PCLIP_OK) return rc;
             LinearEpi tail = epi;
             tail.C = epi.C + (size_t)split_rows * epi.ldc;
             if (epi.residual) tail.residual = epi.residual + (size_t)split_rows * epi.ldc;
-            return gemm_dispatch(A + (size_t)split_rows * lda, lda, B, ldb, M - (int)split_rows, N, K, tail, cus, -1, true, s, rt);
+            return gemm_dispatch(A + (size_t)split_rows * lda, lda, B, ldb, M - (int)split_rows, N, K, tail, cus, -1, true, s, rt, blk);
         }
     }
     ++g_gemm_launches;
@@ -488,6 +499,10 @@
         if ((rt ? rt->use4w : g_use4w) && pclip_gemm4w_supports(M, N, K, lda, ldb, epi.ldc, epi.C, epi.bias, epi.residual, epi.act)) {
             const TileOrder& order = rt ? rt->order : tile_order();
             const int rev = order.descending(K) ? 1 : 0, band = N / 256 >= 8 ? order.band : order.band_n;
+            if (blk) {
+                if (blk->var < 0) return pclip_gemm4w_launch(A, lda, blk->Bperm, ldb, M, N, K, blk->bias_perm, epi.C, epi.ldc, 7, nullptr, cus, rev, band, s);
+                return pclip_gemm4w_launch_var(A, lda, blk->Bperm, ldb, M, N, K, blk->bias_perm, epi.C, epi.ldc, 7, nullptr, cus, rev, band, blk->var, s);
+            }
             if (!rt) return pclip_gemm4w_launch(A, lda, B, ldb, M, N, K, epi.bias, epi.C, epi.ldc, epi.act, epi.residual, cus, rev, band, s);
             rt->note(PCLIP_ROUTE_RAN_FOUR_WAVE, false, M, rev, band);
             return pclip_gemm4w_launch_var(A, lda, B, ldb, M, N, K, epi.bias, epi.C, epi.ldc, epi.act, epi.residual, cus, rev, band, rt->use4w == 2 ? 1 : 0, s);
@@ -532,6 +547,25 @@
         nosplit = getenv("PCLIP_GEMM_NOSPLIT") != nullptr;
     }
     return gemm_dispatch((const half_t*)A, lda, (const half_t*)B, ldb, M, N, K, epi, cus, forced, !nosplit, (hipStream_t)stream);
+}
+
+extern "C" int pclip_gemm_blocked_f16(const void* A, int lda, const void* B, const void* Bperm, int ldb, void* C, int M, int N, int K, const void* bias,
+                                      const void* bias_perm, int var, pclip_stream_t stream) {
+    PCLIP_REQUIRE(A && B && Bperm && C && bias && bias_perm, "pclip_gemm_blocked_f16: null pointer");
+    PCLIP_REQUIRE(M >= 0 && N > 0 && K > 0, "pclip_gemm_blocked_f16: bad shape M=%d N=%d K=%d", M, N, K);
+    PCLIP_REQUIRE(N % pblk::COLS == 0 && K % pgemm::BK == 0, "pclip_gemm_blocked_f16: N=%d must be a multiple of 32 and K=%d of 64", N, K);
+    PCLIP_REQUIRE(lda >= K && ldb >= K && lda % 8 == 0 && ldb % 8 == 0, "pclip_gemm_blocked_f16: bad leading dims");
+    PCLIP_REQUIRE(var >= -1 && var <= 2, "pclip_gemm_blocked_f16: unknown kernel choice %d", var);
+    PCLIP_REQUIRE(((uintptr_t)C & 15) == 0 && (((uintptr_t)bias | (uintptr_t)bias_perm) & 15) == 0, "pclip_gemm_blocked_f16: operands must be 16-byte aligned");
+    if (M == 0) return PCLIP_OK;
+    LinearEpi epi{(const half_t*)bias, nullptr, (half_t*)C, N, 7, nullptr, nullptr};
+    const BlockedOperands blk{(const half_t*)Bperm, (const half_t*)bias_perm, var == 2 ? -1 : var};
+    if (var == 2) {
+        int report[1] = {0};
+        Route rt{tile_order(), 0, report, 0};
+        return gemm_dispatch((const half_t*)A, lda, (const half_t*)B, ldb, M, N, K, epi, pclip_cus(), -1, true, (hipStream_t)stream, &rt, &blk);
+    }
+    return gemm_dispatch((const half_t*)A, lda, (const half_t*)B, ldb, M, N, K, epi, pclip_cus(), -1, getenv("PCLIP_GEMM_NOSPLIT") == nullptr, (hipStream_t)stream, nullptr, &blk);
 }
 
 extern "C" int pclip_gemm_route_f16(const void* A, int lda, const void* B, int ldb, void* C, int ldc, int M, int N, int K, const void* bias, int act,
diff --git a/proto-clip_amd/ops.py b/proto-clip_amd/ops.py
--- a/proto-clip_amd/ops.py
+++ b/proto-clip_amd/ops.py
@@ -767,6 +767,58 @@
     check(_lib.load().pclip_gemm4w_var_f16(ptr(a), a.stride(0), ptr(w), w.stride(0), ptr(out), out.stride(0), M, N, K, ptr(bias), act, ptr(residual), var,
                                            stream()), "pclip_gemm4w_f16")
     return out
+
+
+
+def blocked_perm(n: int, device=None) -> torch.Tensor:
+    p = torch.arange(n, device=device)
+    rem = p % 32
+    return (p - rem) + 8 * ((rem % 16) // 4) + 4 * (rem // 16) + rem % 4
+
+
+def blocked_permute(w: torch.Tensor) -> torch.Tensor:
+    return w[blocked_perm(w.shape[0], w.device)].contiguous()
+
+
+def unblock(c: torch.Tensor, M: int, N: int) -> torch.Tensor:
+    Mp = (M + 15) // 16 * 16
+    return c.view(Mp // 16, N // 32, 16, 32).permute(0, 2, 1, 3).reshape(Mp, N)[:M].contiguous()
+
+
+def gemm_blocked(a, w, bias, w_perm, bias_perm, var: int = -1, out=None):
+    require_cuda(a, w, bias, w_perm, bias_perm, out)
+    M, K = a.shape
+    N = w.shape[0]
+    if w.stride(0) != w_perm.stride(0) or w_perm.shape != w.shape or bias_perm.shape != bias.shape:
+        raise _lib.PclipError("gemm_blocked: the permuted operands must have the shapes and row stride of the plain ones")
+    need = (M + 15) // 16 * 16 * N
+    if out is None:
+        out = torch.empty(need, dtype=torch.float16, device=a.device)
+    elif out.dtype != torch.float16 or not out.is_contiguous() or out.numel() < need:
+        raise _lib.PclipError(f"gemm_blocked: out must be a contiguous fp16 buffer of at least {need} elements")
+    check(_lib.load().pclip_gemm_blocked_f16(ptr(a), a.stride(0), ptr(w), ptr(w_perm), w.stride(0), ptr(out), M, N, K, ptr(bias), ptr(bias_perm), var, stream()),
+          "pclip_gemm_blocked_f16")
+    return out
+
+
+def attention_blocked(qkv, B: int, L: int, H: int):
+    require_cuda(qkv)
+    W = H * 64
+    out = torch.empty(B * L, W, dtype=torch.float16, device=qkv.device)
+    check(_lib.load().pclip_attention_blocked_f16(ptr(qkv), 3 * W, 0, 1, ptr(qkv), 3 * W, W, 2 * W, ptr(out), B, L, L, H, 64, stream()), "pclip_attention_blocked_f16")
+    return out
+
+
+def attention_first_queries_blocked(q, kv, B: int, L: int, Lq: int, H: int):
+    require_cuda(q, kv)
+    W = H * 64
+    out = torch.empty(B * Lq, W, dtype=torch.float16, device=q.device)
+    check(_lib.load().pclip_attention_blocked_f16(ptr(q), W, Lq * W, 0, ptr(kv), 2 * W, 0, W, ptr(out), B, L, Lq, H, 64, stream()), "pclip_attention_blocked_f16")
+    return out
+
+
+def qkv_blocked_applies(M: int, N: int, K: int, L: int) -> bool:
+    return N % 256 == 0 and K % 64 == 0 and K >= 192 and 0 < L <= ATT_SHORT_MAX_L and (M + 15) // 16 * 16 * N * 2 < 2 ** 31 - 1 and not splitk_active(M)
 
 
 ROUTE_AUTO, ROUTE_GENERIC, ROUTE_RING = _lib.ROUTE_AUTO, _lib.ROUTE_GENERIC, _lib.ROUTE_RING
diff --git a/proto-clip_amd/tower.py b/proto-clip_amd/tower.py
--- a/proto-clip_amd/tower.py
+++ b/proto-clip_amd/tower.py
@@ -11,20 +11,38 @@
             pr.weight, pr.bias]
 
 
-def residual_block(x, h, params, B, L, heads, causal, pick=None, first_token=False, splitk=False, rec=None):
+def _blocked_in_proj(blocked, win, bin_):
+    cache, i = blocked
+    return cache.get(("in_proj_perm", i), win, ops.blocked_permute), cache.get(("in_proj_bias_perm", i), bin_, ops.blocked_permute)
+
+
+def residual_block(x, h, params, B, L, heads, causal, pick=None, first_token=False, splitk=False, rec=None, blocked=None):
     ln1w, ln1b, win, bin_, wout, bout, ln2w, ln2b, wfc, bfc, wpr, bpr = params
+    use_blocked = blocked is not None and rec is None and not causal and win.dtype == torch.float16 and bin_ is not None and \
+        ops.qkv_blocked_applies(h.shape[0], win.shape[0], win.shape[1], L)
     if rec is not None:
         rec.update(x_in=x.clone(), h1=h, picked=pick is not None)
     if pick is not None and first_token and not causal:
         W = x.shape[1]
-        kv = ops.gemm(h, win[W:3 * W], bin_[W:3 * W])
+        if use_blocked:
+            wp, bp = _blocked_in_proj(blocked, win, bin_)
+            kv = ops.gemm_blocked(h, win[W:3 * W], bin_[W:3 * W], wp[W:3 * W], bp[W:3 * W])
+        else:
+            kv = ops.gemm(h, win[W:3 * W], bin_[W:3 * W])
         q = ops.gemm(pick(h), win[0:W], bin_[0:W])
-        a, x = ops.attention_first_queries(q, kv, B, L, 1, heads), pick(x)
+        if use_blocked:
+            a, x = ops.attention_first_queries_blocked(q, kv, B, L, 1, heads), pick(x)
+        else:
+            a, x = ops.attention_first_queries(q, kv, B, L, 1, heads), pick(x)
         if rec is not None:
             rec.update(q=q, kv=kv)
     else:
-        qkv = ops.gemm(h, win, bin_)
-        a = ops.attention(qkv, B, L, heads, causal=causal)
+        if use_blocked:
+            qkv = ops.gemm_blocked(h, win, bin_, *_blocked_in_proj(blocked, win, bin_))
+            a = ops.attention_blocked(qkv, B, L, heads)
+        else:
+            qkv = ops.gemm(h, win, bin_)
+            a = ops.attention(qkv, B, L, heads, causal=causal)
         if rec is not None:
             rec.update(qkv=qkv)
         if pick is not None:
@@ -45,14 +63,15 @@
     return x, None
 
 
-def _run_blocks(x, blocks, B, L, heads, causal, select=None, first_token=False, h0=None):
+def _run_blocks(x, blocks, B, L, heads, causal, select=None, first_token=False, h0=None, blocked=None):
     params = [_block_params(blk) for blk in blocks]
     n, d = len(params), None
     if n > 0:
         h = h0 if h0 is not None else ops.layernorm(x, params[0][0], params[0][1])
     for i in range(n):
         last = i == n - 1
-        x, d = residual_block(x, h, params[i], B, L, heads, causal, select if last else None, first_token, splitk=True)
+        x, d = residual_block(x, h, params[i], B, L, heads, causal, select if last else None, first_token, splitk=True,
+                              blocked=None if blocked is None else (blocked, i))
         if not last:
             lnw, lnb = params[i + 1][0], params[i + 1][1]
             h = ops.layernorm(x, lnw, lnb) if d is None else ops.add_layernorm(x, d, lnw, lnb)
@@ -77,8 +96,8 @@
 
 class Tower:
 
-    def __init__(self, entry, name, stem_word, *, blocks, heads, causal, ln, proj, cache, projT_key, prefix, head, pick):
-        self.entry, self.name, self.stem_word = entry, name, stem_word
+    def __init__(self, entry, name, stem_word, *, blocks, heads, causal, ln, proj, cache, projT_key, prefix, head, pick, qkv_blocked=True):
+        self.entry, self.name, self.stem_word, self.qkv_blocked = entry, name, stem_word, qkv_blocked
         self.blocks, self.heads, self.causal, self.ln, self.proj, self.cache, self.projT_key = blocks, heads, causal, ln, proj, cache, projT_key
         self.prefix, self.head, self.pick, self.first_token = prefix, head, pick, not causal
         self.stem_opt_in = False
@@ -113,8 +132,9 @@
 def run_tower(tw, x, B, L, plan, pick, what=None, h0=None, deep=None, deep_off=None):
     first, stem = plan
     select, _ = pick
+    blocked = tw.cache if tw.qkv_blocked else None
     if first is None:
-        x, d = _run_blocks(x, tw.blocks, B, L, tw.heads, tw.causal, select=select, first_token=tw.first_token, h0=h0)
+        x, d = _run_blocks(x, tw.blocks, B, L, tw.heads, tw.causal, select=select, first_token=tw.first_token, h0=h0, blocked=blocked)
         if d is None:
             y = ops.layernorm(x, tw.ln.weight, tw.ln.bias)
         else:
@@ -124,11 +144,11 @@
     what = tw.what(first, stem) if what is None else what
     if first == len(tw.blocks) and not x.requires_grad:
         with torch.no_grad():
-            x, _ = _run_blocks(x, tw.blocks, B, L, tw.heads, tw.causal, select=select, first_token=tw.first_token, h0=h0)
+            x, _ = _run_blocks(x, tw.blocks, B, L, tw.heads, tw.causal, select=select, first_token=tw.first_token, h0=h0, blocked=blocked)
         return run_tower_tail(tw, x, None, first, B, L, (None, None), what)
     if first > 0:
         with torch.no_grad():
-            x, _ = _run_blocks(x, tw.blocks[:first], B, L, tw.heads, tw.causal, h0=h0)
+            x, _ = _run_blocks(x, tw.blocks[:first], B, L, tw.heads, tw.causal, h0=h0, blocked=blocked)
         h0 = None
     return run_tower_tail(tw, x, h0, first, B, L, pick, what, deep=deep, deep_off=deep_off)
 
```

Result: no change. 28950 query images/sec (-0.5%).
